# GeoMop/MLMC

Hardware: AMD Instinct MI355X
Metric: moment-evals/sec (samples x n_moments) (higher is better)
Workload: dtype f64

## Files before the change

mlmc_amd/csrc/api.hip:

```cpp
#include <cmath>
#include <chrono>
#include <cstring>
#include <new>

#include "common.hpp"
#include <algorithm>
#include <map>

namespace mlmc {

static thread_local std::string g_err;
void set_error(const std::string &msg) { g_err = msg; }
int fail(const std::string &msg) {
    g_err = msg;
    return 1;
}
Runtime &rt() {
    static Runtime r;
    return r;
}
std::recursive_mutex &api_mutex() {
    static std::recursive_mutex m;
    return m;
}

void bind_thread_to_device() {
    static thread_local int bound = -1;
    const Runtime &r = rt();
    if (r.ready && bound != r.device) {
        if (hipSetDevice(r.device) == hipSuccess) bound = r.device;
    } else if (!r.ready) {
        bound = -1;
    }
}

int ensure(void **p, size_t *cap, size_t bytes) {
    if (bytes <= *cap && *p) return 0;
    if (*p) {
        MLMC_HIP_CHECK(wait_stream(rt().stream));
        MLMC_HIP_CHECK(hipFree(*p));
        *p = nullptr;
        *cap = 0;
    }
    size_t want = bytes < 256 ? 256 : bytes;
    MLMC_HIP_CHECK(hipMalloc(p, want));
    *cap = want;
    return 0;
}

static int timing_collect(mlmc_accum *a);
int timing_begin(mlmc_accum *a) {
    if (!(rt().flags & 1)) return 0;
    if (a->ev_used >= 8192) {
        MLMC_HIP_CHECK(hipEventSynchronize(a->ev[a->ev_used - 1]));
        if (int rc = timing_collect(a)) return rc;
    }
    if (a->ev_used + 2 > a->ev.size()) {
        hipEvent_t e0, e1;
        MLMC_HIP_CHECK(hipEventCreate(&e0));
        MLMC_HIP_CHECK(hipEventCreate(&e1));
        a->ev.push_back(e0);
        a->ev.push_back(e1);
    }
    MLMC_HIP_CHECK(hipEventRecord(a->ev[a->ev_used], rt().stream));
    return 0;
}
int timing_end(mlmc_accum *a) {
    if (!(rt().flags & 1)) return 0;
    MLMC_HIP_CHECK(hipEventRecord(a->ev[a->ev_used + 1], rt().stream));
    a->ev_used += 2;
    return 0;
}
static int timing_collect(mlmc_accum *a) {
    for (size_t i = 0; i + 1 < a->ev_used; i += 2) {
        float ms = 0.f;
        MLMC_HIP_CHECK(hipEventElapsedTime(&ms, a->ev[i], a->ev[i + 1]));
        a->ms_total += ms;
    }
    a->ev_used = 0;
    return 0;
}

static void log_keep_interval(const BasisParams &p, double *x_lo, double *x_hi) {
    auto t_of = [&](uint64_t bits) {
        double x;
        std::memcpy(&x, &bits, sizeof x);
        volatile double v = std::log(x);
        volatile double w = (v - p.shift) * p.scale;
        return (double)(w + p.ref0);
    };
    auto as_double = [](uint64_t bits) { double x; std::memcpy(&x, &bits, sizeof x); return x; };
    const uint64_t top = 0x7ff0000000000000ull;
    uint64_t lo = 1, hi = top;
    while (lo < hi) {
        const uint64_t mid = lo + (hi - lo) / 2;
        if (t_of(mid) >= p.ref0) hi = mid; else lo = mid + 1;
    }
    const uint64_t first = lo;
    lo = 0; hi = top - 1;
    while (lo < hi) {
        const uint64_t mid = lo + (hi - lo + 1) / 2;
        if (t_of(mid) <= p.ref1) lo = mid; else hi = mid - 1;
    }
    const uint64_t last = lo;
    if (first >= top || last == 0 || first > last) {
        *x_lo = HUGE_VAL;
        *x_hi = 0.0;
        return;
    }
    *x_lo = as_double(first);
    *x_hi = as_double(last);
}

bool product_table(int kind, int R, std::vector<double> &out) {
    if (kind != MLMC_LEGENDRE && kind != MLMC_MONOMIAL) return false;
    const int K = 2 * R - 1;
    const size_t RR = (size_t)R * R;
    out.assign((size_t)K * RR, 0.0);
    for (int i = 0; i < R; ++i)
        for (int j = 0; j < R; ++j) {
            const size_t ij = (size_t)i * R + j;
            if (kind == MLMC_MONOMIAL) { out[(size_t)(i + j) * RR + ij] = 1.0; continue; }
            typedef long double ld;
            const int hi = i > j ? i : j, lo = i > j ? j : i;
            const ld diff = (ld)(hi - lo);
            ld c = (2 * diff + 1) / (2 * (ld)hi + 1);
            for (int t = 1; t <= lo; ++t) {
                const ld tt = (ld)t;
                c = c * ((2 * tt - 1) / tt * (diff + tt) / (2 * (diff + tt) - 1));
            }
            for (int t = 0; t <= lo; ++t) {
                const int k = (hi - lo) + 2 * t;
                out[(size_t)k * RR + ij] = (double)c;
                if (t == lo) break;
                const ld s = (ld)hi + t, kk = (ld)k;
                const ld si = s - hi, sj = s - lo, sk = s - kk;
                ld ratio = ((2 * kk + 5) / (2 * s + 3)) / ((2 * kk + 1) / (2 * s + 1));
                ratio = ratio * ((2 * si + 1) / (si + 1)) * ((2 * sj + 1) / (sj + 1));
                ratio = ratio * (sk / (2 * sk - 1));
                ratio = ratio * ((s + 1) / (2 * s + 1));
                c = c * ratio;
            }
        }
    return true;
}

bool square_product_table(int kind, int R, std::vector<double> &out) {
    if (kind != MLMC_LEGENDRE && kind != MLMC_MONOMIAL) return false;
    const int K = 4 * R - 3;
    const size_t RR = (size_t)R * R;
    out.assign((size_t)K * RR, 0.0);
    if (kind == MLMC_MONOMIAL) {
        for (int i = 0; i < R; ++i)
            for (int j = 0; j < R; ++j) out[(size_t)(2 * (i + j)) * RR + (size_t)i * R + j] = 1.0;
        return true;
    }
    typedef long double ld;
    const int Q = 4 * R;
    const ld pi = 3.14159265358979323846264338327950288L;
    std::vector<ld> x(Q), w(Q), P((size_t)K * Q);
    for (int q = 0; q < Q; ++q) {
        ld t = std::cos(pi * ((ld)q + 0.75L) / ((ld)Q + 0.5L)), dp = 1.0L;
        for (int it = 0; it < 100; ++it) {
            ld p0 = 1.0L, p1 = t;
            for (int k = 2; k <= Q; ++k) {
                const ld p2 = ((2 * k - 1) * t * p1 - (k - 1) * p0) / k;
                p0 = p1;
                p1 = p2;
            }
            dp = Q * (t * p1 - p0) / (t * t - 1.0L);
            const ld dt = p1 / dp;
            t -= dt;
            if (std::fabs(dt) < 1e-20L) break;
        }
        {
            ld p0 = 1.0L, p1 = t;
            for (int k = 2; k <= Q; ++k) {
                const ld p2 = ((2 * k - 1) * t * p1 - (k - 1) * p0) / k;
                p0 = p1;
                p1 = p2;
            }
            dp = Q * (t * p1 - p0) / (t * t - 1.0L);
        }
        x[q] = t;
        w[q] = 2.0L / ((1.0L - t * t) * dp * dp);
        ld p0 = 1.0L, p1 = t;
        P[(size_t)0 * Q + q] = 1.0L;
        if (K > 1) P[(size_t)1 * Q + q] = t;
        for (int k = 2; k < K; ++k) {
            const ld p2 = ((2 * k - 1) * t * p1 - (k - 1) * p0) / k;
            p0 = p1;
            p1 = p2;
            P[(size_t)k * Q + q] = p2;
        }
    }
    std::vector<ld> sq(Q);
    for (int i = 0; i < R; ++i)
        for (int j = i; j < R; ++j) {
            for (int q = 0; q < Q; ++q) {
                const ld u = P[(size_t)i * Q + q] * P[(size_t)j * Q + q];
                sq[q] = w[q] * u * u;
            }
            for (int k = 0; k <= 2 * (i + j); k += 2) {
                ld acc = 0.0L;
                const ld *Pk = &P[(size_t)k * Q];
                for (int q = 0; q < Q; ++q) acc += sq[q] * Pk[q];
                const double c = (double)(acc * (2 * k + 1) / 2);
                out[(size_t)k * RR + (size_t)i * R + j] = c;
                out[(size_t)k * RR + (size_t)j * R + i] = c;
            }
        }
    std::vector<double> t1;
    product_table(kind, R, t1);
    for (int j = 0; j < R; ++j)
        for (int k = 0; k < K; ++k) {
            const double c = k < 2 * R - 1 ? t1[(size_t)k * RR + (size_t)j * R + j] : 0.0;
            out[(size_t)k * RR + (size_t)j] = c;
            out[(size_t)k * RR + (size_t)j * R] = c;
        }
    return true;
}

static bool linearize_enabled() {
    const char *e = std::getenv("MLMC_HIP_LINEARIZE");
    return !(e && e[0] == '0');
}

static int lin_min_size() {
    const char *e = std::getenv("MLMC_HIP_LINEARIZE_MIN");
    return e ? std::atoi(e) : 16;
}

static int need_runtime() {
    if (!rt().ready) return fail("mlmc_init has not been called (no HIP device bound)");
    return 0;
}

}

using namespace mlmc;

extern "C" {

int mlmc_abi_version(void) { return MLMC_ABI_VERSION; }
const char *mlmc_last_error(void) { return g_err.c_str(); }

int mlmc_init(int device, int flags) {
    MLMC_API_GUARD;
    Runtime &r = rt();
    int count = 0;
    hipError_t e = hipGetDeviceCount(&count);
    if (e != hipSuccess || count <= 0) return fail("no HIP device available: libmlmc_hip has no CPU fallback");
    if (device < 0 || device >= count) return fail("mlmc_init: device index out of range");
    if (r.ready && r.device == device) {
        r.flags = flags;
        return 0;
    }
    if (r.ready) return fail("mlmc_init: this process is already bound to another device (one process per GPU)");
    MLMC_HIP_CHECK(hipSetDevice(device));
    MLMC_HIP_CHECK(hipGetDeviceProperties(&r.prop, device));
    if (std::strncmp(r.prop.gcnArchName, "gfx950", 6) != 0)
        return fail(std::string("mlmc_init: kernels are built for gfx950 only, device is ") + r.prop.gcnArchName);
    MLMC_HIP_CHECK(hipStreamCreateWithFlags(&r.stream, hipStreamNonBlocking));
    r.own_stream = true;
    r.device = device;
    r.flags = flags;
    r.n_cu = r.prop.multiProcessorCount;
    r.ready = true;
    return 0;
}

}

namespace mlmc {
hipError_t wait_stream(hipStream_t st) {
    const auto t0 = std::chrono::steady_clock::now();
    for (int spins = 0;; ++spins) {
        const hipError_t e = hipStreamQuery(st);
        if (e != hipErrorNotReady) return e;
        if ((spins & 63) == 63 && std::chrono::steady_clock::now() - t0 > std::chrono::milliseconds(4)) break;
    }
    return hipStreamSynchronize(st);
}
}

extern "C" {

int mlmc_set_stream(void *stream) {
    MLMC_API_GUARD;
    Runtime &r = rt();
    if (!r.ready) return fail("mlmc_init has not been called (no HIP device bound)");
    MLMC_HIP_CHECK(wait_stream(r.stream));
    if (r.own_stream) (void)hipStreamDestroy(r.stream);
    r.stream = (hipStream_t)stream;
    r.own_stream = false;
    return 0;
}

int mlmc_wait_event(void *hip_event) {
    MLMC_API_GUARD;
    Runtime &r = rt();
    if (!r.ready) return fail("mlmc_init has not been called (no HIP device bound)");
    if (!hip_event) return fail("mlmc_wait_event: null event");
    MLMC_HIP_CHECK(hipStreamWaitEvent(r.stream, (hipEvent_t)hip_event, 0));
    return 0;
}

int mlmc_synchronize(void) {
    MLMC_API_GUARD;
    Runtime &r = rt();
    if (!r.ready) return fail("mlmc_init has not been called (no HIP device bound)");
    MLMC_HIP_CHECK(wait_stream(r.stream));
    return 0;
}

void mlmc_shutdown(void) {
    MLMC_API_GUARD;
    Runtime &r = rt();
    if (!r.ready) return;
    (void)wait_stream(r.stream);
    if (r.own_stream) (void)hipStreamDestroy(r.stream);
    r.stream = nullptr;
    r.ready = false;
    r.device = -1;
}

int mlmc_device_info(char *name, int name_len, int *n_cu, int *wave_size, int64_t *hbm_bytes) {
    MLMC_API_GUARD;
    if (need_runtime()) return 1;
    if (name && name_len > 0) {
        std::strncpy(name, rt().prop.name, (size_t)name_len - 1);
        name[name_len - 1] = 0;
    }
    if (n_cu) *n_cu = rt().prop.multiProcessorCount;
    if (wave_size) *wave_size = rt().prop.warpSize;
    if (hbm_bytes) *hbm_bytes = (int64_t)rt().prop.totalGlobalMem;
    return 0;
}

int mlmc_basis_create(const mlmc_basis_desc *d, mlmc_basis **out) {
    MLMC_API_GUARD;
    if (need_runtime()) return 1;
    if (!d || !out) return fail("mlmc_basis_create: null argument");
    if (d->size <= 0) return fail("mlmc_basis_create: size must be > 0");
    if (d->kind < MLMC_LEGENDRE || d->kind > MLMC_SPLINE) return fail("mlmc_basis_create: unknown kind");
    if (d->kind == MLMC_SPLINE && d->size < 4) return fail("mlmc_basis_create: cubic spline moments need size >= 4");
    if (d->kind == MLMC_IDENTITY && d->size != 1) return fail("mlmc_basis_create: IDENTITY has size 1");
    if (d->out_size < 0 || (d->out_size > 0 && !d->matrix)) return fail("mlmc_basis_create: matrix missing");
    if (d->kind == MLMC_LEGENDRE && d->size > 512) return fail("mlmc_basis_create: at most 512 Legendre moments");
    mlmc_basis *b = new (std::nothrow) mlmc_basis();
    if (!b) return fail("out of memory");
    b->p.kind = d->kind;
    b->p.size = d->size;
    b->p.shift = d->shift;
    b->p.scale = d->scale;
    b->p.ref0 = d->ref0;
    b->p.ref1 = d->ref1;
    b->p.is_log = d->is_log;
    b->p.is_clip = d->is_clip;
    b->p.x_lo = d->x_lo;
    b->p.x_hi = d->x_hi;
    if (d->is_log && d->is_clip && d->x_lo == 0.0 && d->x_hi == 0.0) log_keep_interval(b->p, &b->p.x_lo, &b->p.x_hi);
    b->out_size = d->out_size;
    const int R = d->size;
    b->scale_c.assign(R, 1.0);
    if (d->kind == MLMC_LEGENDRE) {
        long double c = 1.0L;
        for (int i = 0; i < R; ++i) {
            if (i >= 1) c = c * (long double)(2 * i - 1) / (long double)(2 * i);
            b->scale_c[i] = (double)c;
        }
    }
    hipError_t e = hipMalloc(&b->d_scale, sizeof(double) * R);
    if (e == hipSuccess) e = hipMemcpy(b->d_scale, b->scale_c.data(), sizeof(double) * R, hipMemcpyHostToDevice);
    if (e == hipSuccess && d->out_size > 0) {
        b->matrix.assign(d->matrix, d->matrix + (size_t)d->out_size * R);
        e = hipMalloc(&b->d_matrix, sizeof(double) * b->matrix.size());
        if (e == hipSuccess)
            e = hipMemcpy(b->d_matrix, b->matrix.data(), sizeof(double) * b->matrix.size(), hipMemcpyHostToDevice);
    }
    if (e != hipSuccess) {
        mlmc_basis_destroy(b);
        return fail(std::string("mlmc_basis_create: ") + hipGetErrorString(e));
    }
    *out = b;
    return 0;
}

void mlmc_basis_destroy(mlmc_basis *b) {
    MLMC_API_GUARD;
    if (!b) return;
    if (b->d_scale) (void)hipFree(b->d_scale);
    if (b->d_matrix) (void)hipFree(b->d_matrix);
    delete b;
}

int mlmc_basis_eval(const mlmc_basis *b, const double *x, int64_t n, int32_t size, double *out, int mem_kind) {
    MLMC_API_GUARD;
    if (need_runtime()) return 1;
    if (!b || (n > 0 && (!x || !out))) return fail("mlmc_basis_eval: null argument");
    const int max_size = b->out_size > 0 ? b->out_size : b->p.size;
    if (size <= 0 || size > max_size) return fail("mlmc_basis_eval: size out of range");
    if (n == 0) return 0;
    hipStream_t st = rt().stream;
    if (mem_kind == MLMC_DEVICE) {
        if (int rc = launch_eval(b, x, n, size, out)) return rc;
        MLMC_HIP_CHECK(wait_stream(st));
        return 0;
    }
    double *d_x = nullptr, *d_o = nullptr;
    hipError_t e0 = hipMalloc(&d_x, sizeof(double) * (size_t)n);
    if (e0 == hipSuccess) e0 = hipMalloc(&d_o, sizeof(double) * (size_t)n * size);
    if (e0 == hipSuccess) e0 = hipMemcpyAsync(d_x, x, sizeof(double) * (size_t)n, hipMemcpyHostToDevice, st);
    int rc = e0 == hipSuccess ? launch_eval(b, d_x, n, size, d_o) : fail(std::string("mlmc_basis_eval: ") + hipGetErrorString(e0));
    if (!rc) {
        hipError_t e = hipMemcpyAsync(out, d_o, sizeof(double) * (size_t)n * size, hipMemcpyDeviceToHost, st);
        if (e == hipSuccess) e = wait_stream(st);
        if (e != hipSuccess) rc = fail(std::string("mlmc_basis_eval copy back: ") + hipGetErrorString(e));
    }
    (void)hipFree(d_x);
    (void)hipFree(d_o);
    return rc;
}

struct LinTables {
    double *d_prod = nullptr, *d_prod2 = nullptr;
};
static int lin_tables(int kind, int R, bool squares, LinTables **out) {
    static std::map<std::pair<int, int>, LinTables> cache;
    LinTables &t = cache[std::make_pair(kind, R)];
    if (!t.d_prod) {
        std::vector<double> h;
        product_table(kind, R, h);
        MLMC_HIP_CHECK(hipMalloc(&t.d_prod, sizeof(double) * h.size()));
        MLMC_HIP_CHECK(hipMemcpy(t.d_prod, h.data(), sizeof(double) * h.size(), hipMemcpyHostToDevice));
    }
    if (squares && !t.d_prod2) {
        std::vector<double> h;
        square_product_table(kind, R, h);
        MLMC_HIP_CHECK(hipMalloc(&t.d_prod2, sizeof(double) * h.size()));
        MLMC_HIP_CHECK(hipMemcpy(t.d_prod2, h.data(), sizeof(double) * h.size(), hipMemcpyHostToDevice));
    }
    *out = &t;
    return 0;
}

static int ensure_lin(mlmc_accum *a) {
    if (a->lin) return 0;
    const mlmc_basis *b = a->basis;
    LinTables *t = nullptr;
    if (int rc = lin_tables(b->p.kind, a->R, a->lin0_eligible, &t)) return rc;
    mlmc_basis_desc d;
    std::memset(&d, 0, sizeof(d));
    d.kind = b->p.kind;
    d.size = 2 * a->R - 1;
    d.shift = b->p.shift; d.scale = b->p.scale; d.ref0 = b->p.ref0; d.ref1 = b->p.ref1;
    d.is_log = b->p.is_log; d.is_clip = b->p.is_clip;
    d.x_lo = b->p.x_lo; d.x_hi = b->p.x_hi;
    int rc = mlmc_basis_create(&d, &a->lin_basis);
    if (!rc) rc = mlmc_accum_create(a->lin_basis, a->n_levels, MLMC_MODE_MOMENTS | MLMC_MODE_MEAN_ONLY, a->n_comp, &a->lin);
    if (!rc) {
        a->lin_basis->p.x_lo = b->p.x_lo;
        a->lin_basis->p.x_hi = b->p.x_hi;
        a->lin->host_outputs = false;
        a->lin_K = d.size;
        a->d_lin_prod = t->d_prod;
    }
    if (!rc && a->lin0_eligible) {
        d.size = 4 * a->R - 3;
        rc = mlmc_basis_create(&d, &a->lin0_basis);
        if (!rc) rc = mlmc_accum_create(a->lin0_basis, a->n_levels, MLMC_MODE_MOMENTS | MLMC_MODE_MEAN_ONLY, a->n_comp, &a->lin0);
        if (!rc) {
            a->lin0_basis->p.x_lo = b->p.x_lo;
            a->lin0_basis->p.x_hi = b->p.x_hi;
            a->lin0->host_outputs = false;
            a->lin0_K = d.size;
            a->d_lin0_prod = t->d_prod2;
        }
    }
    if (rc) {
        if (a->lin) mlmc_accum_destroy(a->lin);
        if (a->lin_basis) mlmc_basis_destroy(a->lin_basis);
        if (a->lin0) mlmc_accum_destroy(a->lin0);
        if (a->lin0_basis) mlmc_basis_destroy(a->lin0_basis);
        a->lin = a->lin0 = nullptr;
        a->lin_basis = a->lin0_basis = nullptr;
        a->lin_eligible = a->lin0_eligible = false;
    }
    return rc;
}

int mlmc_accum_create(const mlmc_basis *b, int32_t n_levels, int32_t mode, int32_t n_comp, mlmc_accum **out) {
    MLMC_API_GUARD;
    if (need_runtime()) return 1;
    if (!b || !out) return fail("mlmc_accum_create: null argument");
    if (n_levels <= 0 || n_comp <= 0) return fail("mlmc_accum_create: n_levels and n_comp must be > 0");
    const bool mean_only = (mode & MLMC_MODE_MEAN_ONLY) != 0;
    mode &= ~MLMC_MODE_MEAN_ONLY;
    if (mode != MLMC_MODE_MOMENTS && mode != MLMC_MODE_COV) return fail("mlmc_accum_create: unknown mode");
    mlmc_accum *a = new (std::nothrow) mlmc_accum();
    if (!a) return fail("out of memory");
    a->basis = b;
    a->n_levels = n_levels;
    a->mode = mode;
    const bool spline_band = mode == MLMC_MODE_COV && mean_only && b->out_size == 0 && b->p.kind == MLMC_SPLINE && b->p.size <= SPLINE_BAND_MAX_R;
    a->cov_from_values = mode == MLMC_MODE_COV && (b->out_size > 0 || (b->p.size > 128 && !spline_band));
    a->mean_only = mean_only && ((mode == MLMC_MODE_COV && !a->cov_from_values) || (mode == MLMC_MODE_MOMENTS && b->out_size > 0));
    a->mean_only_plain = mean_only && mode == MLMC_MODE_MOMENTS && b->out_size == 0 &&
                         (b->p.kind == MLMC_LEGENDRE || b->p.kind == MLMC_MONOMIAL) && b->p.size > 64 && b->p.size <= 256;
    a->n_comp = n_comp;
    a->R = b->p.size;
    a->Rout = b->out_size > 0 ? b->out_size : b->p.size;
    a->RP = (((mode == MLMC_MODE_COV && b->out_size > 0 ? a->Rout : a->R) + 15) / 16) * 16;
    if (mode == MLMC_MODE_MOMENTS) {
        a->K = (int64_t)n_comp * a->Rout;
        a->int_width = 2 * (int64_t)a->R + (b->out_size > 0 ? (int64_t)a->RP * a->RP : 0);
    } else {
        a->K = (int64_t)n_comp * a->Rout * a->Rout;
        a->int_width = 3 * (int64_t)a->RP * a->RP;
    }
    const size_t tot = (size_t)n_levels * n_comp * a->int_width;
    a->state_bytes = sizeof(double) * tot + sizeof(int64_t) * 2 * n_levels;
    a->out_bytes = (sizeof(int64_t) + sizeof(double)) * 2 * n_levels + 2 * sizeof(double) * (size_t)n_levels * a->K;
    if (hipMalloc(&a->d_state, a->state_bytes) != hipSuccess || hipMalloc(&a->d_out, a->out_bytes) != hipSuccess ||
        hipHostMalloc(&a->h_out, a->out_bytes, hipHostMallocDefault) != hipSuccess) {
        mlmc_accum_destroy(a);
        return fail("mlmc_accum_create: device / pinned allocation failed");
    }
    a->d_totals = (double *)a->d_state;
    a->d_counts = (int64_t *)(a->d_totals + tot);
    a->level_flushed.assign(n_levels, 0);
    if (mode == MLMC_MODE_MOMENTS && n_comp == 1 && b->out_size == 0) {
        void *dev_view = nullptr;
        if (hipHostGetDevicePointer(&dev_view, a->h_out, 0) == hipSuccess && dev_view) {
            a->host_outputs = true;
            a->h_out_n = (int64_t *)dev_view;
            a->h_out_s = (double *)(a->h_out_n + 2 * (size_t)n_levels) + 2 * (size_t)n_levels;
            a->h_out_sp = a->h_out_s + (size_t)n_levels * a->K;
        }
    }
    a->d_out_n = (int64_t *)a->d_out;
    a->d_out_nd = (double *)(a->d_out_n + 2 * (size_t)n_levels);
    a->d_out_s = a->d_out_nd + 2 * (size_t)n_levels;
    a->d_out_sp = a->d_out_s + (size_t)n_levels * a->K;
    if (mode == MLMC_MODE_COV && !mean_only && !a->cov_from_values && b->out_size == 0 && b->p.size > lin_min_size() && b->p.size <= 128 &&
        (b->p.kind == MLMC_LEGENDRE || b->p.kind == MLMC_MONOMIAL) && b->p.is_clip &&
        std::fabs(b->p.ref0) <= 1.0 && std::fabs(b->p.ref1) <= 1.0 &&
        linearize_enabled()) {
        a->lin_eligible = true;
        const char *min_n = std::getenv("MLMC_HIP_LINEARIZE_MIN_N");
        a->lin_min_n = min_n ? std::atoll(min_n) : (a->R > 32 ? 100000 : 1500000);
        const char *lin0_env = std::getenv("MLMC_HIP_LINEARIZE_LEVEL0");
        a->lin0_eligible = a->R <= 64 && !(lin0_env && lin0_env[0] == '0');
    }
    *out = a;
    return mlmc_accum_reset(a);
}

int mlmc_accum_reset(mlmc_accum *a) {
    MLMC_API_GUARD;
    if (need_runtime()) return 1;
    if (!a) return fail("mlmc_accum_reset: null argument");
    hipStream_t st = rt().stream;
    a->pending.clear();
    std::fill(a->level_flushed.begin(), a->level_flushed.end(), 0);
    MLMC_HIP_CHECK(hipMemsetAsync(a->d_state, 0, a->state_bytes, st));
    if (a->xcov) {
        MLMC_HIP_CHECK(hipMemcpyAsync(a->d_shift, a->shift_host.data(), sizeof(double) * a->shift_host.size(), hipMemcpyHostToDevice, st));
        a->xcov_pushes = 0;
    }
    a->lin_used = a->lin0_used = false;
    if (a->lin0)
        if (int rc = mlmc_accum_reset(a->lin0)) return rc;
    if (a->lin) return mlmc_accum_reset(a->lin);
    return 0;
}

void mlmc_accum_destroy(mlmc_accum *a) {
    MLMC_API_GUARD;
    if (!a) return;
    if (rt().ready) (void)wait_stream(rt().stream);
    if (a->lin) mlmc_accum_destroy(a->lin);
    if (a->lin_basis) mlmc_basis_destroy(a->lin_basis);
    if (a->lin0) mlmc_accum_destroy(a->lin0);
    if (a->lin0_basis) mlmc_basis_destroy(a->lin0_basis);
    void *ptrs[] = {a->d_state, a->d_partials, a->d_pcounts, a->d_stage_f, a->d_stage_c, a->d_mask, a->d_out, a->d_vals_f, a->d_vals_c, a->d_vals_tmp,
                    a->d_shift};
    for (void *p : ptrs)
        if (p) (void)hipFree(p);
    if (a->h_out) (void)hipHostFree(a->h_out);
    for (hipEvent_t e : a->ev) (void)hipEventDestroy(e);
    delete a;
}

int mlmc_accum_push(mlmc_accum *a, int32_t level, const double *fine, const double *coarse, int64_t n, int mem_kind) {
    MLMC_API_GUARD;
    if (need_runtime()) return 1;
    if (!a) return fail("mlmc_accum_push: null argument");
    if (level < 0 || level >= a->n_levels) return fail("mlmc_accum_push: level out of range");
    if (n < 0) return fail("mlmc_accum_push: negative n");
    if (n == 0) return 0;
    if (!fine) return fail("mlmc_accum_push: fine is NULL");
    if (n > ((int64_t)1 << 40)) return fail("mlmc_accum_push: chunk too large, split it");
    hipStream_t st = rt().stream;
    const size_t bytes = sizeof(double) * (size_t)n * a->n_comp;
    const double *d_f = fine, *d_c = coarse;
    if (mem_kind == MLMC_HOST) {
        if (bytes > a->stage_cap) {
            MLMC_HIP_CHECK(wait_stream(st));
            if (a->d_stage_f) (void)hipFree(a->d_stage_f);
            if (a->d_stage_c) (void)hipFree(a->d_stage_c);
            a->d_stage_f = a->d_stage_c = nullptr;
            a->stage_cap = 0;
            MLMC_HIP_CHECK(hipMalloc(&a->d_stage_f, bytes));
            MLMC_HIP_CHECK(hipMalloc(&a->d_stage_c, bytes));
            a->stage_cap = bytes;
        } else {
            MLMC_HIP_CHECK(wait_stream(st));
        }
        MLMC_HIP_CHECK(hipMemcpyAsync(a->d_stage_f, fine, bytes, hipMemcpyHostToDevice, st));
        d_f = a->d_stage_f;
        if (coarse) {
            MLMC_HIP_CHECK(hipMemcpyAsync(a->d_stage_c, coarse, bytes, hipMemcpyHostToDevice, st));
            d_c = a->d_stage_c;
        }
        MLMC_HIP_CHECK(wait_stream(st));
    } else if (mem_kind != MLMC_DEVICE) {
        return fail("mlmc_accum_push: bad mem_kind");
    }
    if (a->xcov) {
        ++a->xcov_pushes;
        return launch_xcov_push(a, level, d_f, d_c, n);
    }
    const uint8_t *d_mask = nullptr;
    bool count_in_kernel = true;
    if (a->n_comp > 1) {
        if (int rc = ensure((void **)&a->d_mask, &a->mask_cap, (size_t)n)) return rc;
        if (int rc = launch_mask(a, d_f, d_c, n, a->d_mask, a->d_counts + 2 * (int64_t)level)) return rc;
        d_mask = a->d_mask;
        count_in_kernel = false;
    }
    for (int m = 0; m < a->n_comp; ++m) {
        const double *f_m = d_f + (int64_t)m * n;
        const double *c_m = d_c ? d_c + (int64_t)m * n : nullptr;
        const bool count = count_in_kernel && m == 0;
        int rc;
        if (a->mode == MLMC_MODE_MOMENTS) {
            const bool defer = mem_kind == MLMC_DEVICE || a->n_comp > 1;
            rc = launch_moments_accum(a, level, m, f_m, c_m, d_mask, n, count, defer);
            if (!rc && a->basis->out_size > 0 && !a->mean_only) {
                if (a->R <= 128) {
                    rc = launch_cov_accum(a, level, m, f_m, c_m, d_mask, n, false, 1);
                } else {
                    int64_t chunk = 1 << 22;
                    while (chunk > 4096 && chunk * a->R > ((int64_t)1 << 28)) chunk >>= 1;
                    const size_t need = sizeof(double) * (size_t)(n < chunk ? n : chunk) * a->R;
                    if (need > a->vals_cap) {
                        MLMC_HIP_CHECK(wait_stream(st));
                        if (a->d_vals_f) (void)hipFree(a->d_vals_f);
                        if (a->d_vals_c) (void)hipFree(a->d_vals_c);
                        a->d_vals_f = a->d_vals_c = nullptr;
                        a->vals_cap = 0;
                        MLMC_HIP_CHECK(hipMalloc(&a->d_vals_f, need));
                        MLMC_HIP_CHECK(hipMalloc(&a->d_vals_c, need));
                        a->vals_cap = need;
                    }
                    for (int64_t off = 0; off < n && !rc; off += chunk) {
                        const int64_t m_n = (n - off < chunk) ? n - off : chunk;
                        rc = launch_eval_scaled_base(a->basis, f_m + off, m_n, a->d_vals_f);
                        if (!rc && c_m) rc = launch_eval_scaled_base(a->basis, c_m + off, m_n, a->d_vals_c);
                        if (!rc) rc = launch_cov_from_values(a, level, m, a->d_vals_f, c_m ? a->d_vals_c : nullptr,
                                                             d_mask ? d_mask + off : nullptr, m_n, false, 1);
                    }
                }
            }
        } else if (a->cov_from_values) {
            const int R1 = a->Rout;
            int64_t chunk = 1 << 22;
            while (chunk > 4096 && chunk * R1 > ((int64_t)1 << 28)) chunk >>= 1;
            const size_t need = sizeof(double) * (size_t)(n < chunk ? n : chunk) * R1;
            if (need > a->vals_cap) {
                MLMC_HIP_CHECK(wait_stream(st));
                if (a->d_vals_f) (void)hipFree(a->d_vals_f);
                if (a->d_vals_c) (void)hipFree(a->d_vals_c);
                a->d_vals_f = a->d_vals_c = nullptr;
                a->vals_cap = 0;
                MLMC_HIP_CHECK(hipMalloc(&a->d_vals_f, need));
                MLMC_HIP_CHECK(hipMalloc(&a->d_vals_c, need));
                a->vals_cap = need;
            }
            if (a->basis->out_size > 0) {
                const size_t need_tmp = sizeof(double) * (size_t)(n < chunk ? n : chunk) * a->R;
                if (need_tmp > a->vals_tmp_cap) {
                    MLMC_HIP_CHECK(wait_stream(st));
                    if (a->d_vals_tmp) (void)hipFree(a->d_vals_tmp);
                    a->d_vals_tmp = nullptr;
                    a->vals_tmp_cap = 0;
                    MLMC_HIP_CHECK(hipMalloc(&a->d_vals_tmp, need_tmp));
                    a->vals_tmp_cap = need_tmp;
                }
            }
            rc = 0;
            for (int64_t off = 0; off < n && !rc; off += chunk) {
                const int64_t m_n = (n - off < chunk) ? n - off : chunk;
                rc = launch_eval(a->basis, f_m + off, m_n, R1, a->d_vals_f, a->d_vals_tmp);
                if (!rc && c_m) rc = launch_eval(a->basis, c_m + off, m_n, R1, a->d_vals_c, a->d_vals_tmp);
                if (!rc) rc = launch_cov_from_values(a, level, m, a->d_vals_f, c_m ? a->d_vals_c : nullptr,
                                                     d_mask ? d_mask + off : nullptr, m_n, count);
            }
        } else {
            if (a->lin_eligible && !a->lin && n >= a->lin_min_n)
                if (int rcl = ensure_lin(a)) return rcl;
            const bool use_lin0 = a->lin0 && !d_c && n >= a->lin_min_n;
            if (use_lin0) {
                a->lin0_used = true;
                rc = launch_moments_accum(a->lin0, level, m, f_m, nullptr, d_mask, n, count_in_kernel && m == 0,
                                          mem_kind == MLMC_DEVICE || a->n_comp > 1);
                if (rc) return rc;
                continue;
            }
            const bool use_lin = a->lin && n >= a->lin_min_n;
            rc = m == 0 ? launch_cov_accum(a, level, 0, d_f, d_c, d_mask, n, count_in_kernel, a->mean_only ? 2 : (use_lin ? 3 : 0), a->n_comp) : 0;
            if (!rc && use_lin) a->lin_used = true;
            if (!rc && use_lin)
                rc = launch_moments_accum(a->lin, level, m, f_m, c_m, d_mask, n, false, mem_kind == MLMC_DEVICE || a->n_comp > 1);
        }
        if (rc) return rc;
    }
    if (a->mode == MLMC_MODE_MOMENTS && (mem_kind == MLMC_HOST || a->n_comp > 1))
        if (int rc = flush_moments(a)) return rc;
    if (a->lin && (mem_kind == MLMC_HOST || a->n_comp > 1))
        if (int rc = flush_moments(a->lin)) return rc;
    if (a->lin0 && (mem_kind == MLMC_HOST || a->n_comp > 1))
        if (int rc = flush_moments(a->lin0)) return rc;
    return 0;
}

int mlmc_accum_finalize(mlmc_accum *a, int64_t *n, int64_t *n_rm, double *s, double *sp, int mem_kind) {
    MLMC_API_GUARD;
    if (need_runtime()) return 1;
    if (!a || !n || !n_rm || !s || !sp) return fail("mlmc_accum_finalize: null argument");
    hipStream_t st = rt().stream;
    if (a->mode == MLMC_MODE_MOMENTS)
        if (int rcf = flush_moments(a)) return rcf;
    const int L = a->n_levels;
    const size_t nk = (size_t)L * a->K;
    if (a->host_outputs && mem_kind == MLMC_HOST) {
        MLMC_HIP_CHECK(wait_stream(st));
        const int64_t *hn = (const int64_t *)a->h_out;
        const double *hs = (const double *)(hn + 2 * (size_t)L) + 2 * (size_t)L;
        const size_t K = (size_t)a->K;
        for (int l = 0; l < L; ++l) {
            if (a->level_flushed[l]) {
                n[l] = hn[l];
                n_rm[l] = hn[L + l];
                std::memcpy(s + l * K, hs + l * K, sizeof(double) * K);
                std::memcpy(sp + l * K, hs + nk + l * K, sizeof(double) * K);
            } else {
                n[l] = n_rm[l] = 0;
                std::fill(s + l * K, s + (l + 1) * K, 0.0);
                std::fill(sp + l * K, sp + (l + 1) * K, 0.0);
            }
        }
        return 0;
    }
    int rc = a->xcov ? launch_xcov_finalize(a) : (a->mode == MLMC_MODE_MOMENTS) ? launch_moments_finalize(a) : launch_cov_finalize(a);
    if (rc) return rc;
    if (mem_kind == MLMC_DEVICE) {
        MLMC_HIP_CHECK(hipMemcpyAsync(n, a->d_out_n, sizeof(int64_t) * L, hipMemcpyDeviceToDevice, st));
        MLMC_HIP_CHECK(hipMemcpyAsync(n_rm, a->d_out_n + L, sizeof(int64_t) * L, hipMemcpyDeviceToDevice, st));
        MLMC_HIP_CHECK(hipMemcpyAsync(s, a->d_out_s, sizeof(double) * nk, hipMemcpyDeviceToDevice, st));
        MLMC_HIP_CHECK(hipMemcpyAsync(sp, a->d_out_sp, sizeof(double) * nk, hipMemcpyDeviceToDevice, st));
        MLMC_HIP_CHECK(wait_stream(st));
    } else {
        MLMC_HIP_CHECK(hipMemcpyAsync(a->h_out, a->d_out, a->out_bytes, hipMemcpyDeviceToHost, st));
        MLMC_HIP_CHECK(wait_stream(st));
        const int64_t *hn = (const int64_t *)a->h_out;
        const double *hs = (const double *)(hn + 2 * (size_t)L) + 2 * (size_t)L;
        std::memcpy(n, hn, sizeof(int64_t) * L);
        std::memcpy(n_rm, hn + L, sizeof(int64_t) * L);
        std::memcpy(s, hs, sizeof(double) * nk);
        std::memcpy(sp, hs + nk, sizeof(double) * nk);
    }
    return 0;
}

int mlmc_accum_estimate(mlmc_accum *a, int32_t n_chunks, const int32_t *levels, const double *const *fine,
                        const double *const *coarse, const int64_t *n_samples, int mem_kind, int64_t *n, int64_t *n_rm,
                        double *s, double *sp) {
    MLMC_API_GUARD;
    if (!a || n_chunks < 0 || (n_chunks > 0 && (!levels || !fine || !n_samples))) return fail("mlmc_accum_estimate: null argument");
    if (int rc = mlmc_accum_reset(a)) return rc;
    for (int k = 0; k < n_chunks; ++k)
        if (int rc = mlmc_accum_push(a, levels[k], fine[k], coarse ? coarse[k] : nullptr, n_samples[k], mem_kind)) return rc;
    return mlmc_accum_finalize(a, n, n_rm, s, sp, MLMC_HOST);
}

int mlmc_accum_finalize_packed(mlmc_accum *a, double *packed, int mem_kind) {
    MLMC_API_GUARD;
    if (need_runtime()) return 1;
    if (!a || !packed) return fail("mlmc_accum_finalize_packed: null argument");
    hipStream_t st = rt().stream;
    if (a->mode == MLMC_MODE_MOMENTS && a->host_outputs && mem_kind == MLMC_DEVICE && a->R <= MAX_TERMS_PER_PASS &&
        (int)a->pending.size() == a->n_levels &&
        std::none_of(a->level_flushed.begin(), a->level_flushed.end(), [](char f) { return f != 0; })) {
        a->packed_target = packed;
        const int rcf = flush_moments(a);
        a->packed_target = nullptr;
        return rcf;
    }
    if (a->mode == MLMC_MODE_MOMENTS)
        if (int rcf = flush_moments(a)) return rcf;
    int rc = a->xcov ? launch_xcov_finalize(a) : (a->mode == MLMC_MODE_MOMENTS) ? launch_moments_finalize(a) : launch_cov_finalize(a);
    if (rc) return rc;
    const size_t bytes = sizeof(double) * (2 * (size_t)a->n_levels + 2 * (size_t)a->n_levels * a->K);
    MLMC_HIP_CHECK(hipMemcpyAsync(packed, a->d_out_nd, bytes, mem_kind == MLMC_DEVICE ? hipMemcpyDeviceToDevice : hipMemcpyDeviceToHost, st));
    if (mem_kind == MLMC_DEVICE) return 0;
    MLMC_HIP_CHECK(wait_stream(st));
    return 0;
}

int mlmc_accum_estimate_packed(mlmc_accum *a, int32_t n_chunks, const int32_t *levels, const double *const *fine,
                               const double *const *coarse, const int64_t *n_samples, int mem_kind, double *packed,
                               int packed_kind) {
    MLMC_API_GUARD;
    if (!a || n_chunks < 0 || (n_chunks > 0 && (!levels || !fine || !n_samples))) return fail("mlmc_accum_estimate_packed: null argument");
    if (int rc = mlmc_accum_reset(a)) return rc;
    for (int k = 0; k < n_chunks; ++k)
        if (int rc = mlmc_accum_push(a, levels[k], fine[k], coarse ? coarse[k] : nullptr, n_samples[k], mem_kind)) return rc;
    return mlmc_accum_finalize_packed(a, packed, packed_kind);
}

int mlmc_accum_kernel_time(mlmc_accum *a, double *ms, int64_t *launches, int64_t *alg_bytes) {
    MLMC_API_GUARD;
    if (!a) return fail("mlmc_accum_kernel_time: null argument");
    if (a->ev_used) {
        MLMC_HIP_CHECK(hipEventSynchronize(a->ev[a->ev_used - 1]));
        if (int rc = timing_collect(a)) return rc;
    }
    if (ms) *ms = a->ms_total;
    if (launches) *launches = a->launches;
    if (alg_bytes) *alg_bytes = a->alg_bytes;
    a->ms_total = 0;
    a->launches = 0;
    a->alg_bytes = 0;
    return 0;
}

int mlmc_accum_aux_kernel_time(mlmc_accum *a, double *ms, int64_t *launches, int64_t *alg_bytes) {
    MLMC_API_GUARD;
    if (!a) return fail("mlmc_accum_aux_kernel_time: null argument");
    double t = 0.0, t0 = 0.0;
    int64_t l = 0, l0 = 0, b = 0, b0 = 0;
    if (a->lin)
        if (int rc = mlmc_accum_kernel_time(a->lin, &t, &l, &b)) return rc;
    if (a->lin0)
        if (int rc = mlmc_accum_kernel_time(a->lin0, &t0, &l0, &b0)) return rc;
    if (ms) *ms = t + t0;
    if (launches) *launches = l + l0;
    if (alg_bytes) *alg_bytes = b + b0;
    return 0;
}

int mlmc_linearization_table(int32_t kind, int32_t R, int32_t squares, double *out, int64_t out_len) {
    if (!out) return fail("mlmc_linearization_table: null argument");
    if (kind != MLMC_LEGENDRE && kind != MLMC_MONOMIAL) return fail("mlmc_linearization_table: Legendre or monomial moments");
    if (R < 1 || R > (squares ? 64 : 128)) return fail("mlmc_linearization_table: size out of range");
    const int64_t K = squares ? 4 * (int64_t)R - 3 : 2 * (int64_t)R - 1;
    if (out_len < K * R * R) return fail("mlmc_linearization_table: output too small");
    std::vector<double> t;
    if (squares) square_product_table(kind, R, t);
    else product_table(kind, R, t);
    std::memcpy(out, t.data(), sizeof(double) * t.size());
    return 0;
}

int mlmc_xcov_create(int32_t M, int32_t n_levels, int32_t flags, mlmc_accum **out) {
    MLMC_API_GUARD;
    if (need_runtime()) return 1;
    if (!out) return fail("mlmc_xcov_create: null argument");
    if (M < 1 || M > XCOV_MAX_M)
        return fail("mlmc_xcov_create: M = " + std::to_string(M) + " components, supported are 1 .. " + std::to_string(XCOV_MAX_M));
    if (n_levels <= 0) return fail("mlmc_xcov_create: n_levels must be > 0");
    if (flags & ~MLMC_MODE_MEAN_ONLY) return fail("mlmc_xcov_create: unknown flags (only MLMC_MODE_MEAN_ONLY)");
    mlmc_accum *a = new (std::nothrow) mlmc_accum();
    if (!a) return fail("out of memory");
    a->xcov = true;
    a->mode = MODE_XCOV;
    a->n_levels = n_levels;
    a->n_comp = M;
    a->mean_only = (flags & MLMC_MODE_MEAN_ONLY) != 0;
    a->K = (int64_t)M * M;
    a->int_width = 2 * a->K;
    const size_t tot = (size_t)n_levels * a->int_width;
    a->state_bytes = sizeof(double) * tot + sizeof(int64_t) * 2 * n_levels;
    a->out_bytes = (sizeof(int64_t) + sizeof(double)) * 2 * n_levels + 2 * sizeof(double) * (size_t)n_levels * a->K;
    a->shift_host.assign(M, 0.0);
    if (hipMalloc(&a->d_state, a->state_bytes) != hipSuccess || hipMalloc(&a->d_out, a->out_bytes) != hipSuccess ||
        hipMalloc(&a->d_shift, sizeof(double) * M) != hipSuccess ||
        hipHostMalloc(&a->h_out, a->out_bytes, hipHostMallocDefault) != hipSuccess) {
        mlmc_accum_destroy(a);
        return fail("mlmc_xcov_create: device / pinned allocation failed");
    }
    a->d_totals = (double *)a->d_state;
    a->d_counts = (int64_t *)(a->d_totals + tot);
    a->level_flushed.assign(n_levels, 0);
    a->d_out_n = (int64_t *)a->d_out;
    a->d_out_nd = (double *)(a->d_out_n + 2 * (size_t)n_levels);
    a->d_out_s = a->d_out_nd + 2 * (size_t)n_levels;
    a->d_out_sp = a->d_out_s + (size_t)n_levels * a->K;
    *out = a;
    return mlmc_accum_reset(a);
}

int mlmc_xcov_set_shift(mlmc_accum *a, const double *shift_host) {
    MLMC_API_GUARD;
    if (need_runtime()) return 1;
    if (!a) return fail("mlmc_xcov_set_shift: null argument");
    if (!a->xcov) return fail("mlmc_xcov_set_shift: not a component-covariance accumulator (mlmc_xcov_create)");
    if (a->xcov_pushes > 0) return fail("mlmc_xcov_set_shift: pushes are pending; reset the accumulator first");
    const int M = a->n_comp;
    if (shift_host)
        for (int m = 0; m < M; ++m)
            if (!std::isfinite(shift_host[m])) return fail("mlmc_xcov_set_shift: shift[" + std::to_string(m) + "] is not finite");
    MLMC_HIP_CHECK(wait_stream(rt().stream));
    if (shift_host) std::memcpy(a->shift_host.data(), shift_host, sizeof(double) * M);
    else std::fill(a->shift_host.begin(), a->shift_host.end(), 0.0);
    return 0;
}

int mlmc_accum_kernel_flops(mlmc_accum *a, int64_t *mfma_flops) {
    MLMC_API_GUARD;
    if (!a) return fail("mlmc_accum_kernel_flops: null argument");
    if (mfma_flops) *mfma_flops = a->mfma_flops;
    a->mfma_flops = 0;
    return 0;
}

}
```

mlmc_amd/csrc/common.hpp:

```cpp
#pragma once
#include <hip/hip_runtime.h>
#include <stdint.h>
#include <mutex>
#include <string>
#include <vector>

#include "../../include/mlmc_hip.h"

namespace mlmc {

constexpr int WAVE = 64;
constexpr int ACC_THREADS = 256;
#ifndef MLMC_TERMS_PER_PASS
#define MLMC_TERMS_PER_PASS 64
#endif
constexpr int MAX_TERMS_PER_PASS = MLMC_TERMS_PER_PASS;
constexpr int SPLINE_BAND_MAX_R = 256;

void set_error(const std::string &msg);
int fail(const std::string &msg);
#define MLMC_HIP_CHECK(expr)                                                                   \
    do {                                                                                       \
        hipError_t _e = (expr);                                                                \
        if (_e != hipSuccess)                                                                  \
            return ::mlmc::fail(std::string(#expr) + ": " + hipGetErrorString(_e));            \
    } while (0)

std::recursive_mutex &api_mutex();
void bind_thread_to_device();
struct ApiGuard {
    std::lock_guard<std::recursive_mutex> lock;
    ApiGuard() : lock(api_mutex()) { bind_thread_to_device(); }
};
#define MLMC_API_GUARD ::mlmc::ApiGuard mlmc_api_guard_

struct Runtime {
    bool ready = false;
    int device = -1;
    int flags = 0;
    int n_cu = 0;
    hipStream_t stream = nullptr;
    bool own_stream = false;
    hipDeviceProp_t prop;
};
Runtime &rt();
hipError_t wait_stream(hipStream_t st);

__device__ __forceinline__ unsigned long long order_key(double x) {
    unsigned long long u = (unsigned long long)__double_as_longlong(x);
    return (u >> 63) ? ~u : (u | 0x8000000000000000ull);
}

__device__ __forceinline__ void philox_round(uint32_t (&c)[4], uint32_t k0, uint32_t k1) {
    const uint64_t p0 = (uint64_t)0xD2511F53u * c[0], p1 = (uint64_t)0xCD9E8D57u * c[2];
    const uint32_t n0 = (uint32_t)(p1 >> 32) ^ c[1] ^ k0, n1 = (uint32_t)p1;
    const uint32_t n2 = (uint32_t)(p0 >> 32) ^ c[3] ^ k1, n3 = (uint32_t)p0;
    c[0] = n0; c[1] = n1; c[2] = n2; c[3] = n3;
}

struct BasisParams {
    int kind;
    int size;
    double shift, scale, ref0, ref1;
    int is_log, is_clip;
    double x_lo, x_hi;
};

}

struct mlmc_basis {
    mlmc::BasisParams p;
    int out_size = 0;
    std::vector<double> matrix;
    std::vector<double> scale_c;
    double *d_scale = nullptr;
    double *d_matrix = nullptr;
};

struct PendingSeg {
    const double *fine, *coarse;
    const uint8_t *mask;
    int64_t n;
    int level, comp;
    bool count;
};

struct mlmc_accum {
    const mlmc_basis *basis = nullptr;
    int n_levels = 0, mode = 0, n_comp = 1;
    bool mean_only = false;
    bool cov_from_values = false;
    bool mean_only_plain = false;
    int R = 0;
    int Rout = 0;
    int64_t K = 0;
    int64_t int_width = 0;
    void *d_state = nullptr;
    size_t state_bytes = 0;
    double *d_totals = nullptr;
    int64_t *d_counts = nullptr;
    double *d_partials = nullptr; size_t partials_cap = 0;
    int64_t *d_pcounts = nullptr; size_t pcounts_cap = 0;
    double *d_stage_f = nullptr, *d_stage_c = nullptr; size_t stage_cap = 0;
    uint8_t *d_mask = nullptr; size_t mask_cap = 0;
    double *d_vals_f = nullptr, *d_vals_c = nullptr; size_t vals_cap = 0;
    double *d_vals_tmp = nullptr; size_t vals_tmp_cap = 0;
    void *d_out = nullptr;
    size_t out_bytes = 0;
    void *h_out = nullptr;
    bool host_outputs = false;
    double *packed_target = nullptr;
    double *h_out_s = nullptr, *h_out_sp = nullptr; int64_t *h_out_n = nullptr;
    std::vector<char> level_flushed;
    double *d_out_s = nullptr, *d_out_sp = nullptr, *d_out_nd = nullptr; int64_t *d_out_n = nullptr;
    std::vector<hipEvent_t> ev;
    size_t ev_used = 0;
    double ms_total = 0;
    int64_t launches = 0, alg_bytes = 0;
    int64_t mfma_flops = 0;
    int RP = 0;
    bool lin_eligible = false, lin0_eligible = false;
    mlmc_accum *lin = nullptr;
    mlmc_basis *lin_basis = nullptr;
    double *d_lin_prod = nullptr;
    int lin_K = 0;
    mlmc_accum *lin0 = nullptr;
    mlmc_basis *lin0_basis = nullptr;
    double *d_lin0_prod = nullptr;
    int lin0_K = 0;
    bool lin0_used = false;
    int64_t lin_min_n = 0;
    bool lin_used = false;
    std::vector<PendingSeg> pending;
    bool xcov = false;
    double *d_shift = nullptr;
    std::vector<double> shift_host;
    int64_t xcov_pushes = 0;
};

namespace mlmc {
int launch_eval(const mlmc_basis *b, const double *d_x, int64_t n, int size, double *d_out, double *scratch = nullptr);
int launch_eval_scaled_base(const mlmc_basis *b, const double *d_x, int64_t n, double *d_out);
int launch_mask(const mlmc_accum *a, const double *d_f, const double *d_c, int64_t n, uint8_t *d_mask, int64_t *d_counts_level);
int launch_moments_accum(mlmc_accum *a, int level, int comp, const double *d_f, const double *d_c, const uint8_t *d_mask,
                         int64_t n, bool count, bool defer);
int flush_moments(mlmc_accum *a);
int launch_moments_finalize(mlmc_accum *a);
int launch_cov_accum(mlmc_accum *a, int level, int comp, const double *d_f, const double *d_c, const uint8_t *d_mask,
                     int64_t n, bool count, int gram_mode, int ncomp = 1);
int launch_cov_finalize(mlmc_accum *a);
constexpr int XCOV_MAX_M = 1024;
constexpr int MODE_XCOV = 2;
int launch_xcov_push(mlmc_accum *a, int level, const double *d_f, const double *d_c, int64_t n);
int launch_xcov_finalize(mlmc_accum *a);
bool product_table(int kind, int R, std::vector<double> &out);
bool square_product_table(int kind, int R, std::vector<double> &out);
int launch_cov_from_values(mlmc_accum *a, int level, int comp, const double *d_vf, const double *d_vc, const uint8_t *d_mask,
                           int64_t n, bool count, int gram_mode = 0);
int ensure(void **p, size_t *cap, size_t bytes);
void gauss_legendre(int n, std::vector<double> &x, std::vector<double> &w);
std::vector<double> effective_coeffs(const mlmc_basis *b, const double *lambda, const double *sigma, int R1);
int timing_begin(mlmc_accum *a);
int timing_end(mlmc_accum *a);
}
```

mlmc_amd/csrc/cov.hip:

```cpp
#include "device_basis.hpp"

namespace mlmc {

typedef double v4f64 __attribute__((ext_vector_type(4)));
#ifdef MLMC_PROF_COV
__device__ unsigned long long *g_prof_cov;
#define MLMC_COV_STAMP(slot)                                      \
    {                                                             \
        const unsigned long long now_ = __builtin_amdgcn_s_memtime(); \
        prof_acc[slot] += now_ - prof_t;                          \
        prof_t = now_;                                            \
    }
#else
#define MLMC_COV_STAMP(slot)
#endif
#ifndef MLMC_COV_PRIO_MFMA
#define MLMC_COV_PRIO_MFMA 0
#define MLMC_COV_PRIO_EVAL 2
#endif
#ifndef MLMC_COV_SLICE_BITS
#define MLMC_COV_SLICE_BITS 17
#endif
#ifndef MLMC_COV_EXTRA
#define MLMC_COV_EXTRA 2
#endif
#define MLMC_COV_MFMA_PRIO(ranks, slot, nslots, clock)                                                \
    do {                                                                                              \
        const unsigned t_ = (unsigned)((clock) >> MLMC_COV_SLICE_BITS);                               \
        unsigned top_ = t_ % (nslots);                                                                \
        if (MLMC_COV_EXTRA > 0) {                                                                     \
            const unsigned u_ = t_ % ((nslots) * MLMC_COV_EXTRA + 1u);                                \
            top_ = u_ == (nslots) * MLMC_COV_EXTRA ? (nslots) - 1u : u_ % (nslots);                   \
        }                                                                                             \
        const unsigned rank_ = ((slot) + (nslots) - top_ + (nslots) - 1u) % (nslots);   \
        if (ranks) {                                                                                  \
            if (rank_ == 0) __builtin_amdgcn_s_setprio(0);                                            \
            else if (rank_ == 1) __builtin_amdgcn_s_setprio(1);                                       \
            else if (rank_ == 2) __builtin_amdgcn_s_setprio(2);                                       \
            else __builtin_amdgcn_s_setprio(3);                                                       \
        } else {                                                                                      \
            if (rank_ == (nslots) - 1u) __builtin_amdgcn_s_setprio(1);                                \
            else __builtin_amdgcn_s_setprio(0);                                                       \
        }                                                                                             \
    } while (0)
#define MLMC_COV_EVAL_PRIO(ranks)                                                                     \
    do {                                                                                              \
        if (ranks) __builtin_amdgcn_s_setprio(3);                                                     \
        else __builtin_amdgcn_s_setprio(MLMC_COV_PRIO_EVAL);                                          \
    } while (0)
constexpr int COV_BATCH = 64;
#ifndef MLMC_COV_BLK22
#define MLMC_COV_BLK22 1
#endif
#ifndef MLMC_COV_T4_ONE_LIST
#define MLMC_COV_T4_ONE_LIST 1
#endif
#ifndef MLMC_COV_T4_BATCH
#define MLMC_COV_T4_BATCH 32
#define MLMC_COV_T4_WGS 4
#endif
constexpr int COV_T4_BATCH = MLMC_COV_T4_BATCH;
constexpr int COV_T4_WGS = MLMC_COV_T4_WGS;
#ifndef MLMC_COV_B128
#define MLMC_COV_B128 1
#endif
#ifndef MLMC_COV_B128_PAD
#define MLMC_COV_B128_PAD (MLMC_COV_B128 ? 4 : 2)
#endif
__device__ __forceinline__ int cov_t4_pos(int s) { return MLMC_COV_B128 ? ((s & ~7) | ((s & 3) << 1) | ((s >> 2) & 1)) : s; }
#ifndef MLMC_COV_WIDE_BATCH
#define MLMC_COV_WIDE_BATCH 32
#endif
__host__ __device__ constexpr int cov_ng(int mode) { return mode == 0 ? 3 : (mode == 3 ? 2 : 1); }
#ifndef MLMC_COV_VAR_RANKS
#define MLMC_COV_VAR_RANKS 1
#endif
__host__ __device__ constexpr int cov_batch(int T, bool wide, bool vals, bool pair = true) {
    return (T <= 2 && !wide && !vals) ? (pair ? 128 : 256) : ((wide && pair && !vals) ? MLMC_COV_WIDE_BATCH : 64);
}

template <int NT, int STRIDE, int TA>
__device__ __forceinline__ void cov_spline_store(const TermGen<MLMC_SPLINE> &g, double *__restrict__ dst, int samp) {
#pragma unroll
    for (int i = 0; i < NT; ++i) dst[i * STRIDE + samp] = 0.0;
    if (TA == 0) dst[samp] = g.w;
    const double nj[4] = {g.n0, g.n1, g.n2, g.n3};
#pragma unroll
    for (int j = 0; j < 4; ++j) {
        const int term = g.k + j;
        const int r = term - TA;
        if (term >= 1 && r >= 0 && r < NT) dst[r * STRIDE + samp] = nj[j];
    }
}

template <int KIND, int T, bool PAIR, int MODE, int BI = 0, int BJ = 0, bool VALS = false>
__global__ __launch_bounds__(256, (BI != BJ && (!PAIR || MLMC_COV_WIDE_BATCH == 64 || VALS)) ? 1 : 2) void k_cov_accum(BasisParams bp, 
                                                      const double *__restrict__ fine,
                                                      const double *__restrict__ coarse,
                                                      const uint8_t *__restrict__ mask, int64_t n, int R,
                                                      double *__restrict__ partials, int64_t *__restrict__ pcounts,
                                                      int vals_ta, int vals_tb) {
    constexpr int NT = 16 * T;
    constexpr int BATCH = cov_batch(T, BI != BJ, VALS, PAIR);
    constexpr int STRIDE = BATCH + 2;
    constexpr int NSL = 4 / T;
    constexpr bool M0 = MODE == 0 || MODE == 3;
    constexpr bool DO_G0 = MODE == 0;
    constexpr int NG = M0 ? (PAIR ? 3 : 2) : 1;
    constexpr bool WIDE = BI != BJ;
    constexpr int TA = 64 * BI, TB = 64 * BJ;
    constexpr int N_EVAL = (BI > BJ ? TA : TB) + NT;
    static_assert(T == 4 || (BI == 0 && BJ == 0), "term windows need T = 4");
    __shared__ double lds_f[NT * STRIDE];
    __shared__ double lds_c[PAIR ? NT * STRIDE : 1];
    __shared__ double lds_fb[WIDE ? NT * STRIDE : 1];
    __shared__ double lds_cb[(WIDE && PAIR) ? NT * STRIDE : 1];
    __shared__ int ldc[4][2];
    __shared__ unsigned char keep_s[VALS ? BATCH : 1];

    fine += (int64_t)blockIdx.y * n;
    if (PAIR) coarse += (int64_t)blockIdx.y * n;
    partials += (int64_t)blockIdx.y * gridDim.x * ((T <= 2 && BI == BJ) ? 4 : 4 / T) * ((M0 ? 3 : 1) * (16 * T) * (16 * T));
    if (blockIdx.y) pcounts = nullptr;

    const int lane = threadIdx.x & 63, wave = threadIdx.x >> 6;
    const int I = wave % T, kslice = wave / T;

    constexpr bool SLICED = (T <= 2) && !WIDE;
    constexpr int TI = SLICED ? T : 1;
    v4f64 acc[NG][TI][T];
#pragma unroll
    for (int g = 0; g < NG; ++g)
#pragma unroll
        for (int i = 0; i < TI; ++i)
#pragma unroll
            for (int j = 0; j < T; ++j) acc[g][i][j] = (v4f64){0.0, 0.0, 0.0, 0.0};

    const int n_eval_waves = PAIR ? BATCH / 32 : BATCH / 64;
    const bool evaluator = wave < n_eval_waves;
    const int samp = PAIR ? (wave * 32 + (lane & 31)) : (wave * 64 + lane);
    const bool is_coarse = PAIR && (lane >> 5);
    const double *__restrict__ src = is_coarse ? coarse : fine;
    double *__restrict__ dst = is_coarse ? lds_c : lds_f;
    double *__restrict__ dst_b = WIDE ? (is_coarse ? lds_cb : lds_fb) : dst;
    int n_keep = 0, n_rm = 0;

    const int64_t n_batches = (n + BATCH - 1) / BATCH;
    int64_t batch = blockIdx.x;
    double xv = 0.0;
    uint8_t mv = 1;
    if (!VALS && evaluator && batch < n_batches) {
        int64_t idx = batch * BATCH + samp;
        if (idx < n) { xv = src[idx]; if (mask) mv = mask[idx]; }
    }
    constexpr int VSPP = 256 / NT;
    constexpr int VNP = VALS ? BATCH / VSPP : 1;
    const int vtt = threadIdx.x % NT, vss = threadIdx.x / NT;
    const bool v_in_a = VALS && vals_ta + vtt < R, v_in_b = VALS && WIDE && vals_tb + vtt < R;
    double pf[VNP][4];
    auto vals_load = [&](int64_t b) {
#pragma unroll
        for (int p = 0; p < VNP; ++p) {
            int64_t idx = b * BATCH + p * VSPP + vss;
            if (idx >= n) idx = n - 1;
            const int64_t ra = idx * (int64_t)R + (v_in_a ? vals_ta + vtt : 0), rb = idx * (int64_t)R + (v_in_b ? vals_tb + vtt : 0);
            pf[p][0] = fine[ra];
            pf[p][1] = PAIR ? coarse[ra] : 0.0;
            pf[p][2] = WIDE ? fine[rb] : 0.0;
            pf[p][3] = (WIDE && PAIR) ? coarse[rb] : 0.0;
        }
    };
    if (VALS && batch < n_batches) vals_load(batch);
#ifdef MLMC_PROF_COV
    unsigned long long prof_acc[4] = {0, 0, 0, 0}, prof_t = __builtin_amdgcn_s_memtime();
    const unsigned long long prof_t0 = prof_t, prof_r0 = __builtin_amdgcn_s_memrealtime();
#endif
    __builtin_amdgcn_s_setprio(MLMC_COV_PRIO_EVAL);
    for (; batch < n_batches; batch += gridDim.x) {
        if (VALS) {
            if (threadIdx.x < BATCH) {
                const int64_t idx = batch * BATCH + threadIdx.x;
                const bool valid = idx < n;
                bool keep = valid && (!mask || mask[idx] != 0);
                if (keep) { const double v0 = fine[idx * (int64_t)R]; keep = !(v0 != v0); }
                if (PAIR && keep) { const double c0 = coarse[idx * (int64_t)R]; keep = !(c0 != c0); }
                n_keep += (int)keep;
                n_rm += (int)(valid && !keep);
                keep_s[threadIdx.x] = keep ? 1 : 0;
            }
            __syncthreads();
#pragma unroll
            for (int p = 0; p < VNP; ++p) {
                const int sl = p * VSPP + vss;
                const bool k = keep_s[sl] != 0;
                lds_f[vtt * STRIDE + sl] = (k && v_in_a) ? pf[p][0] : 0.0;
                if (PAIR) lds_c[vtt * STRIDE + sl] = (k && v_in_a) ? pf[p][1] : 0.0;
                if (WIDE) {
                    lds_fb[vtt * STRIDE + sl] = (k && v_in_b) ? pf[p][2] : 0.0;
                    if (PAIR) lds_cb[vtt * STRIDE + sl] = (k && v_in_b) ? pf[p][3] : 0.0;
                }
            }
            if (batch + gridDim.x < n_batches) vals_load(batch + gridDim.x);
        } else if (evaluator) {
            const int64_t idx = batch * BATCH + samp;
            const bool valid = idx < n;
            bool keep;
            double t = transform_value(bp, xv, keep);
            keep = keep && valid && (mv != 0);
            if (PAIR) {
                const int other = __shfl_xor((int)keep, 32, 64);
                keep = keep && (other != 0);
            }
            if (!is_coarse) { n_keep += (int)keep; n_rm += (int)(valid && !keep); }
            const int64_t nidx = (batch + gridDim.x) * BATCH + samp;
            if (nidx < n) { xv = src[nidx]; if (mask) mv = mask[nidx]; }
            TermGen<KIND> g;
            g.init(keep ? t : 0.0, keep ? 1.0 : 0.0, bp);
            if constexpr (KIND == MLMC_SPLINE) {
                cov_spline_store<NT, STRIDE, TA>(g, dst, samp);
                if (WIDE) cov_spline_store<NT, STRIDE, TB>(g, dst_b, samp);
            } else {
#pragma unroll
                for (int i = 0; i < N_EVAL; ++i) {
                    const double q = g.next(i);
                    if (i >= TA && i < TA + NT) dst[(i - TA) * STRIDE + samp] = q;
                    if (WIDE && i >= TB && i < TB + NT) dst_b[(i - TB) * STRIDE + samp] = q;
                }
            }
        }
        MLMC_COV_STAMP(0)
        __syncthreads();
        MLMC_COV_STAMP(1)
        __builtin_amdgcn_s_setprio(MLMC_COV_PRIO_MFMA);
        if constexpr (SLICED) {
            const int rowl = lane & 15;
#pragma unroll
            for (int kk = 0; kk < BATCH / 16; ++kk) {
                const int col = 4 * (wave + 4 * kk) + (lane >> 4);
                double d[T], sv[T], dd[T], ss[T], ds[T];
#pragma unroll
                for (int i = 0; i < T; ++i) {
                    const double f = lds_f[(16 * i + rowl) * STRIDE + col];
                    d[i] = sv[i] = f;
                    if (PAIR) {
                        const double c = lds_c[(16 * i + rowl) * STRIDE + col];
                        d[i] = f - c;
                        sv[i] = f + c;
                    }
                    if (M0) {
                        dd[i] = d[i] * d[i];
                        ss[i] = sv[i] * sv[i];
                        ds[i] = d[i] * sv[i];
                    }
                }
#pragma unroll
                for (int i = 0; i < T; ++i)
#pragma unroll
                    for (int j = 0; j < T; ++j) {
                        const bool upper = j >= i;
                        if (M0) {
                            if (DO_G0 && (PAIR || upper)) acc[0][i][j] = __builtin_amdgcn_mfma_f64_16x16x4f64(d[i], sv[j], acc[0][i][j], 0, 0, 0);
                            if (PAIR || upper) acc[1][i][j] = __builtin_amdgcn_mfma_f64_16x16x4f64(dd[i], ss[j], acc[1][i][j], 0, 0, 0);
                            if (PAIR && upper) acc[NG - 1][i][j] = __builtin_amdgcn_mfma_f64_16x16x4f64(ds[i], ds[j], acc[NG - 1][i][j], 0, 0, 0);
                        } else if (MODE == 1 || !PAIR) {
                            if (upper) acc[0][i][j] = __builtin_amdgcn_mfma_f64_16x16x4f64(d[i], d[j], acc[0][i][j], 0, 0, 0);
                        } else {
                            acc[0][i][j] = __builtin_amdgcn_mfma_f64_16x16x4f64(d[i], sv[j], acc[0][i][j], 0, 0, 0);
                        }
                    }
            }
            __builtin_amdgcn_s_setprio(MLMC_COV_PRIO_EVAL);
            MLMC_COV_STAMP(2)
            __syncthreads();
            MLMC_COV_STAMP(3)
            continue;
        }
        const int arow = 16 * I + (lane & 15);
#pragma unroll
        for (int kk = 0; kk < BATCH / 4 / NSL; ++kk) {
            const int ks = kslice + kk * NSL;
            const int col = 4 * ks + (lane >> 4);
            double fa = lds_f[arow * STRIDE + col];
            double da = fa, sa = fa;
            if (PAIR) {
                double ca = lds_c[arow * STRIDE + col];
                da = fa - ca;
                sa = fa + ca;
            }
            const double a1 = da * da, a2 = da * sa;
#pragma unroll
            for (int J = 0; J < T; ++J) {
                const int brow = 16 * J + (lane & 15);
                double fb = (WIDE ? lds_fb : lds_f)[brow * STRIDE + col];
                double db = fb, sb = fb;
                if (PAIR) {
                    double cb = (WIDE ? lds_cb : lds_c)[brow * STRIDE + col];
                    db = fb - cb;
                    sb = fb + cb;
                }
                if (M0) {
                    if (DO_G0) acc[0][0][J] = __builtin_amdgcn_mfma_f64_16x16x4f64(da, sb, acc[0][0][J], 0, 0, 0);
                    if (PAIR) {
                        acc[1][0][J] = __builtin_amdgcn_mfma_f64_16x16x4f64(a1, sb * sb, acc[1][0][J], 0, 0, 0);
                        acc[2][0][J] = __builtin_amdgcn_mfma_f64_16x16x4f64(a2, db * sb, acc[2][0][J], 0, 0, 0);
                    } else {
                        acc[1][0][J] = __builtin_amdgcn_mfma_f64_16x16x4f64(a1, fb * fb, acc[1][0][J], 0, 0, 0);
                    }
                } else {
                    acc[0][0][J] = __builtin_amdgcn_mfma_f64_16x16x4f64(da, MODE == 2 ? sb : db, acc[0][0][J], 0, 0, 0);
                }
            }
        }
        __builtin_amdgcn_s_setprio(MLMC_COV_PRIO_EVAL);
        __syncthreads();
    }

#ifdef MLMC_PROF_COV
    if (lane == 0 && blockIdx.y == 0) {
        unsigned long long *q = g_prof_cov + ((size_t)blockIdx.x * 4 + wave) * 6;
        q[0] = prof_acc[0]; q[1] = prof_acc[1]; q[2] = prof_acc[2]; q[3] = prof_acc[3];
        q[4] = __builtin_amdgcn_s_memtime() - prof_t0;
        q[5] = ((unsigned long long)__builtin_amdgcn_s_getreg((4 << 0) | (0 << 6) | (31 << 11)) & 0xffffu) |
               ((unsigned long long)__builtin_amdgcn_s_getreg((20 << 0) | (0 << 6) | (3 << 11)) << 16) |
               ((__builtin_amdgcn_s_memrealtime() - prof_r0) << 24);
    }
#endif
    constexpr int NGOUT = M0 ? 3 : 1;
    double *__restrict__ prow = partials + (SLICED ? ((int64_t)blockIdx.x * 4 + wave) : ((int64_t)blockIdx.x * NSL + kslice)) * (NGOUT * NT * NT);
#pragma unroll
    for (int Iw = 0; Iw < TI; ++Iw) {
        const int It = SLICED ? Iw : I;
#pragma unroll
        for (int J = 0; J < T; ++J) {
#pragma unroll
            for (int r = 0; r < 4; ++r) {
                const int row = 16 * It + (lane >> 4) + 4 * r;
                const int col = 16 * J + (lane & 15);
                const bool low = SLICED && J < It;
                const int mirror = (16 * It + (lane & 15)) * NT + (16 * J + (lane >> 4) + 4 * r);
                if (M0) {
                    if (PAIR) {
                        prow[0 * NT * NT + row * NT + col] = acc[0][Iw][J][r];
                        prow[1 * NT * NT + row * NT + col] = acc[1][Iw][J][r];
                        if (!low) prow[2 * NT * NT + row * NT + col] = acc[NG - 1][Iw][J][r];
                        else prow[2 * NT * NT + mirror] = acc[NG - 1][SLICED ? J : 0][It][r];
                    } else if (!low) {
                        prow[0 * NT * NT + row * NT + col] = acc[0][Iw][J][r];
                        prow[1 * NT * NT + row * NT + col] = acc[1][Iw][J][r];
                        prow[2 * NT * NT + row * NT + col] = acc[1][Iw][J][r];
                    } else {
                        prow[0 * NT * NT + mirror] = acc[0][SLICED ? J : 0][It][r];
                        prow[1 * NT * NT + mirror] = acc[1][SLICED ? J : 0][It][r];
                        prow[2 * NT * NT + mirror] = acc[1][SLICED ? J : 0][It][r];
                    }
                } else if (low && (MODE == 1 || !PAIR)) {
                    prow[mirror] = acc[0][SLICED ? J : 0][It][r];
                } else {
                    prow[row * NT + col] = acc[0][Iw][J][r];
                }
            }
        }
    }
    if (pcounts) {
        n_keep = wave_sum_i(n_keep);
        n_rm = wave_sum_i(n_rm);
        if (lane == 0) { ldc[wave][0] = n_keep; ldc[wave][1] = n_rm; }
        __syncthreads();
        if (threadIdx.x < 2) {
            const int v = ldc[0][threadIdx.x] + ldc[1][threadIdx.x] + ldc[2][threadIdx.x] + ldc[3][threadIdx.x];
            pcounts[(int64_t)blockIdx.x * 2 + threadIdx.x] = v;
        }
    }
}

__host__ __device__ constexpr int sym_n(int w) { return w < 2 ? 2 : 3; }
__host__ __device__ constexpr int sym_i(int w, int t) { return t == 0 ? w : (w < 2 ? w : (w == 2 ? (t == 1 ? 2 : 0) : (t == 1 ? 0 : 1))); }
__host__ __device__ constexpr int sym_j(int w, int t) { return t == 0 ? w : (w < 2 ? w + 1 : (w == 2 ? (t == 1 ? 3 : 2) : 3)); }
__host__ __device__ constexpr int psym_n(int w) { return w == 0 ? 1 : 3; }
__host__ __device__ constexpr int psym_i(int w, int t) { return t == 0 ? w : (w == 1 ? (t == 1 ? 1 : 0) : (w == 2 ? (t == 1 ? 2 : 0) : (t == 1 ? 0 : 1))); }
__host__ __device__ constexpr int psym_j(int w, int t) { return t == 0 ? w : (w == 1 ? (t == 1 ? 2 : 1) : (w == 2 ? (t == 1 ? 3 : 2) : 3)); }
__host__ __device__ constexpr int bsym_n(int w) { return (w == 0 || w == 3) ? 3 : 2; }
__host__ __device__ constexpr int bsym_i(int w, int t) { return w == 0 ? (t == 2 ? 1 : 0) : (w == 1 ? 0 : (w == 2 ? 1 : (t == 2 ? 3 : 2))); }
__host__ __device__ constexpr int bsym_j(int w, int t) { return w == 0 ? (t == 0 ? 0 : 1) : (w == 1 ? 2 + t : (w == 2 ? 2 + t : (t == 0 ? 2 : 3))); }
__host__ __device__ constexpr int xsym_n(int kind, int w) { return kind == 2 ? bsym_n(w) : (kind == 1 ? psym_n(w) : sym_n(w)); }
__host__ __device__ constexpr int xsym_i(int kind, int w, int t) { return kind == 2 ? bsym_i(w, t) : (kind == 1 ? psym_i(w, t) : sym_i(w, t)); }
__host__ __device__ constexpr int xsym_j(int kind, int w, int t) { return kind == 2 ? bsym_j(w, t) : (kind == 1 ? psym_j(w, t) : sym_j(w, t)); }

template <int KIND, bool PAIR, int MODE, int BD, int W>
__device__ __forceinline__ void cov_t4_body(const BasisParams &bp, 
                                            const double *__restrict__ fine, const double *__restrict__ coarse,
                                            const uint8_t *__restrict__ mask, int64_t n, double *__restrict__ partials,
                                            int64_t *__restrict__ pcounts, double *__restrict__ lds_f,
                                            double *__restrict__ lds_c, int (*ldc)[2]) {
    constexpr int NT = 64;
    constexpr int TA = 64 * BD;
    constexpr int N_EVAL = TA + NT;
    constexpr bool BLK = PAIR && (MODE == 0 || MODE == 3) && MLMC_COV_BLK22 && COV_T4_BATCH == 32;
    constexpr bool BLK2 = PAIR && MODE == 2 && MLMC_COV_BLK22 && COV_T4_BATCH == 32;
    constexpr int ONE = BLK ? 2 : ((PAIR && MLMC_COV_T4_ONE_LIST && COV_T4_BATCH == 32) ? 1 : 0);
    constexpr int NS = xsym_n(ONE, W);
    constexpr int W1 = (MODE == 0 && !PAIR) ? (W + 2) % 4 : W;
    constexpr int NS1 = sym_n(W1);
    constexpr int NFULL = (MODE == 0 && PAIR) ? 2 : (((MODE == 2 || MODE == 3) && PAIR) ? 1 : 0);
    constexpr int GV = MODE == 3 ? 0 : 1;
    constexpr int NSYMM = (MODE == 0 && !PAIR) ? 2 : 1;
    const int lane = threadIdx.x & 63;

    v4f64 accf[NFULL > 0 ? NFULL : 1][4];
    v4f64 accs[NSYMM][3];
#pragma unroll
    for (int g = 0; g < (NFULL > 0 ? NFULL : 1); ++g)
#pragma unroll
        for (int j = 0; j < 4; ++j) accf[g][j] = (v4f64){0.0, 0.0, 0.0, 0.0};
#pragma unroll
    for (int g = 0; g < NSYMM; ++g)
#pragma unroll
        for (int t = 0; t < 3; ++t) accs[g][t] = (v4f64){0.0, 0.0, 0.0, 0.0};

    constexpr int BATCH = PAIR ? COV_T4_BATCH : 2 * COV_T4_BATCH;
    constexpr int STRIDE = BATCH + MLMC_COV_B128_PAD;
    constexpr bool evaluator = BLK ? (W == 1) : (W < COV_T4_BATCH / 32);
    constexpr int EW = BLK ? 0 : W;
    const int samp = PAIR ? (EW * 32 + (lane & 31)) : (EW * 64 + lane);
    const int psamp = cov_t4_pos(samp);
    const bool is_coarse = PAIR && (lane >> 5);
    const double *__restrict__ src = is_coarse ? coarse : fine;
    double *__restrict__ dst = is_coarse ? lds_c : lds_f;
    int n_keep = 0, n_rm = 0;

    const int64_t n_batches = (n + BATCH - 1) / BATCH;
    int64_t batch = blockIdx.x;
    double xv = 0.0;
    uint8_t mv = 1;
    if (evaluator && batch < n_batches) {
        int64_t idx = batch * BATCH + samp;
        if (idx < n) { xv = src[idx]; if (mask) mv = mask[idx]; }
    }
#ifdef MLMC_PROF_COV
    unsigned long long prof_acc[4] = {0, 0, 0, 0}, prof_t = __builtin_amdgcn_s_memtime();
    const unsigned long long prof_t0 = prof_t, prof_r0 = __builtin_amdgcn_s_memrealtime();
#endif
    constexpr bool RANKS = (MODE == 0 || (MODE == 3 && MLMC_COV_VAR_RANKS)) && PAIR;
    const unsigned per_round = gridDim.x >= (unsigned)COV_T4_WGS ? gridDim.x / (unsigned)COV_T4_WGS : 1u;
    const unsigned prio_slot = (blockIdx.x / per_round) % (unsigned)COV_T4_WGS;
    MLMC_COV_EVAL_PRIO(RANKS);
    for (; batch < n_batches; batch += gridDim.x) {
        if (evaluator) {
            const int64_t idx = batch * BATCH + samp;
            const bool valid = idx < n;
            bool keep;
            double t = transform_value(bp, xv, keep);
            keep = keep && valid && (mv != 0);
            if (PAIR) {
                const int other = __shfl_xor((int)keep, 32, 64);
                keep = keep && (other != 0);
            }
            if (!is_coarse) { n_keep += (int)keep; n_rm += (int)(valid && !keep); }
            const int64_t nidx = (batch + gridDim.x) * BATCH + samp;
            if (nidx < n) { xv = src[nidx]; if (mask) mv = mask[nidx]; }
            TermGen<KIND> g;
            g.init(keep ? t : 0.0, keep ? 1.0 : 0.0, bp);
            if constexpr (KIND == MLMC_SPLINE) {
                cov_spline_store<NT, STRIDE, TA>(g, dst, psamp);
            } else {
#pragma unroll
                for (int i = 0; i < N_EVAL; ++i) {
                    const double q = g.next(i);
                    if (i >= TA) dst[(i - TA) * STRIDE + psamp] = q;
                }
            }
        }
        MLMC_COV_STAMP(0)
        const unsigned long long prio_clock = __builtin_amdgcn_s_memtime();
        __syncthreads();
        MLMC_COV_STAMP(1)
        MLMC_COV_MFMA_PRIO(RANKS, prio_slot, (unsigned)COV_T4_WGS, prio_clock);
        typedef double v2f64 __attribute__((ext_vector_type(2)));
        v2f64 f2[4], c2[4];
#pragma unroll
        for (int ks = 0; ks < BATCH / 4; ++ks) {
            const int col = 4 * ks + (lane >> 4);
            double d[4], sm[4];
#pragma unroll
            for (int J = 0; J < 4; ++J) {
                const int row = 16 * J + (lane & 15);
                double f, c = 0.0;
                if (MLMC_COV_B128) {
                    if ((ks & 1) == 0) {
                        const int base = row * STRIDE + 8 * (ks >> 1) + 2 * (lane >> 4);
                        f2[J] = *reinterpret_cast<const v2f64 *>(lds_f + base);
                        if (PAIR) c2[J] = *reinterpret_cast<const v2f64 *>(lds_c + base);
                    }
                    f = (ks & 1) ? f2[J].y : f2[J].x;
                    if (PAIR) c = (ks & 1) ? c2[J].y : c2[J].x;
                } else {
                    f = lds_f[row * STRIDE + col];
                    if (PAIR) c = lds_c[row * STRIDE + col];
                }
                d[J] = f;
                sm[J] = f;
                if (PAIR) {
                    d[J] = f - c;
                    sm[J] = f + c;
                }
            }
            if (BLK) {
                constexpr int RA = 2 * (W >> 1), CA = 2 * (W & 1);
                double ds[4];
#pragma unroll
                for (int J = 0; J < 4; ++J) ds[J] = d[J] * sm[J];
#pragma unroll
                for (int r = 0; r < 2; ++r) {
                    const double dr2 = d[RA + r] * d[RA + r];
#pragma unroll
                    for (int c = 0; c < 2; ++c) {
                        if (MODE == 0)
                            accf[0][2 * r + c] = __builtin_amdgcn_mfma_f64_16x16x4f64(d[RA + r], sm[CA + c], accf[0][2 * r + c], 0, 0, 0);
                        accf[GV][2 * r + c] = __builtin_amdgcn_mfma_f64_16x16x4f64(dr2, sm[CA + c] * sm[CA + c], accf[GV][2 * r + c], 0, 0, 0);
                    }
                }
#pragma unroll
                for (int t = 0; t < NS; ++t)
                    accs[0][t] = __builtin_amdgcn_mfma_f64_16x16x4f64(ds[xsym_i(ONE, W, t)], ds[xsym_j(ONE, W, t)], accs[0][t], 0, 0, 0);
            } else if ((MODE == 0 || MODE == 3) && PAIR) {
                const double dw2 = d[W] * d[W];
                double ds[4];
#pragma unroll
                for (int J = 0; J < 4; ++J) {
                    if (MODE == 0) accf[0][J] = __builtin_amdgcn_mfma_f64_16x16x4f64(d[W], sm[J], accf[0][J], 0, 0, 0);
                    accf[GV][J] = __builtin_amdgcn_mfma_f64_16x16x4f64(dw2, sm[J] * sm[J], accf[GV][J], 0, 0, 0);
                    ds[J] = d[J] * sm[J];
                }
#pragma unroll
                for (int t = 0; t < NS; ++t)
                    accs[0][t] = __builtin_amdgcn_mfma_f64_16x16x4f64(ds[xsym_i(ONE, W, t)], ds[xsym_j(ONE, W, t)], accs[0][t], 0, 0, 0);
            } else if (MODE == 0) {
                double f2[4];
#pragma unroll
                for (int J = 0; J < 4; ++J) f2[J] = d[J] * d[J];
#pragma unroll
                for (int t = 0; t < NS; ++t)
                    accs[0][t] = __builtin_amdgcn_mfma_f64_16x16x4f64(d[xsym_i(ONE, W, t)], d[xsym_j(ONE, W, t)], accs[0][t], 0, 0, 0);
#pragma unroll
                for (int t = 0; t < NS1; ++t)
                    accs[1][t] = __builtin_amdgcn_mfma_f64_16x16x4f64(f2[sym_i(W1, t)], f2[sym_j(W1, t)], accs[1][t], 0, 0, 0);
            } else if (MODE == 3) {
                double f2[4];
#pragma unroll
                for (int J = 0; J < 4; ++J) f2[J] = d[J] * d[J];
#pragma unroll
                for (int t = 0; t < NS; ++t)
                    accs[0][t] = __builtin_amdgcn_mfma_f64_16x16x4f64(f2[xsym_i(ONE, W, t)], f2[xsym_j(ONE, W, t)], accs[0][t], 0, 0, 0);
            } else if (MODE == 2 && PAIR && BLK2) {
                constexpr int RA = 2 * (W >> 1), CA = 2 * (W & 1);
#pragma unroll
                for (int r = 0; r < 2; ++r)
#pragma unroll
                    for (int c = 0; c < 2; ++c)
                        accf[0][2 * r + c] = __builtin_amdgcn_mfma_f64_16x16x4f64(d[RA + r], sm[CA + c], accf[0][2 * r + c], 0, 0, 0);
            } else if (MODE == 2 && PAIR) {
#pragma unroll
                for (int J = 0; J < 4; ++J)
                    accf[0][J] = __builtin_amdgcn_mfma_f64_16x16x4f64(d[W], sm[J], accf[0][J], 0, 0, 0);
            } else {
#pragma unroll
                for (int t = 0; t < NS; ++t)
                    accs[0][t] = __builtin_amdgcn_mfma_f64_16x16x4f64(d[xsym_i(ONE, W, t)], d[xsym_j(ONE, W, t)], accs[0][t], 0, 0, 0);
            }
        }
        MLMC_COV_EVAL_PRIO(RANKS);
        MLMC_COV_STAMP(2)
        __syncthreads();
        MLMC_COV_STAMP(3)
    }
#ifdef MLMC_PROF_COV
    if (lane == 0 && blockIdx.y == 0) {
        unsigned long long *q = g_prof_cov + ((size_t)blockIdx.x * 4 + W) * 6;
        q[0] = prof_acc[0]; q[1] = prof_acc[1]; q[2] = prof_acc[2]; q[3] = prof_acc[3];
        q[4] = __builtin_amdgcn_s_memtime() - prof_t0;
        q[5] = ((unsigned long long)__builtin_amdgcn_s_getreg((4 << 0) | (0 << 6) | (31 << 11)) & 0xffffu) |
               ((unsigned long long)__builtin_amdgcn_s_getreg((20 << 0) | (0 << 6) | (3 << 11)) << 16) |
               ((__builtin_amdgcn_s_memrealtime() - prof_r0) << 24);
    }
#endif

    constexpr int NGOUT = cov_ng(MODE);
    double *__restrict__ prow = partials + (int64_t)blockIdx.x * (NGOUT * NT * NT);
    const int r0 = lane >> 4, c0 = lane & 15;
    if (MODE == 3 && PAIR) {
#pragma unroll
        for (int J = 0; J < 4; ++J)
#pragma unroll
            for (int r = 0; r < 4; ++r) {
                const int tr = BLK ? 2 * (W >> 1) + (J >> 1) : W, tc = BLK ? 2 * (W & 1) + (J & 1) : J;
                prow[(16 * tr + r0 + 4 * r) * NT + 16 * tc + c0] = accf[0][J][r];
            }
    }
    if (MODE == 0 && PAIR) {
#pragma unroll
        for (int J = 0; J < 4; ++J)
#pragma unroll
            for (int r = 0; r < 4; ++r) {
                const int tr = BLK ? 2 * (W >> 1) + (J >> 1) : W, tc = BLK ? 2 * (W & 1) + (J & 1) : J;
                const int row = 16 * tr + r0 + 4 * r, col = 16 * tc + c0;
                prow[0 * NT * NT + row * NT + col] = accf[0][J][r];
                prow[1 * NT * NT + row * NT + col] = accf[1][J][r];
            }
    }
    if (MODE == 2 && PAIR) {
#pragma unroll
        for (int J = 0; J < 4; ++J)
#pragma unroll
            for (int r = 0; r < 4; ++r) {
                const int tr = BLK2 ? 2 * (W >> 1) + (J >> 1) : W, tc = BLK2 ? 2 * (W & 1) + (J & 1) : J;
                prow[(16 * tr + r0 + 4 * r) * NT + 16 * tc + c0] = accf[0][J][r];
            }
    }
#pragma unroll
    for (int t = 0; t < ((MODE == 2 && PAIR) ? 0 : NS); ++t)
#pragma unroll
        for (int r = 0; r < 4; ++r) {
            const int row = 16 * xsym_i(ONE, W, t) + r0 + 4 * r, col = 16 * xsym_j(ONE, W, t) + c0;
            if (MODE == 0 && PAIR) {
                prow[2 * NT * NT + row * NT + col] = accs[0][t][r];
                if (xsym_i(ONE, W, t) != xsym_j(ONE, W, t)) prow[2 * NT * NT + col * NT + row] = accs[0][t][r];
            } else if (MODE == 3) {
                const bool off = xsym_i(ONE, W, t) != xsym_j(ONE, W, t);
                prow[NT * NT + row * NT + col] = accs[0][t][r];
                if (off) prow[NT * NT + col * NT + row] = accs[0][t][r];
                if (!PAIR) {
                    prow[row * NT + col] = accs[0][t][r];
                    if (off) prow[col * NT + row] = accs[0][t][r];
                }
            } else if (MODE == 0) {
                prow[0 * NT * NT + row * NT + col] = accs[0][t][r];
                if (xsym_i(ONE, W, t) != xsym_j(ONE, W, t)) prow[0 * NT * NT + col * NT + row] = accs[0][t][r];
            } else {
                prow[row * NT + col] = accs[0][t][r];
                if (xsym_i(ONE, W, t) != xsym_j(ONE, W, t)) prow[col * NT + row] = accs[0][t][r];
            }
        }
    if (MODE == 0 && !PAIR) {
#pragma unroll
        for (int t = 0; t < NS1; ++t)
#pragma unroll
            for (int r = 0; r < 4; ++r) {
                const int row = 16 * sym_i(W1, t) + r0 + 4 * r, col = 16 * sym_j(W1, t) + c0;
                prow[1 * NT * NT + row * NT + col] = accs[1][t][r];
                prow[2 * NT * NT + row * NT + col] = accs[1][t][r];
                if (sym_i(W1, t) != sym_j(W1, t)) {
                    prow[1 * NT * NT + col * NT + row] = accs[1][t][r];
                    prow[2 * NT * NT + col * NT + row] = accs[1][t][r];
                }
            }
    }
    if (pcounts) {
        n_keep = wave_sum_i(n_keep);
        n_rm = wave_sum_i(n_rm);
        if (lane == 0 && W < 2) { ldc[W][0] = n_keep; ldc[W][1] = n_rm; }
        __syncthreads();
        if (threadIdx.x < 2) pcounts[(int64_t)blockIdx.x * 2 + threadIdx.x] = ldc[0][threadIdx.x] + ldc[1][threadIdx.x];
    }
}

template <int KIND, bool PAIR, int MODE, int BD>
__global__ __launch_bounds__(256, COV_T4_WGS) void k_cov_accum_t4(BasisParams bp, 
                                                         const double *__restrict__ fine, const double *__restrict__ coarse,
                                                         const uint8_t *__restrict__ mask, int64_t n, int R,
                                                         double *__restrict__ partials, int64_t *__restrict__ pcounts) {
    __shared__ __attribute__((aligned(16))) double lds_f[64 * ((PAIR ? COV_T4_BATCH : 2 * COV_T4_BATCH) + MLMC_COV_B128_PAD)];
    __shared__ __attribute__((aligned(16))) double lds_c[PAIR ? 64 * (COV_T4_BATCH + MLMC_COV_B128_PAD) : 1];
    __shared__ int ldc[2][2];
    (void)R;
    fine += (int64_t)blockIdx.y * n;
    if (PAIR) coarse += (int64_t)blockIdx.y * n;
    partials += (int64_t)blockIdx.y * gridDim.x * (cov_ng(MODE) * 64 * 64);
    if (blockIdx.y) pcounts = nullptr;
    switch (__builtin_amdgcn_readfirstlane((int)(threadIdx.x >> 6))) {
        case 0: cov_t4_body<KIND, PAIR, MODE, BD, 0>(bp, fine, coarse, mask, n, partials, pcounts, lds_f, lds_c, ldc); break;
        case 1: cov_t4_body<KIND, PAIR, MODE, BD, 1>(bp, fine, coarse, mask, n, partials, pcounts, lds_f, lds_c, ldc); break;
        case 2: cov_t4_body<KIND, PAIR, MODE, BD, 2>(bp, fine, coarse, mask, n, partials, pcounts, lds_f, lds_c, ldc); break;
        default: cov_t4_body<KIND, PAIR, MODE, BD, 3>(bp, fine, coarse, mask, n, partials, pcounts, lds_f, lds_c, ldc); break;
    }
}

__global__ __launch_bounds__(1024) void k_reduce_cov(const double *__restrict__ partials, int nrows, int NT, int NG, int RP,
                                                    int roff, int coff, double *__restrict__ totals, int64_t comp_stride,
                                                    int mirror, const int64_t *__restrict__ pcounts, int nblocks,
                                                    int64_t *__restrict__ counts) {
    __shared__ double lds[64][17];
    const int c = threadIdx.x & 15, g = threadIdx.x >> 4;
    const int width = NG * NT * NT;
    if (pcounts && blockIdx.x == gridDim.x - 1) {
        if (blockIdx.y == 0 && threadIdx.x < 64) {
            int64_t a = 0, b = 0;
            for (int i = threadIdx.x; i < nblocks; i += 64) { a += pcounts[2 * i]; b += pcounts[2 * i + 1]; }
            for (int off = 32; off >= 1; off >>= 1) { a += __shfl_xor(a, off, 64); b += __shfl_xor(b, off, 64); }
            if (threadIdx.x == 0) { counts[0] += a; counts[1] += b; }
        }
        return;
    }
    partials += (int64_t)blockIdx.y * nrows * width;
    totals += (int64_t)blockIdx.y * comp_stride;
    const int col = blockIdx.x * 16 + c;
    double acc = 0.0;
    if (col < width)
        for (int b = g; b < nrows; b += 64) acc += partials[(int64_t)b * width + col];
    lds[g][c] = acc;
    __syncthreads();
    if (g == 0 && col < width) {
        double v = 0.0;
#pragma unroll
        for (int k = 0; k < 64; ++k) v += lds[k][c];
        const int gi = col / (NT * NT), rem = col % (NT * NT);
        const int row = roff + rem / NT, cc = coff + rem % NT;
        if (row < RP && cc < RP) {
            totals[(int64_t)gi * RP * RP + (int64_t)row * RP + cc] += v;
            if (mirror) totals[(int64_t)gi * RP * RP + (int64_t)cc * RP + row] += v;
        }
    }
}

template <int KIND, int T, int MODE, int BI, int BJ>
static int launch_cov_t(const BasisParams &bp, bool pair, int blocks, int ncomp, const double *d_f, const double *d_c,
                        const uint8_t *d_mask, int64_t n, int R, double *partials, int64_t *pcounts) {
    hipStream_t st = rt().stream;
    if constexpr (T == 4 && BI == BJ) {
        if (pair)
            hipLaunchKernelGGL((k_cov_accum_t4<KIND, true, MODE, BI>), dim3(blocks, ncomp), dim3(256), 0, st, bp, d_f, d_c, d_mask, n, R, partials, pcounts);
        else
            hipLaunchKernelGGL((k_cov_accum_t4<KIND, false, MODE, BI>), dim3(blocks, ncomp), dim3(256), 0, st, bp, d_f, d_c, d_mask, n, R, partials, pcounts);
    } else {
        if (pair)
            hipLaunchKernelGGL((k_cov_accum<KIND, T, true, MODE, BI, BJ>), dim3(blocks, ncomp), dim3(256), 0, st, bp, d_f, d_c, d_mask, n, R, partials, pcounts, 0, 0);
        else
            hipLaunchKernelGGL((k_cov_accum<KIND, T, false, MODE, BI, BJ>), dim3(blocks, ncomp), dim3(256), 0, st, bp, d_f, d_c, d_mask, n, R, partials, pcounts, 0, 0);
    }
    MLMC_HIP_CHECK(hipGetLastError());
    return 0;
}

template <int KIND, int MODE>
static int launch_cov_kind(const BasisParams &bp, int T, int bi, int bj, bool pair, int blocks, int ncomp, const double *d_f,
                           const double *d_c, const uint8_t *d_mask, int64_t n, int R, double *partials, int64_t *pcounts) {
#define MLMC_COV_ARGS bp, pair, blocks, ncomp, d_f, d_c, d_mask, n, R, partials, pcounts
    if (T == 1) return launch_cov_t<KIND, 1, MODE, 0, 0>(MLMC_COV_ARGS);
    if (T == 2) return launch_cov_t<KIND, 2, MODE, 0, 0>(MLMC_COV_ARGS);
    if (bi == 0 && bj == 0) return launch_cov_t<KIND, 4, MODE, 0, 0>(MLMC_COV_ARGS);
    if (bi == 0 && bj == 1) return launch_cov_t<KIND, 4, MODE, 0, 1>(MLMC_COV_ARGS);
    if (bi == 1 && bj == 0) return launch_cov_t<KIND, 4, MODE, 1, 0>(MLMC_COV_ARGS);
    if (bi == 1 && bj == 1) return launch_cov_t<KIND, 4, MODE, 1, 1>(MLMC_COV_ARGS);
#undef MLMC_COV_ARGS
    return fail("covariance: at most 128 moments");
}

int launch_cov_from_values(mlmc_accum *a, int level, int comp, const double *d_vf, const double *d_vc, const uint8_t *d_mask,
                           int64_t n, bool count, int gram_mode) {
    if (n == 0) return 0;
    const bool diff_gram = gram_mode == 1;
    const int R = diff_gram ? a->R : a->Rout;
    hipStream_t st = rt().stream;
    const int T = (R <= 16) ? 1 : (R <= 32 ? 2 : 4);
    const int NT = 16 * T, NSL = 4 / T;
    const bool pair = d_vc != nullptr;
    const int NB = (R + 63) / 64;
    const int64_t n_batches = (n + COV_BATCH - 1) / COV_BATCH;
    const int NG = diff_gram ? 1 : 3;
    const size_t width = (size_t)NG * NT * NT;
    const BasisParams &bp = a->basis->p;
    double *totals = a->d_totals + ((int64_t)level * a->n_comp + comp) * a->int_width + (diff_gram ? 2 * (int64_t)R : 0);
    const bool symmetric = !pair || diff_gram;
    for (int bi = 0; bi < NB; ++bi)
        for (int bj = 0; bj < NB; ++bj) {
            if (symmetric && bj < bi) continue;
            const bool wide = bi != bj;
            int blocks = rt().n_cu * (wide ? 1 : 2);
            if (n_batches < blocks) blocks = (int)n_batches;
            const int n_slices = T <= 2 ? 4 : NSL;
            if (int rc = ensure((void **)&a->d_partials, &a->partials_cap, sizeof(double) * (size_t)blocks * n_slices * width)) return rc;
            if (int rc = ensure((void **)&a->d_pcounts, &a->pcounts_cap, sizeof(int64_t) * (size_t)blocks * 2)) return rc;
            const bool do_count = count && bi == 0 && bj == 0 && !diff_gram;
            int64_t *pc = do_count ? a->d_pcounts : nullptr;
            if (int rc = timing_begin(a)) return rc;
#define MLMC_COV_VALS1(TT, BJJ, MODE)                                                                                           \
    do {                                                                                                                        \
        if (pair)                                                                                                               \
            hipLaunchKernelGGL((k_cov_accum<MLMC_IDENTITY, TT, true, MODE, 0, BJJ, true>), dim3(blocks), dim3(256), 0, st, bp,      \
                               d_vf, d_vc, d_mask, n, R, a->d_partials, pc, 64 * bi, 64 * bj);                                  \
        else                                                                                                                    \
            hipLaunchKernelGGL((k_cov_accum<MLMC_IDENTITY, TT, false, MODE, 0, BJJ, true>), dim3(blocks), dim3(256), 0, st, bp,     \
                               d_vf, d_vc, d_mask, n, R, a->d_partials, pc, 64 * bi, 64 * bj);                                  \
    } while (0)
#define MLMC_COV_VALS(TT, BJJ)                                                                                                  \
    do {                                                                                                                        \
        if (diff_gram) MLMC_COV_VALS1(TT, BJJ, 1); else MLMC_COV_VALS1(TT, BJJ, 0);                                             \
    } while (0)
            if (T == 1) MLMC_COV_VALS(1, 0);
            else if (T == 2) MLMC_COV_VALS(2, 0);
            else if (!wide) MLMC_COV_VALS(4, 0);
            else MLMC_COV_VALS(4, 1);
#undef MLMC_COV_VALS
#undef MLMC_COV_VALS1
            MLMC_HIP_CHECK(hipGetLastError());
            if (int rc = timing_end(a)) return rc;
            if (!diff_gram) {
                a->launches += 1;
                a->alg_bytes += (int64_t)n * (pair ? 16 : 8);
                a->mfma_flops += (int64_t)512 * n * (T <= 2 ? (pair ? 2 * T * T + T * (T + 1) / 2 : T * (T + 1)) : (pair ? 3 : 2) * 16);
            }
            hipLaunchKernelGGL(k_reduce_cov, dim3((unsigned)((width + 15) / 16) + (do_count ? 1u : 0u)), dim3(1024), 0, st, a->d_partials,
                               blocks * n_slices, NT, NG, a->RP, 64 * bi, 64 * bj, totals, (int64_t)0, (symmetric && wide) ? 1 : 0,
                               do_count ? a->d_pcounts : (const int64_t *)nullptr, blocks, a->d_counts + 2 * (int64_t)level);
            MLMC_HIP_CHECK(hipGetLastError());
        }
    return 0;
}

constexpr int BAND_W = 5;
template <bool PAIR>
__global__ __launch_bounds__(256) void k_spline_band_accum(BasisParams bp, const double *__restrict__ fine,
                                                          const double *__restrict__ coarse, const uint8_t *__restrict__ mask,
                                                          int64_t n, int R, double *__restrict__ partials,
                                                          int64_t *__restrict__ pcounts) {
    extern __shared__ double band_tab[];
    __shared__ int ldc[4][2];
    const int RP8 = R + 8;
    fine += (int64_t)blockIdx.y * n;
    if (PAIR) coarse += (int64_t)blockIdx.y * n;
    partials += (int64_t)blockIdx.y * gridDim.x * (BAND_W * R);
    if (blockIdx.y) pcounts = nullptr;
    const int lane = threadIdx.x & 63, wave = threadIdx.x >> 6;
    for (int i = threadIdx.x; i < 4 * RP8 * BAND_W; i += 256) band_tab[i] = 0.0;
    __syncthreads();
    double *__restrict__ tab = band_tab + (size_t)wave * RP8 * BAND_W;
    int n_keep = 0, n_rm = 0;
    const int64_t T = (int64_t)gridDim.x * 256;
    for (int64_t i = (int64_t)blockIdx.x * 256 + threadIdx.x; i < n; i += T) {
        bool kf, kc = true;
        const double tf = transform_value(bp, fine[i], kf);
        double tc = 0.0;
        if (PAIR) tc = transform_value(bp, coarse[i], kc);
        const bool keep = kf && kc && (!mask || mask[i] != 0);
        n_keep += (int)keep;
        n_rm += (int)!keep;
        if (!keep) continue;
        TermGen<MLMC_SPLINE> gf, gc;
        gf.init(tf, 1.0, bp);
        const double nf[4] = {gf.n0, gf.n1, gf.n2, gf.n3};
        double nc[4] = {0.0, 0.0, 0.0, 0.0};
        bool same = false;
        if (PAIR) {
            gc.init(tc, 1.0, bp);
            nc[0] = gc.n0; nc[1] = gc.n1; nc[2] = gc.n2; nc[3] = gc.n3;
            same = gc.k == gf.k;
        }
#pragma unroll
        for (int j = 0; j < 4; ++j) {
            const int r = gf.k + j;
            if (r < 1) continue;
            double *__restrict__ row = tab + (size_t)r * BAND_W;
            atomicAdd(&row[4], same ? nf[j] - nc[j] : nf[j]);
#pragma unroll
            for (int j2 = j; j2 < 4; ++j2)
                atomicAdd(&row[j2 - j], same ? __builtin_fma(nf[j], nf[j2], -(nc[j] * nc[j2])) : nf[j] * nf[j2]);
        }
        if (PAIR && !same) {
#pragma unroll
            for (int j = 0; j < 4; ++j) {
                const int r = gc.k + j;
                if (r < 1) continue;
                double *__restrict__ row = tab + (size_t)r * BAND_W;
                atomicAdd(&row[4], -nc[j]);
#pragma unroll
                for (int j2 = j; j2 < 4; ++j2) atomicAdd(&row[j2 - j], -(nc[j] * nc[j2]));
            }
        }
    }
    n_keep = wave_sum_i(n_keep);
    n_rm = wave_sum_i(n_rm);
    if (lane == 0) { ldc[wave][0] = n_keep; ldc[wave][1] = n_rm; }
    __syncthreads();
    for (int j = threadIdx.x; j < BAND_W * R; j += 256) {
        const int o = j;
        partials[(int64_t)blockIdx.x * (BAND_W * R) + j] =
            ((band_tab[o] + band_tab[(size_t)RP8 * BAND_W + o]) + band_tab[(size_t)2 * RP8 * BAND_W + o]) + band_tab[(size_t)3 * RP8 * BAND_W + o];
    }
    if (pcounts && threadIdx.x < 2)
        pcounts[(int64_t)blockIdx.x * 2 + threadIdx.x] = ldc[0][threadIdx.x] + ldc[1][threadIdx.x] + ldc[2][threadIdx.x] + ldc[3][threadIdx.x];
}

__global__ __launch_bounds__(1024) void k_reduce_band(const double *__restrict__ partials, const int64_t *__restrict__ pcounts, int nblocks,
                                                     int R, int RP, double *__restrict__ totals, int64_t comp_stride,
                                                     int64_t *__restrict__ counts, int corner) {
    __shared__ double lds[64][17];
    __shared__ long long lc[16][2];
    const int width = BAND_W * R;
    const int n_col_groups = (width + 15) / 16;
    totals += (int64_t)blockIdx.y * comp_stride;
    if ((int)blockIdx.x == n_col_groups) {
        long long a = 0, b = 0;
        for (int i = threadIdx.x; i < nblocks; i += 1024) { a += pcounts[2 * i]; b += pcounts[2 * i + 1]; }
        for (int off = 32; off >= 1; off >>= 1) { a += __shfl_xor(a, off, 64); b += __shfl_xor(b, off, 64); }
        if ((threadIdx.x & 63) == 0) { lc[threadIdx.x >> 6][0] = a; lc[threadIdx.x >> 6][1] = b; }
        __syncthreads();
        if (threadIdx.x == 0) {
            a = 0; b = 0;
            for (int w = 0; w < 16; ++w) { a += lc[w][0]; b += lc[w][1]; }
            if (counts && blockIdx.y == 0) { counts[0] += a; counts[1] += b; }
            if (corner) totals[0] += (double)a;
        }
        return;
    }
    partials += (int64_t)blockIdx.y * nblocks * width;
    const int c = threadIdx.x & 15, g = threadIdx.x >> 4;
    const int col = blockIdx.x * 16 + c;
    double acc = 0.0;
    if (col < width)
        for (int b = g; b < nblocks; b += 64) acc += partials[(int64_t)b * width + col];
    lds[g][c] = acc;
    __syncthreads();
    if (g == 0 && col < width) {
        double v = 0.0;
#pragma unroll
        for (int k = 0; k < 64; ++k) v += lds[k][c];
        const int r = col / BAND_W, w = col % BAND_W;
        if (r >= 1) {
            if (w == 4) {
                totals[r] += v;
                totals[(int64_t)r * RP] += v;
            } else if (r + w < R) {
                totals[(int64_t)r * RP + r + w] += v;
                if (w) totals[(int64_t)(r + w) * RP + r] += v;
            }
        }
    }
}

static int launch_spline_band(mlmc_accum *a, int level, int comp, const double *d_f, const double *d_c, const uint8_t *d_mask, int64_t n,
                              bool count, int ncomp) {
    hipStream_t st = rt().stream;
    const int R = a->R;
    const bool pair = d_c != nullptr;
    int blocks = rt().n_cu * 4;
    const int64_t want = (n + 255) / 256;
    if (want < blocks) blocks = (int)want;
    if (int rc = ensure((void **)&a->d_partials, &a->partials_cap, sizeof(double) * (size_t)blocks * BAND_W * R * ncomp)) return rc;
    if (int rc = ensure((void **)&a->d_pcounts, &a->pcounts_cap, sizeof(int64_t) * (size_t)blocks * 2)) return rc;
    const size_t lds = sizeof(double) * 4 * (size_t)(R + 8) * BAND_W;
    const BasisParams &bp = a->basis->p;
    double *totals = a->d_totals + ((int64_t)level * a->n_comp + comp) * a->int_width;
    if (int rc = timing_begin(a)) return rc;
    if (pair)
        hipLaunchKernelGGL(k_spline_band_accum<true>, dim3(blocks, ncomp), dim3(256), lds, st, bp, d_f, d_c, d_mask, n, R, a->d_partials, a->d_pcounts);
    else
        hipLaunchKernelGGL(k_spline_band_accum<false>, dim3(blocks, ncomp), dim3(256), lds, st, bp, d_f, d_c, d_mask, n, R, a->d_partials, a->d_pcounts);
    MLMC_HIP_CHECK(hipGetLastError());
    if (int rc = timing_end(a)) return rc;
    a->launches += 1;
    a->alg_bytes += (int64_t)n * (pair ? 16 : 8) * ncomp;
    hipLaunchKernelGGL(k_reduce_band, dim3((BAND_W * R + 15) / 16 + 1, ncomp), dim3(1024), 0, st, a->d_partials, a->d_pcounts, blocks, R, a->RP,
                       totals, a->int_width, count ? a->d_counts + 2 * (int64_t)level : (int64_t *)nullptr, pair ? 0 : 1);
    MLMC_HIP_CHECK(hipGetLastError());
    return 0;
}

static int cov_tiles_per_sample(int T, bool diagonal, bool pair, int gram_mode) {
    const int full = T * T, upper = T * (T + 1) / 2;
    if (!diagonal) return (gram_mode == 0 ? (pair ? 3 : 2) : (gram_mode == 3 ? (pair ? 2 : 1) : 1)) * full;
    if (gram_mode == 0) return pair ? 2 * full + upper : 2 * upper;
    if (gram_mode == 3) return pair ? full + upper : upper;
    if (gram_mode == 1 || !pair) return upper;
    return full;
}

int launch_cov_accum(mlmc_accum *a, int level, int comp, const double *d_f, const double *d_c, const uint8_t *d_mask,
                     int64_t n, bool count, int gram_mode, int ncomp) {
    const bool diff_gram_only = gram_mode == 1;
    if (n == 0) return 0;
    const int R = a->R;
    if (a->basis->p.kind == MLMC_SPLINE && gram_mode == 2 && R <= SPLINE_BAND_MAX_R)
        return launch_spline_band(a, level, comp, d_f, d_c, d_mask, n, count, ncomp);
    if (R > 128) return fail("covariance accumulation in registers covers 128 moments; larger bases go through launch_cov_from_values");
    hipStream_t st = rt().stream;
    const int T = (R <= 16) ? 1 : (R <= 32 ? 2 : 4);
    const int NT = 16 * T, NSL = 4 / T;
    const int NB = (R + 63) / 64;
    const bool pair = d_c != nullptr;
    const int64_t bsz = T == 4 ? (pair ? COV_T4_BATCH : 2 * COV_T4_BATCH) : cov_batch(T, false, false, pair);
    const int64_t n_batches = (n + bsz - 1) / bsz;
    const BasisParams &bp = a->basis->p;
    double *totals0 = a->d_totals + ((int64_t)level * a->n_comp + comp) * a->int_width + (diff_gram_only ? 2 * (int64_t)R : 0);
    for (int bi = 0; bi < NB; ++bi)
        for (int bj = 0; bj < NB; ++bj) {
            if (!pair && bj < bi) continue;
            const bool two_slots = gram_mode == 3 && T == 4 && bi == bj;
            const int NG = gram_mode == 3 ? (two_slots ? 2 : 3) : cov_ng(gram_mode);
            const size_t width = (size_t)NG * NT * NT;
            double *totals = totals0 + (two_slots ? (int64_t)a->RP * a->RP : 0);
            int blocks = rt().n_cu * ((bi != bj) ? ((pair && MLMC_COV_WIDE_BATCH < 64) ? 2 : 1) : (T == 1 ? 4 : (T == 4 ? COV_T4_WGS : 2)));
            if ((n_batches + 3) / 4 < blocks) blocks = (int)((n_batches + 3) / 4);
            const int n_slices = T <= 2 ? 4 : NSL;
            if (int rc = ensure((void **)&a->d_partials, &a->partials_cap, sizeof(double) * (size_t)blocks * n_slices * width * ncomp)) return rc;
            if (int rc = ensure((void **)&a->d_pcounts, &a->pcounts_cap, sizeof(int64_t) * (size_t)blocks * 2)) return rc;
            const bool do_count = count && bi == 0 && bj == 0;
            int64_t *pc = do_count ? a->d_pcounts : nullptr;
            const bool timed = !diff_gram_only;
            if (timed) if (int rc = timing_begin(a)) return rc;
            int rc;
#define MLMC_COV_DISPATCH(KIND)                                                                                               \
    rc = gram_mode == 3 ? launch_cov_kind<KIND, 3>(bp, T, bi, bj, pair, blocks, ncomp, d_f, d_c, d_mask, n, R, a->d_partials, pc) \
       : gram_mode == 2 ? launch_cov_kind<KIND, 2>(bp, T, bi, bj, pair, blocks, ncomp, d_f, d_c, d_mask, n, R, a->d_partials, pc) \
       : diff_gram_only ? launch_cov_kind<KIND, 1>(bp, T, bi, bj, pair, blocks, ncomp, d_f, d_c, d_mask, n, R, a->d_partials, pc) \
                        : launch_cov_kind<KIND, 0>(bp, T, bi, bj, pair, blocks, ncomp, d_f, d_c, d_mask, n, R, a->d_partials, pc)
#define MLMC_COV_DISPATCH012(KIND)                                                                                            \
    rc = gram_mode == 2 ? launch_cov_kind<KIND, 2>(bp, T, bi, bj, pair, blocks, ncomp, d_f, d_c, d_mask, n, R, a->d_partials, pc) \
       : diff_gram_only ? launch_cov_kind<KIND, 1>(bp, T, bi, bj, pair, blocks, ncomp, d_f, d_c, d_mask, n, R, a->d_partials, pc) \
                        : launch_cov_kind<KIND, 0>(bp, T, bi, bj, pair, blocks, ncomp, d_f, d_c, d_mask, n, R, a->d_partials, pc)
            if (gram_mode == 3 && bp.kind != MLMC_LEGENDRE && bp.kind != MLMC_MONOMIAL)
                return fail("covariance: the variance-only pass exists for the polynomial families");
            switch (bp.kind) {
                case MLMC_LEGENDRE: MLMC_COV_DISPATCH(MLMC_LEGENDRE); break;
                case MLMC_MONOMIAL: MLMC_COV_DISPATCH(MLMC_MONOMIAL); break;
                case MLMC_FOURIER: MLMC_COV_DISPATCH012(MLMC_FOURIER); break;
                case MLMC_SPLINE: MLMC_COV_DISPATCH012(MLMC_SPLINE); break;
                default: return fail("covariance: unsupported basis kind");
            }
#undef MLMC_COV_DISPATCH
#undef MLMC_COV_DISPATCH012
            if (rc) return rc;
            if (timed) {
                if (int rc2 = timing_end(a)) return rc2;
                a->launches += 1;
                a->alg_bytes += (int64_t)n * (pair ? 16 : 8) * ncomp;
                a->mfma_flops += (int64_t)512 * cov_tiles_per_sample(T, bi == bj, pair, gram_mode) * n * ncomp;
            }
            hipLaunchKernelGGL(k_reduce_cov, dim3((unsigned)((width + 15) / 16) + (do_count ? 1u : 0u), ncomp), dim3(1024), 0, st, a->d_partials,
                               blocks * n_slices, NT, NG, a->RP, 64 * bi, 64 * bj, totals, a->int_width, (!pair && bi != bj) ? 1 : 0,
                               do_count ? a->d_pcounts : (const int64_t *)nullptr, blocks, a->d_counts + 2 * (int64_t)level);
            MLMC_HIP_CHECK(hipGetLastError());
        }
    return 0;
}

__global__ void k_cov_finalize(const double *__restrict__ totals, const double *__restrict__ scale_c, int R, int RP,
                               int64_t int_width, double *__restrict__ out_s, double *__restrict__ out_sp,
                               const int64_t *__restrict__ counts, int n_levels, int64_t *__restrict__ out_n,
                               double *__restrict__ out_nd, int mean_only, const int64_t *__restrict__ counts2) {
    const int lc = blockIdx.y;
    if (lc == 0 && blockIdx.x == 0)
        for (int l = threadIdx.x; l < n_levels; l += blockDim.x) {
            const int64_t kept = counts[2 * l] + (counts2 ? counts2[2 * l] : 0), removed = counts[2 * l + 1] + (counts2 ? counts2[2 * l + 1] : 0);
            out_n[l] = kept;
            out_n[n_levels + l] = removed;
            out_nd[l] = (double)kept;
            out_nd[n_levels + l] = (double)removed;
        }
    const double *G0 = totals + (int64_t)lc * int_width;
    const double *G1 = G0 + (int64_t)RP * RP;
    const double *G2 = G1 + (int64_t)RP * RP;
    const int idx = blockIdx.x * blockDim.x + threadIdx.x;
    if (idx >= R * R) return;
    const int i = idx / R, j = idx % R;
    const double ci = scale_c ? scale_c[i] : 1.0, cj = scale_c ? scale_c[j] : 1.0;
    const double cc = ci * cj;
    out_s[(int64_t)lc * R * R + idx] = 0.5 * cc * (G0[i * RP + j] + G0[j * RP + i]);
    out_sp[(int64_t)lc * R * R + idx] = mean_only ? __builtin_nan("")
                                                  : 0.25 * (cc * cc) * ((G1[i * RP + j] + G1[j * RP + i]) + 2.0 * G2[i * RP + j]);
}

constexpr int LIN_LC = 8;
__global__ void k_cov_lin_mean(const double *__restrict__ prod, const double *__restrict__ lin_totals, const double *__restrict__ lin_scale,
                               int R, int K, int64_t lin_width, double *__restrict__ out_s, int n_lc, int parity_step, int squares) {
    extern __shared__ double m_s[];
    const int lc0 = blockIdx.y * LIN_LC;
    for (int q = threadIdx.x; q < LIN_LC * K; q += blockDim.x) {
        const int l = q / K, k = q % K;
        m_s[q] = lc0 + l < n_lc ? lin_scale[k] * lin_totals[(int64_t)(lc0 + l) * lin_width + k] : 0.0;
    }
    __syncthreads();
    const int idx = blockIdx.x * blockDim.x + threadIdx.x;
    const int RR = R * R;
    if (idx >= RR) return;
    double acc[LIN_LC];
#pragma unroll
    for (int l = 0; l < LIN_LC; ++l) acc[l] = 0.0;
    const int k0 = (parity_step == 2 && !squares) ? ((idx / R + idx % R) & 1) : 0;
    for (int k = k0; k < K; k += parity_step) {
        const double c = prod[(int64_t)k * RR + idx];
#pragma unroll
        for (int l = 0; l < LIN_LC; ++l) acc[l] = __builtin_fma(c, m_s[l * K + k], acc[l]);
    }
#pragma unroll
    for (int l = 0; l < LIN_LC; ++l)
        if (lc0 + l < n_lc) out_s[(int64_t)(lc0 + l) * RR + idx] += acc[l];
}

int launch_cov_finalize(mlmc_accum *a) {
    if (a->lin && a->lin_used) {
        if (int rc = flush_moments(a->lin)) return rc;
    }
    const bool lin0 = a->lin0 && a->lin0_used;
    if (lin0) {
        if (int rc = flush_moments(a->lin0)) return rc;
    }
    const dim3 lin_grid((a->R * a->R + 255) / 256, (a->n_levels * a->n_comp + LIN_LC - 1) / LIN_LC);
    const int pstep = a->basis->p.kind == MLMC_LEGENDRE ? 2 : 1;
    const int n_lc = a->n_levels * a->n_comp;
    const bool vals = a->cov_from_values;
    const int R = vals ? a->Rout : a->R;
    hipLaunchKernelGGL(k_cov_finalize, dim3((R * R + 255) / 256, n_lc), dim3(256), 0, rt().stream, a->d_totals,
                       vals ? (const double *)nullptr : a->basis->d_scale, R,
                       a->RP, a->int_width, a->d_out_s, a->d_out_sp, a->d_counts, a->n_levels, a->d_out_n, a->d_out_nd,
                       a->mean_only ? 1 : 0, lin0 ? a->lin0->d_counts : (const int64_t *)nullptr);
    MLMC_HIP_CHECK(hipGetLastError());
    if (lin0) {
        hipLaunchKernelGGL(k_cov_lin_mean, lin_grid, dim3(256), sizeof(double) * LIN_LC * a->lin_K, rt().stream,
                           a->d_lin_prod, a->lin0->d_totals, a->lin0_basis->d_scale, R, a->lin_K, a->lin0->int_width, a->d_out_s, n_lc, pstep, 0);
        hipLaunchKernelGGL(k_cov_lin_mean, lin_grid, dim3(256), sizeof(double) * LIN_LC * a->lin0_K, rt().stream,
                           a->d_lin0_prod, a->lin0->d_totals, a->lin0_basis->d_scale, R, a->lin0_K, a->lin0->int_width, a->d_out_sp, n_lc, pstep, 1);
        MLMC_HIP_CHECK(hipGetLastError());
    }
    if (a->lin && a->lin_used) {
        hipLaunchKernelGGL(k_cov_lin_mean, lin_grid, dim3(256), sizeof(double) * LIN_LC * a->lin_K, rt().stream,
                           a->d_lin_prod, a->lin->d_totals, a->lin_basis->d_scale, R, a->lin_K, a->lin->int_width, a->d_out_s, n_lc, pstep, 0);
        MLMC_HIP_CHECK(hipGetLastError());
    }
    return 0;
}

}
```

mlmc_amd/csrc/device_basis.hpp:

```cpp
#pragma once
#include "common.hpp"

namespace mlmc {

__device__ __forceinline__ double transform_value(const BasisParams &bp, double x, bool &keep) {
    if (bp.kind == MLMC_IDENTITY) {
        keep = !(x != x);
        return x;
    }
    if (bp.is_log) {
        const double tl = (log(x) - bp.shift) * bp.scale + bp.ref0;
        if (bp.is_clip)
            keep = (x >= bp.x_lo) && (x <= bp.x_hi);
        else
            keep = (x > 0.0) && (x < __builtin_inf()) && !(tl != tl) && !(fabs(tl) == __builtin_inf());
        return tl;
    }
    double t = (x - bp.shift) * bp.scale + bp.ref0;
    if (bp.is_clip)
        keep = (t >= bp.ref0) && (t <= bp.ref1);
    else
        keep = !(t != t) && !(fabs(t) == __builtin_inf());
    return t;
}

__device__ __forceinline__ double transform_plain(const BasisParams &bp, double x, bool &keep) {
    const double t = (x - bp.shift) * bp.scale + bp.ref0;
    keep = (t >= bp.ref0) && (t <= bp.ref1);
    return t;
}

constexpr int LEGENDRE_MAX_TERMS = 512;
struct LegendreG {
    double v[LEGENDRE_MAX_TERMS];
    constexpr LegendreG() : v() {
        for (int i = 0; i < LEGENDRE_MAX_TERMS; ++i)
            v[i] = i < 2 ? 0.0 : 4.0 * ((double)((long long)(i - 1) * (i - 1)) / (double)((long long)(2 * i - 1) * (2 * i - 3)));
    }
};
__device__ constexpr LegendreG kLegendreG = LegendreG();

template <int KIND>
struct TermGen {
    double x, p1, p2, c1, s1;
    __device__ __forceinline__ void init(double x_, double w, const BasisParams &) {
        x = KIND == MLMC_LEGENDRE ? 2.0 * x_ : x_;
        p1 = w;
        p2 = 0.0;
        if (KIND == MLMC_FOURIER) {
            sincos(x_, &s1, &c1);
            p1 = w;
            p2 = 0.0;
        }
    }
    __device__ __forceinline__ double skip(int j, double g) {
        if (KIND == MLMC_LEGENDRE) {
            const double q = __builtin_fma(x, p1, -(g * p2));
            p2 = p1;
            p1 = q;
            return q;
        } else {
            return next(2 + (j & 1));
        }
    }
    __device__ __forceinline__ double next(int i) {
        if (i == 0) return p1;
        if (KIND == MLMC_LEGENDRE) {
            double q;
            if (i == 1) q = x * p1;
            else q = __builtin_fma(x, p1, -(kLegendreG.v[i] * p2));
            p2 = p1;
            p1 = q;
            return q;
        } else if (KIND == MLMC_MONOMIAL) {
            p1 = p1 * x;
            return p1;
        } else if (KIND == MLMC_FOURIER) {
            if (i & 1) {
                double c = __builtin_fma(p1, c1, -(p2 * s1));
                double s = __builtin_fma(p2, c1, p1 * s1);
                p1 = c;
                p2 = s;
                return c;
            }
            return p2;
        } else {
            return 0.0;
        }
    }
};

template <>
struct TermGen<MLMC_IDENTITY> {
    double v;
    __device__ __forceinline__ void init(double x_, double w, const BasisParams &) { v = x_ * w; }
    __device__ __forceinline__ double next(int) { return v; }
};

template <>
struct TermGen<MLMC_SPLINE> {
    double n0, n1, n2, n3, w;
    int k;
    static __device__ __forceinline__ double knot(int j, int ns, double inv_ns) {
        int c = j - 3;
        c = c < 0 ? 0 : (c > ns ? ns : c);
        return (double)c * inv_ns;
    }
    __device__ __forceinline__ void init(double t, double w_, const BasisParams &bp) {
        w = w_;
        const int ns = bp.size - 3;
        const double inv_ns = 1.0 / (double)ns;
        const double u = (t - bp.ref0) / (bp.ref1 - bp.ref0);
        int s = (int)(u * (double)ns);
        s = s < 0 ? 0 : (s > ns - 1 ? ns - 1 : s);
        k = s;
        if (s >= 2 && s <= ns - 3) {
            const double v = u * (double)ns - (double)s;
            const double v2 = v * v, v3 = v2 * v, om = 1.0 - v;
            constexpr double sixth = 1.0 / 6.0;
            n0 = (om * om * om * sixth) * w;
            n1 = (__builtin_fma(3.0, v3, __builtin_fma(-6.0, v2, 4.0)) * sixth) * w;
            n2 = (__builtin_fma(-3.0, v3, __builtin_fma(3.0, v2, __builtin_fma(3.0, v, 1.0))) * sixth) * w;
            n3 = (v3 * sixth) * w;
            return;
        }
        const int mu = s + 3;
        double N[4], left[4], right[4];
        N[0] = 1.0;
#pragma unroll
        for (int j = 1; j <= 3; ++j) {
            left[j] = u - knot(mu + 1 - j, ns, inv_ns);
            right[j] = knot(mu + j, ns, inv_ns) - u;
            double saved = 0.0;
#pragma unroll
            for (int r = 0; r < j; ++r) {
                const double temp = N[r] / (right[r + 1] + left[j - r]);
                N[r] = saved + right[r + 1] * temp;
                saved = left[j - r] * temp;
            }
            N[j] = saved;
        }
        n0 = N[0] * w; n1 = N[1] * w; n2 = N[2] * w; n3 = N[3] * w;
    }
    __device__ __forceinline__ double next(int i) {
        if (i == 0) return w;
        const int j = i - k;
        return j == 0 ? n0 : (j == 1 ? n1 : (j == 2 ? n2 : (j == 3 ? n3 : 0.0)));
    }
};

__device__ __forceinline__ double wave_sum(double v) {
#pragma unroll
    for (int off = 32; off >= 1; off >>= 1) v += __shfl_xor(v, off, 64);
    return v;
}
__device__ __forceinline__ int wave_sum_i(int v) {
#pragma unroll
    for (int off = 32; off >= 1; off >>= 1) v += __shfl_xor(v, off, 64);
    return v;
}

}
```

mlmc_amd/csrc/moments.hip:

```cpp
#include <cstdlib>
#include <cstring>

#include "device_basis.hpp"

namespace mlmc {

template <int KIND>
__global__ void k_eval(BasisParams bp, const double *__restrict__ scale_c,
                       const double *__restrict__ x, int64_t n, int size, double *__restrict__ out) {
    int64_t i = (int64_t)blockIdx.x * blockDim.x + threadIdx.x;
    if (i >= n) return;
    bool keep;
    double t = transform_value(bp, x[i], keep);
    TermGen<KIND> g;
    g.init(keep ? t : 0.0, 1.0, bp);
    const double nan = __builtin_nan("");
    for (int r = 0; r < size; ++r) {
        double q = g.next(r);
        if (KIND == MLMC_LEGENDRE && scale_c) q *= scale_c[r];
        out[i * size + r] = keep ? q : nan;
    }
}

__global__ void k_apply_matrix(const double *__restrict__ phi, const double *__restrict__ T, int64_t n, int R0, int size,
                               double *__restrict__ out) {
    int64_t idx = (int64_t)blockIdx.x * blockDim.x + threadIdx.x;
    if (idx >= n * size) return;
    int64_t i = idx / size;
    int j = (int)(idx % size);
    double acc = 0.0;
    for (int r = 0; r < R0; ++r) acc = __builtin_fma(phi[i * R0 + r], T[(int64_t)j * R0 + r], acc);
    out[idx] = acc;
}

__global__ __launch_bounds__(256) void k_apply_matrix_mfma(const double *__restrict__ phi, const double *__restrict__ T, int64_t n,
                                                            int R0, int size, double *__restrict__ out) {
    typedef double v4f64 __attribute__((ext_vector_type(4)));
    const int lane = threadIdx.x & 63, wave = threadIdx.x >> 6;
    const int64_t i0 = (int64_t)blockIdx.x * 64 + 16 * wave;
    if (i0 >= n) return;
    const int64_t ia = i0 + (lane & 15) < n ? i0 + (lane & 15) : n - 1;
    const int kq = lane >> 4;
    const double *__restrict__ arow = phi + ia * (int64_t)R0;
    for (int j0 = 0; j0 < size; j0 += 64) {
        v4f64 acc[4];
        const double *brow[4];
        bool bok[4];
#pragma unroll
        for (int t = 0; t < 4; ++t) {
            acc[t] = (v4f64){0.0, 0.0, 0.0, 0.0};
            const int j = j0 + 16 * t + (lane & 15);
            bok[t] = j < size;
            brow[t] = T + (int64_t)(bok[t] ? j : 0) * R0;
        }
        for (int k0 = 0; k0 < R0; k0 += 4) {
            const int k = k0 + kq;
            const bool kin = k < R0;
            const double a = kin ? arow[k] : 0.0;
#pragma unroll
            for (int t = 0; t < 4; ++t) {
                const double b = (kin && bok[t]) ? brow[t][k] : 0.0;
                acc[t] = __builtin_amdgcn_mfma_f64_16x16x4f64(a, b, acc[t], 0, 0, 0);
            }
        }
#pragma unroll
        for (int t = 0; t < 4; ++t) {
            const int j = j0 + 16 * t + (lane & 15);
#pragma unroll
            for (int r = 0; r < 4; ++r) {
                const int64_t i = i0 + (lane >> 4) + 4 * r;
                if (i < n && j < size) out[i * (int64_t)size + j] = acc[t][r];
            }
        }
    }
}

int launch_eval_scaled_base(const mlmc_basis *b, const double *d_x, int64_t n, double *d_out) {
    if (n == 0) return 0;
    hipStream_t st = rt().stream;
    const int threads = 256;
    const int64_t blocks = (n + threads - 1) / threads;
    const BasisParams &bp = b->p;
    const double *no_scale = nullptr;
    switch (bp.kind) {
        case MLMC_LEGENDRE: hipLaunchKernelGGL(k_eval<MLMC_LEGENDRE>, dim3(blocks), dim3(threads), 0, st, bp, no_scale, d_x, n, bp.size, d_out); break;
        case MLMC_MONOMIAL: hipLaunchKernelGGL(k_eval<MLMC_MONOMIAL>, dim3(blocks), dim3(threads), 0, st, bp, no_scale, d_x, n, bp.size, d_out); break;
        case MLMC_FOURIER: hipLaunchKernelGGL(k_eval<MLMC_FOURIER>, dim3(blocks), dim3(threads), 0, st, bp, no_scale, d_x, n, bp.size, d_out); break;
        case MLMC_SPLINE: hipLaunchKernelGGL(k_eval<MLMC_SPLINE>, dim3(blocks), dim3(threads), 0, st, bp, no_scale, d_x, n, bp.size, d_out); break;
        default: return fail("unknown basis kind");
    }
    MLMC_HIP_CHECK(hipGetLastError());
    return 0;
}

int launch_eval(const mlmc_basis *b, const double *d_x, int64_t n, int size, double *d_out, double *scratch) {
    if (n == 0) return 0;
    hipStream_t st = rt().stream;
    int threads = 256;
    int64_t blocks = (n + threads - 1) / threads;
    const BasisParams &bp = b->p;
    double *target = d_out;
    double *d_tmp = nullptr;
    int esize = size;
    if (b->out_size > 0) {
        esize = bp.size;
        if (scratch) d_tmp = scratch;
        else MLMC_HIP_CHECK(hipMalloc(&d_tmp, sizeof(double) * (size_t)n * esize));
        target = d_tmp;
    }
    switch (bp.kind) {
        case MLMC_LEGENDRE: hipLaunchKernelGGL(k_eval<MLMC_LEGENDRE>, dim3(blocks), dim3(threads), 0, st, bp, b->d_scale, d_x, n, esize, target); break;
        case MLMC_MONOMIAL: hipLaunchKernelGGL(k_eval<MLMC_MONOMIAL>, dim3(blocks), dim3(threads), 0, st, bp, b->d_scale, d_x, n, esize, target); break;
        case MLMC_FOURIER: hipLaunchKernelGGL(k_eval<MLMC_FOURIER>, dim3(blocks), dim3(threads), 0, st, bp, b->d_scale, d_x, n, esize, target); break;
        case MLMC_IDENTITY: hipLaunchKernelGGL(k_eval<MLMC_IDENTITY>, dim3(blocks), dim3(threads), 0, st, bp, b->d_scale, d_x, n, esize, target); break;
        case MLMC_SPLINE: hipLaunchKernelGGL(k_eval<MLMC_SPLINE>, dim3(blocks), dim3(threads), 0, st, bp, b->d_scale, d_x, n, esize, target); break;
        default: return fail("unknown basis kind");
    }
    MLMC_HIP_CHECK(hipGetLastError());
    if (b->out_size > 0) {
        int64_t tot = n * size;
        if (n >= 64)
            hipLaunchKernelGGL(k_apply_matrix_mfma, dim3((unsigned)((n + 63) / 64)), dim3(256), 0, st, d_tmp, b->d_matrix, n, bp.size, size, d_out);
        else
            hipLaunchKernelGGL(k_apply_matrix, dim3((tot + 255) / 256), dim3(256), 0, st, d_tmp, b->d_matrix, n, bp.size, size, d_out);
        MLMC_HIP_CHECK(hipGetLastError());
        if (!scratch) {
            MLMC_HIP_CHECK(wait_stream(st));
            MLMC_HIP_CHECK(hipFree(d_tmp));
        }
    }
    return 0;
}

__global__ __launch_bounds__(256) void k_mask(BasisParams bp, const double *__restrict__ f, const double *__restrict__ c, int64_t n,
                                              int n_comp, uint8_t *__restrict__ mask, int64_t *__restrict__ counts) {
    __shared__ int red[4][2];
    int kept = 0, removed = 0;
    for (int64_t i = (int64_t)blockIdx.x * blockDim.x + threadIdx.x; i < n; i += (int64_t)gridDim.x * blockDim.x) {
        bool keep = true;
        for (int m = 0; m < n_comp; ++m) {
            bool k1, k2 = true;
            transform_value(bp, f[(int64_t)m * n + i], k1);
            if (c) transform_value(bp, c[(int64_t)m * n + i], k2);
            keep = keep && k1 && k2;
        }
        mask[i] = keep ? 1 : 0;
        kept += keep;
        removed += !keep;
    }
    kept = wave_sum_i(kept);
    removed = wave_sum_i(removed);
    if ((threadIdx.x & 63) == 0) { red[threadIdx.x >> 6][0] = kept; red[threadIdx.x >> 6][1] = removed; }
    __syncthreads();
    if (threadIdx.x < 2) {
        const int v = red[0][threadIdx.x] + red[1][threadIdx.x] + red[2][threadIdx.x] + red[3][threadIdx.x];
        atomicAdd((unsigned long long *)&counts[threadIdx.x], (unsigned long long)v);
    }
}

int launch_mask(const mlmc_accum *a, const double *d_f, const double *d_c, int64_t n, uint8_t *d_mask, int64_t *d_counts_level) {
    if (n == 0) return 0;
    const int64_t want = (n + 255) / 256;
    hipLaunchKernelGGL(k_mask, dim3((unsigned)(want < 2048 ? want : 2048)), dim3(256), 0, rt().stream, a->basis->p, d_f, d_c, n,
                       a->n_comp, d_mask, d_counts_level);
    MLMC_HIP_CHECK(hipGetLastError());
    return 0;
}

#ifdef MLMC_PROF
__device__ unsigned long long *g_prof;
#endif
constexpr int MAX_SEG = 16;
constexpr int PRIO_SLICE_BITS = 16;
struct Seg {
    const double *fine, *coarse;
    const uint8_t *mask;
    int64_t n;
    int block0, nblocks;
};
struct SegTable {
    int nseg;
    int prio_mod;
    Seg seg[MAX_SEG];
};
struct ReduceTarget {
    double *totals;
    int64_t *counts;
    double *h_s, *h_sp;
    int64_t *h_n;
    double *p_nd;
    double *p_s, *p_sp;
    const double *scale;
    int64_t h_n_stride;
};
struct ReduceTable {
    ReduceTarget t[MAX_SEG];
};

template <int KIND, int RT, bool PAIR, int T0C, bool PLAIN>
__device__ __forceinline__ void accum_samples(const BasisParams &bp, 
                                              const double *__restrict__ fine, const double *__restrict__ coarse,
                                              const uint8_t *__restrict__ mask, int64_t n, int t0, int bid, int nb,
                                              unsigned prio_mod, double (&s)[RT], double (&sp)[RT], int &n_keep, int &n_rm) {
    const int64_t T = (int64_t)nb * ACC_THREADS;
    const int64_t gtid = (int64_t)bid * ACC_THREADS + threadIdx.x;

    int64_t i0 = gtid, i1 = gtid + T;
    double f0 = 0, f1 = 0, c0 = 0, c1 = 0;
    uint8_t m0 = 1, m1 = 1;
    if (i0 < n) { f0 = fine[i0]; if (PAIR) c0 = coarse[i0]; if (!PLAIN && mask) m0 = mask[i0]; }
    if (i1 < n) { f1 = fine[i1]; if (PAIR) c1 = coarse[i1]; if (!PLAIN && mask) m1 = mask[i1]; }

    const unsigned prio_phase = (__builtin_amdgcn_s_getreg((3 << 11) | (0 << 6) | 4) & 15u) % prio_mod;
    unsigned long long prio_clock = __builtin_amdgcn_s_memtime();
    while (i0 < n) {
        if (((unsigned)(prio_clock >> PRIO_SLICE_BITS)) % prio_mod == prio_phase) __builtin_amdgcn_s_setprio(2);
        else __builtin_amdgcn_s_setprio(0);
        prio_clock = __builtin_amdgcn_s_memtime();
        const bool v1 = i1 < n;
        const double xf0 = f0, xf1 = f1, xc0 = c0, xc1 = c1;
        const uint8_t mm0 = m0, mm1 = m1;
        const int64_t j0 = i0 + 2 * T, j1 = i1 + 2 * T;
        if (j0 < n) { f0 = fine[j0]; if (PAIR) c0 = coarse[j0]; if (!PLAIN && mask) m0 = mask[j0]; }
        if (j1 < n) { f1 = fine[j1]; if (PAIR) c1 = coarse[j1]; if (!PLAIN && mask) m1 = mask[j1]; }

        bool kf0, kf1, kc0 = true, kc1 = true;
        const double tf0 = PLAIN ? transform_plain(bp, xf0, kf0) : transform_value(bp, xf0, kf0);
        const double tf1 = PLAIN ? transform_plain(bp, xf1, kf1) : transform_value(bp, xf1, kf1);
        double tc0 = 0, tc1 = 0;
        if (PAIR) {
            tc0 = PLAIN ? transform_plain(bp, xc0, kc0) : transform_value(bp, xc0, kc0);
            tc1 = PLAIN ? transform_plain(bp, xc1, kc1) : transform_value(bp, xc1, kc1);
        }
        const bool k0 = kf0 && kc0 && (PLAIN || mm0 != 0);
        const bool k1 = v1 && kf1 && kc1 && (PLAIN || mm1 != 0);
        n_keep += (int)k0 + (int)k1;
        n_rm += (int)(!k0) + (int)(v1 && !k1);
        const double w0 = k0 ? 1.0 : 0.0, w1 = k1 ? 1.0 : 0.0;

        TermGen<KIND> gf0, gf1, gc0, gc1;
        gf0.init(k0 ? tf0 : 0.0, w0, bp);
        gf1.init(k1 ? tf1 : 0.0, w1, bp);
        if (PAIR) { gc0.init(k0 ? tc0 : 0.0, w0, bp); gc1.init(k1 ? tc1 : 0.0, w1, bp); }

        if constexpr (T0C > 0) {
#pragma unroll
            for (int i = 0; i < T0C; ++i) {
                gf0.next(i); gf1.next(i);
                if (PAIR) { gc0.next(i); gc1.next(i); }
            }
        } else if constexpr (T0C < 0) {
#pragma unroll
            for (int i = 0; i < 128; ++i) {
                gf0.next(i); gf1.next(i);
                if (PAIR) { gc0.next(i); gc1.next(i); }
            }
            for (int b = 128; b < t0; b += 64) {
                double gb[64];
#pragma unroll
                for (int j = 0; j < 64; ++j) gb[j] = KIND == MLMC_LEGENDRE ? kLegendreG.v[b + j] : 0.0;
#pragma unroll
                for (int j = 0; j < 64; ++j) {
                    gf0.skip(j, gb[j]); gf1.skip(j, gb[j]);
                    if (PAIR) { gc0.skip(j, gb[j]); gc1.skip(j, gb[j]); }
                }
            }
        }
        if constexpr (T0C < 0) {
            static_assert(RT % 16 == 0, "run-time term windows use 64-term tiles");
#pragma unroll
            for (int i0 = 0; i0 < RT; i0 += 16) {
                double ga[16];
#pragma unroll
                for (int j = 0; j < 16; ++j) ga[j] = KIND == MLMC_LEGENDRE ? kLegendreG.v[t0 + i0 + j] : 0.0;
#pragma unroll
                for (int j = 0; j < 16; ++j) {
                    const int i = i0 + j;
                    double d0 = gf0.skip(i, ga[j]);
                    double d1 = gf1.skip(i, ga[j]);
                    if (PAIR) { d0 -= gc0.skip(i, ga[j]); d1 -= gc1.skip(i, ga[j]); }
                    s[i] += d0;
                    sp[i] = __builtin_fma(d0, d0, sp[i]);
                    s[i] += d1;
                    sp[i] = __builtin_fma(d1, d1, sp[i]);
                }
            }
        } else {
#pragma unroll
        for (int i = 0; i < RT; ++i) {
            double d0 = gf0.next(t0 + i);
            double d1 = gf1.next(t0 + i);
            if (PAIR) { d0 -= gc0.next(t0 + i); d1 -= gc1.next(t0 + i); }
            s[i] += d0;
            sp[i] = __builtin_fma(d0, d0, sp[i]);
            s[i] += d1;
            sp[i] = __builtin_fma(d1, d1, sp[i]);
        }
        }
        i0 = j0;
        i1 = j1;
    }
}

template <int KIND, int RT, bool PAIR>
__device__ __forceinline__ void accum_samples_wide(const BasisParams &bp, const double *__restrict__ fine,
                                                   const double *__restrict__ coarse, int64_t n, int bid, int nb,
                                                   double (&s)[RT], double (&sp)[RT], int &n_keep, int &n_rm) {
    constexpr int S = 4;
    const int64_t T = (int64_t)nb * ACC_THREADS;
    int64_t i = (int64_t)bid * ACC_THREADS + threadIdx.x;
    double f[S], c[S];
#pragma unroll
    for (int k = 0; k < S; ++k) {
        const int64_t ik = i + k * T;
        f[k] = 0.0;
        c[k] = 0.0;
        if (ik < n) { f[k] = fine[ik]; if (PAIR) c[k] = coarse[ik]; }
    }
    while (i < n) {
        double xf[S], xc[S];
        bool valid[S];
#pragma unroll
        for (int k = 0; k < S; ++k) { xf[k] = f[k]; xc[k] = c[k]; valid[k] = i + k * T < n; }
        const int64_t j = i + S * T;
#pragma unroll
        for (int k = 0; k < S; ++k) {
            const int64_t jk = j + k * T;
            if (jk < n) { f[k] = fine[jk]; if (PAIR) c[k] = coarse[jk]; }
        }
        TermGen<KIND> gf[S], gc[S];
#pragma unroll
        for (int k = 0; k < S; ++k) {
            bool kf, kc = true;
            const double tf = transform_plain(bp, xf[k], kf);
            const double tc = PAIR ? transform_plain(bp, xc[k], kc) : 0.0;
            const bool keep = valid[k] && kf && kc;
            n_keep += (int)keep;
            n_rm += (int)(valid[k] && !keep);
            const double w = keep ? 1.0 : 0.0;
            gf[k].init(keep ? tf : 0.0, w, bp);
            if (PAIR) gc[k].init(keep ? tc : 0.0, w, bp);
        }
#pragma unroll
        for (int t = 0; t < RT; ++t) {
#pragma unroll
            for (int k = 0; k < S; ++k) {
                double d = gf[k].next(t);
                if (PAIR) d -= gc[k].next(t);
                s[t] += d;
                sp[t] = __builtin_fma(d, d, sp[t]);
            }
        }
        i = j;
    }
}

template <int KIND, int RT, int T0C, bool PLAIN>
__global__ __launch_bounds__(ACC_THREADS) void k_moments_accum(BasisParams bp, SegTable tab,
                                                              int t0_arg, double *__restrict__ partials,
                                                              int64_t *__restrict__ pcounts) {
    const int t0 = T0C >= 0 ? T0C : t0_arg;
    Seg sg = tab.seg[0];
#pragma unroll
    for (int k = 1; k < MAX_SEG; ++k)
        if (k < tab.nseg && (int)blockIdx.x >= tab.seg[k].block0) sg = tab.seg[k];
    const int bid = (int)blockIdx.x - sg.block0;
#ifdef MLMC_PROF
    const unsigned long long prof_r0 = __builtin_amdgcn_s_memrealtime(), prof_c0 = __builtin_amdgcn_s_memtime();
#endif

    double s[RT], sp[RT];
#pragma unroll
    for (int i = 0; i < RT; ++i) { s[i] = 0.0; sp[i] = 0.0; }
    int n_keep = 0, n_rm = 0;
    const unsigned prio_mod = tab.prio_mod > 0 ? (unsigned)tab.prio_mod : 1u;
    constexpr bool WIDE = RT <= 16 && T0C == 0;
    if (PLAIN && WIDE) {
        if (sg.coarse) accum_samples_wide<KIND, RT, true>(bp, sg.fine, sg.coarse, sg.n, bid, sg.nblocks, s, sp, n_keep, n_rm);
        else accum_samples_wide<KIND, RT, false>(bp, sg.fine, sg.coarse, sg.n, bid, sg.nblocks, s, sp, n_keep, n_rm);
    } else if (sg.coarse) {
        accum_samples<KIND, RT, true, T0C, PLAIN>(bp, sg.fine, sg.coarse, sg.mask, sg.n, t0, bid, sg.nblocks, prio_mod, s, sp, n_keep, n_rm);
    } else {
        accum_samples<KIND, RT, false, T0C, PLAIN>(bp, sg.fine, sg.coarse, sg.mask, sg.n, t0, bid, sg.nblocks, prio_mod, s, sp, n_keep, n_rm);
    }
#ifdef MLMC_PROF
    const unsigned long long prof_r1 = __builtin_amdgcn_s_memrealtime(), prof_c1 = __builtin_amdgcn_s_memtime();
#endif
    __shared__ double red[2 * RT][WAVE + 1];
    __shared__ int ldc[4][2];
    const int lane = threadIdx.x & 63, wave = threadIdx.x >> 6;
    for (int w = 0; w < 4; ++w) {
        if (wave == w) {
            if (w == 0) {
#pragma unroll
                for (int i = 0; i < RT; ++i) { red[i][lane] = s[i]; red[RT + i][lane] = sp[i]; }
            } else {
#pragma unroll
                for (int i = 0; i < RT; ++i) { red[i][lane] += s[i]; red[RT + i][lane] += sp[i]; }
            }
        }
        __syncthreads();
    }
    n_keep = wave_sum_i(n_keep);
    n_rm = wave_sum_i(n_rm);
    if (lane == 0) { ldc[wave][0] = n_keep; ldc[wave][1] = n_rm; }
    __syncthreads();
    for (int j = threadIdx.x; j < 2 * RT; j += ACC_THREADS) {
        double v = 0.0;
#pragma unroll 8
        for (int l = 0; l < WAVE; ++l) v += red[j][l];
        partials[(int64_t)blockIdx.x * (2 * RT) + j] = v;
    }
    if (threadIdx.x < 2) {
        int v = ldc[0][threadIdx.x] + ldc[1][threadIdx.x] + ldc[2][threadIdx.x] + ldc[3][threadIdx.x];
        pcounts[(int64_t)blockIdx.x * 2 + threadIdx.x] = v;
    }
#ifdef MLMC_PROF
    if ((threadIdx.x & 63) == 0) {
        unsigned long long *p = g_prof + ((size_t)blockIdx.x * 4 + (threadIdx.x >> 6)) * 5;
        p[0] = prof_r0; p[1] = prof_r1; p[2] = __builtin_amdgcn_s_memrealtime(); p[3] = prof_c1 - prof_c0;
        p[4] = (unsigned long long)__builtin_amdgcn_s_getreg((4 << 0) | (0 << 6) | (31 << 11)) |
               ((unsigned long long)__builtin_amdgcn_s_getreg((20 << 0) | (0 << 6) | (31 << 11)) << 32);
    }
#endif
}

constexpr int SPLIT_LANES = 128;
#ifndef MLMC_SPLIT_HEAD
#define MLMC_SPLIT_HEAD 30
#endif
constexpr int SPLIT_HEAD = MLMC_SPLIT_HEAD;
__host__ __device__ constexpr int split_max(int ht, int tt) { return ht > tt ? ht : tt; }
#ifndef MLMC_SPLIT_WPS
#define MLMC_SPLIT_WPS 2
#endif
#ifdef MLMC_SPLIT_NO_PRIO
#define MLMC_SPLIT_PRIO_INIT
#define MLMC_SPLIT_PRIO_TRIP
#else
#ifndef MLMC_SPLIT_PRIO_BITS
#define MLMC_SPLIT_PRIO_BITS 16
#endif
#define MLMC_SPLIT_PRIO_INIT                                                                                              \
    const unsigned prio_phase = (__builtin_amdgcn_s_getreg((3 << 11) | (0 << 6) | 4) & 15u) % MLMC_SPLIT_WPS;  \
    unsigned long long prio_clock = __builtin_amdgcn_s_memtime();
#define MLMC_SPLIT_PRIO_TRIP                                                                                              \
    if ((((unsigned)(prio_clock >> MLMC_SPLIT_PRIO_BITS)) % MLMC_SPLIT_WPS) == prio_phase) __builtin_amdgcn_s_setprio(2); \
    else __builtin_amdgcn_s_setprio(0);                                                                                   \
    prio_clock = __builtin_amdgcn_s_memtime();
#endif

template <int KIND>
__device__ __forceinline__ void split_export(const TermGen<KIND> &g, double *__restrict__ slot) {
    slot[0 * SPLIT_LANES] = g.x;
    slot[1 * SPLIT_LANES] = g.p1;
    if (KIND == MLMC_LEGENDRE) slot[2 * SPLIT_LANES] = g.p2;
}
template <int KIND>
__device__ __forceinline__ void split_import(TermGen<KIND> &g, const double *__restrict__ slot) {
    g.x = slot[0 * SPLIT_LANES];
    g.p1 = slot[1 * SPLIT_LANES];
    g.p2 = KIND == MLMC_LEGENDRE ? slot[2 * SPLIT_LANES] : 0.0;
    g.c1 = g.s1 = 0.0;
}

#ifndef MLMC_SPLIT_NS
#define MLMC_SPLIT_NS 2
#endif
template <int KIND, bool PAIR, bool PLAIN, int HT, int TT, bool SQ, int NS, int T0 = 0>
__device__ __forceinline__ void split_head(const BasisParams &bp, const double *__restrict__ fine, const double *__restrict__ coarse,
                                           const uint8_t *__restrict__ mask, int64_t n, int bid, int nb, int n_trips,
                                           double *__restrict__ hand, double (&s)[split_max(HT, TT)], double (&sp)[split_max(HT, TT)],
                                           int &n_keep, int &n_rm) {
    const int64_t T = (int64_t)nb * SPLIT_LANES;
    const int l128 = threadIdx.x & (SPLIT_LANES - 1);
    int64_t idx[NS];
    double f[NS], c[NS];
    uint8_t m[NS];
#pragma unroll
    for (int q = 0; q < NS; ++q) {
        idx[q] = (int64_t)bid * SPLIT_LANES + l128 + q * T;
        const int64_t j = idx[q] < n ? idx[q] : n - 1;
        f[q] = fine[j];
        c[q] = PAIR ? coarse[j] : 0.0;
        m[q] = (!PLAIN && mask) ? mask[j] : (uint8_t)1;
    }
    MLMC_SPLIT_PRIO_INIT
    for (int k = 0; k < n_trips; ++k) {
        MLMC_SPLIT_PRIO_TRIP
        bool valid[NS];
        double xf[NS], xc[NS];
        uint8_t mm[NS];
#pragma unroll
        for (int q = 0; q < NS; ++q) {
            valid[q] = idx[q] < n;
            xf[q] = f[q]; xc[q] = c[q]; mm[q] = m[q];
            idx[q] += (int64_t)NS * T;
            const int64_t j = idx[q] < n ? idx[q] : n - 1;
            f[q] = fine[j];
            if (PAIR) c[q] = coarse[j];
            if (!PLAIN && mask) m[q] = mask[j];
        }
        TermGen<KIND> gf[NS], gc[NS];
#pragma unroll
        for (int q = 0; q < NS; ++q) {
            bool kf, kc = true;
            const double tf = PLAIN ? transform_plain(bp, xf[q], kf) : transform_value(bp, xf[q], kf);
            double tc = 0;
            if (PAIR) tc = PLAIN ? transform_plain(bp, xc[q], kc) : transform_value(bp, xc[q], kc);
            const bool keep = valid[q] && kf && kc && (PLAIN || mm[q] != 0);
            n_keep += (int)keep;
            n_rm += (int)(valid[q] && !keep);
            const double w = keep ? 1.0 : 0.0;
            gf[q].init(keep ? tf : 0.0, w, bp);
            if (PAIR) gc[q].init(keep ? tc : 0.0, w, bp);
        }
        if (T0 > 0) {
#pragma unroll
            for (int i = 0; i < T0; ++i) {
#pragma unroll
                for (int q = 0; q < NS; ++q) {
                    gf[q].next(i);
                    if (PAIR) gc[q].next(i);
                }
            }
        }
#pragma unroll
        for (int i = 0; i < HT; ++i) {
#pragma unroll
            for (int q = 0; q < NS; ++q) {
                double d = gf[q].next(T0 + i);
                if (PAIR) d -= gc[q].next(T0 + i);
                s[i] += d;
                if (SQ) sp[i] = __builtin_fma(d, d, sp[i]);
            }
        }
        double *__restrict__ slot = hand + (size_t)(k & 1) * (6 * NS * SPLIT_LANES) + l128;
#pragma unroll
        for (int q = 0; q < NS; ++q) {
            split_export<KIND>(gf[q], slot + (3 * q) * SPLIT_LANES);
            if (PAIR) split_export<KIND>(gc[q], slot + (3 * (NS + q)) * SPLIT_LANES);
        }
        __syncthreads();
    }
    __syncthreads();
}

template <int KIND, bool PAIR, int HT, int TT, bool SQ, int NS, int T0 = 0>
__device__ __forceinline__ void split_tail(const BasisParams &bp, int n_trips, const double *__restrict__ hand,
                                           double (&s)[split_max(HT, TT)], double (&sp)[split_max(HT, TT)]) {
    const int l128 = threadIdx.x & (SPLIT_LANES - 1);
    __syncthreads();
    MLMC_SPLIT_PRIO_INIT
    for (int k = 0; k < n_trips; ++k) {
        MLMC_SPLIT_PRIO_TRIP
        const double *__restrict__ slot = hand + (size_t)(k & 1) * (6 * NS * SPLIT_LANES) + l128;
        TermGen<KIND> gf[NS], gc[NS];
#pragma unroll
        for (int q = 0; q < NS; ++q) {
            split_import<KIND>(gf[q], slot + (3 * q) * SPLIT_LANES);
            if (PAIR) split_import<KIND>(gc[q], slot + (3 * (NS + q)) * SPLIT_LANES);
        }
#pragma unroll
        for (int i = 0; i < TT; ++i) {
#pragma unroll
            for (int q = 0; q < NS; ++q) {
                double d = gf[q].next(T0 + HT + i);
                if (PAIR) d -= gc[q].next(T0 + HT + i);
                s[i] += d;
                if (SQ) sp[i] = __builtin_fma(d, d, sp[i]);
            }
        }
        __syncthreads();
    }
}

template <int KIND, bool PLAIN, int HT, int TT, int WPS, bool SQ = true, int NS = MLMC_SPLIT_NS, int T0 = 0>
__global__ __launch_bounds__(ACC_THREADS, WPS) void k_moments_accum_split(BasisParams bp, SegTable tab,
                                                                        double *__restrict__ partials,
                                                                        int64_t *__restrict__ pcounts) {
    __shared__ double hand[2 * 6 * NS * SPLIT_LANES];
    constexpr int MAXT = split_max(HT, TT), NTOT = HT + TT;
    __shared__ double wsum[4][2 * MAXT];
    __shared__ int ldc[2][2];
    Seg sg = tab.seg[0];
#pragma unroll
    for (int k = 1; k < MAX_SEG; ++k)
        if (k < tab.nseg && (int)blockIdx.x >= tab.seg[k].block0) sg = tab.seg[k];
    const int bid = (int)blockIdx.x - sg.block0;
    const int lane = threadIdx.x & 63;
    const int wave = __builtin_amdgcn_readfirstlane((int)(threadIdx.x >> 6));
    const int64_t T2 = NS * (int64_t)sg.nblocks * SPLIT_LANES;
    const int64_t first = (int64_t)bid * SPLIT_LANES;
    const int n_trips = first < sg.n ? (int)((sg.n - first + T2 - 1) / T2) : 0;

    double s[MAXT], sp[MAXT];
#pragma unroll
    for (int i = 0; i < MAXT; ++i) { s[i] = 0.0; sp[i] = 0.0; }
    int n_keep = 0, n_rm = 0;
    if (wave < 2) {
        if (sg.coarse) split_head<KIND, true, PLAIN, HT, TT, SQ, NS, T0>(bp, sg.fine, sg.coarse, sg.mask, sg.n, bid, sg.nblocks, n_trips, hand, s, sp, n_keep, n_rm);
        else split_head<KIND, false, PLAIN, HT, TT, SQ, NS, T0>(bp, sg.fine, sg.coarse, sg.mask, sg.n, bid, sg.nblocks, n_trips, hand, s, sp, n_keep, n_rm);
    } else {
        if (sg.coarse) split_tail<KIND, true, HT, TT, SQ, NS, T0>(bp, n_trips, hand, s, sp);
        else split_tail<KIND, false, HT, TT, SQ, NS, T0>(bp, n_trips, hand, s, sp);
    }
#pragma unroll
    for (int i = 0; i < MAXT; ++i) {
        const double a = wave_sum(s[i]), b = SQ ? wave_sum(sp[i]) : __builtin_nan("");
        if (lane == 0) { wsum[wave][i] = a; wsum[wave][MAXT + i] = b; }
    }
    n_keep = wave_sum_i(n_keep);
    n_rm = wave_sum_i(n_rm);
    if (lane == 0 && wave < 2) { ldc[wave][0] = n_keep; ldc[wave][1] = n_rm; }
    __syncthreads();
    if (threadIdx.x < 2 * NTOT) {
        const int which = threadIdx.x / NTOT, term = threadIdx.x % NTOT;
        const int half = term < HT ? 0 : 1, i = half ? term - HT : term;
        partials[(int64_t)blockIdx.x * (2 * NTOT) + threadIdx.x] = wsum[2 * half][which * MAXT + i] + wsum[2 * half + 1][which * MAXT + i];
    }
    if (threadIdx.x < 2) pcounts[(int64_t)blockIdx.x * 2 + threadIdx.x] = ldc[0][threadIdx.x] + ldc[1][threadIdx.x];
}

__global__ __launch_bounds__(1024) void k_reduce_partials(const double *__restrict__ partials,
                                                         const int64_t *__restrict__ pcounts, SegTable tab, ReduceTable rtab,
                                                         int width, int RT, int t0, int int_R) {
    __shared__ double lds[16][64];
    Seg sg = tab.seg[0];
    ReduceTarget tg = rtab.t[0];
#pragma unroll
    for (int k = 1; k < MAX_SEG; ++k)
        if ((int)blockIdx.x == k) { sg = tab.seg[k]; tg = rtab.t[k]; }
    const int row0 = sg.block0, nblocks = sg.nblocks;
    const int c = threadIdx.x & 63, g = threadIdx.x >> 6;
    for (int c0 = 0; c0 < width; c0 += 64) {
        const int col = c0 + c;
        double acc = 0.0;
        if (col < width) {
            const double *__restrict__ pc = partials + (int64_t)row0 * width + col;
#pragma unroll 8
            for (int b = g; b < nblocks; b += 16) acc += pc[(int64_t)b * width];
        }
        __syncthreads();
        lds[g][c] = acc;
        __syncthreads();
        if (g == 0 && col < width) {
            double v = 0.0;
#pragma unroll
            for (int k = 0; k < 16; ++k) v += lds[k][c];
            const int which = col / RT, term = t0 + col % RT;
            if (term < int_R) {
                const double t = tg.totals[(int64_t)which * int_R + term] + v;
                tg.totals[(int64_t)which * int_R + term] = t;
                if (tg.h_s) {
                    const double c = tg.scale[term];
                    if (which == 0) tg.h_s[term] = c * t;
                    else tg.h_sp[term] = (c * c) * t;
                    if (tg.p_s) {
                        if (which == 0) tg.p_s[term] = c * t;
                        else tg.p_sp[term] = (c * c) * t;
                    }
                }
            }
        }
    }
    if (tg.counts && g == 15) {
        int64_t a = 0, b = 0;
        for (int i = c; i < nblocks; i += 64) { a += pcounts[2 * (int64_t)(row0 + i)]; b += pcounts[2 * (int64_t)(row0 + i) + 1]; }
        for (int off = 32; off >= 1; off >>= 1) { a += __shfl_xor(a, off, 64); b += __shfl_xor(b, off, 64); }
        if (c == 0) {
            a += tg.counts[0];
            b += tg.counts[1];
            tg.counts[0] = a;
            tg.counts[1] = b;
            if (tg.h_n) { tg.h_n[0] = a; tg.h_n[tg.h_n_stride] = b; }
            if (tg.p_nd) { tg.p_nd[0] = (double)a; tg.p_nd[tg.h_n_stride] = (double)b; }
        }
    }
}

constexpr int SPLINE_MAX_R = 512;

template <bool NEED_SQ>
__global__ __launch_bounds__(ACC_THREADS) void k_spline_accum(BasisParams bp, SegTable tab, int R, double *__restrict__ partials,
                                                             int64_t *__restrict__ pcounts) {
    extern __shared__ double sacc[];
    __shared__ int ldc[4][2];
    const int RP = R + 8;
    Seg sg = tab.seg[0];
#pragma unroll
    for (int k = 1; k < MAX_SEG; ++k)
        if (k < tab.nseg && (int)blockIdx.x >= tab.seg[k].block0) sg = tab.seg[k];
    const int bid = (int)blockIdx.x - sg.block0;
    const int lane = threadIdx.x & 63, wave = threadIdx.x >> 6;
    for (int i = threadIdx.x; i < 4 * 2 * RP; i += ACC_THREADS) sacc[i] = 0.0;
    __syncthreads();
    double *__restrict__ ws = sacc + (size_t)wave * 2 * RP;
    double *__restrict__ wsp = ws + RP;
    const bool pair = sg.coarse != nullptr;
    int n_keep = 0, n_rm = 0;
    const int64_t T = (int64_t)sg.nblocks * ACC_THREADS;
    for (int64_t i = (int64_t)bid * ACC_THREADS + threadIdx.x; i < sg.n; i += T) {
        bool kf, kc = true;
        const double tf = transform_value(bp, sg.fine[i], kf);
        double tc = 0.0;
        if (pair) tc = transform_value(bp, sg.coarse[i], kc);
        const bool keep = kf && kc && (!sg.mask || sg.mask[i] != 0);
        n_keep += (int)keep;
        n_rm += (int)!keep;
        if (!keep) continue;
        TermGen<MLMC_SPLINE> gf, gc;
        gf.init(tf, 1.0, bp);
        const double nf[4] = {gf.n0, gf.n1, gf.n2, gf.n3};
        if (!pair) {
#pragma unroll
            for (int j = 0; j < 4; ++j) {
                const int r = gf.k + j;
                if (r > 0) { atomicAdd(&ws[r], nf[j]); if (NEED_SQ) atomicAdd(&wsp[r], nf[j] * nf[j]); }
            }
            continue;
        }
        gc.init(tc, 1.0, bp);
        const double nc[4] = {gc.n0, gc.n1, gc.n2, gc.n3};
        const int delta = gc.k - gf.k;
        if (delta == 0) {
#pragma unroll
            for (int j = 0; j < 4; ++j) {
                const int r = gf.k + j;
                const double d = nf[j] - nc[j];
                if (r > 0) { atomicAdd(&ws[r], d); if (NEED_SQ) atomicAdd(&wsp[r], d * d); }
            }
        } else {
#pragma unroll
            for (int j = 0; j < 4; ++j) {
                const int r = gf.k + j, jc = j - delta;
                const double c = jc == 0 ? nc[0] : (jc == 1 ? nc[1] : (jc == 2 ? nc[2] : (jc == 3 ? nc[3] : 0.0)));
                const double d = nf[j] - c;
                if (r > 0) { atomicAdd(&ws[r], d); if (NEED_SQ) atomicAdd(&wsp[r], d * d); }
            }
#pragma unroll
            for (int j = 0; j < 4; ++j) {
                const int r = gc.k + j, jf = j + delta;
                if ((jf < 0 || jf > 3) && r > 0) { atomicAdd(&ws[r], -nc[j]); if (NEED_SQ) atomicAdd(&wsp[r], nc[j] * nc[j]); }
            }
        }
    }
    n_keep = wave_sum_i(n_keep);
    n_rm = wave_sum_i(n_rm);
    if (lane == 0) { ldc[wave][0] = n_keep; ldc[wave][1] = n_rm; }
    __syncthreads();
    const int keep_block = ldc[0][0] + ldc[1][0] + ldc[2][0] + ldc[3][0];
    for (int j = threadIdx.x; j < 2 * R; j += ACC_THREADS) {
        const int which = j / R, r = j % R;
        const int o = which * RP + r;
        double v = ((sacc[o] + sacc[2 * RP + o]) + sacc[4 * RP + o]) + sacc[6 * RP + o];
        if (r == 0) v = pair ? 0.0 : (double)keep_block;
        partials[(int64_t)blockIdx.x * (2 * R) + j] = v;
    }
    if (threadIdx.x < 2) {
        int v = ldc[0][threadIdx.x] + ldc[1][threadIdx.x] + ldc[2][threadIdx.x] + ldc[3][threadIdx.x];
        pcounts[(int64_t)blockIdx.x * 2 + threadIdx.x] = v;
    }
}

template <int KIND, int RT, int T0C, bool PLAIN>
static int launch_accum_rt(const BasisParams &bp, const SegTable &tab, int total_blocks, int t0,
                           double *partials, int64_t *pcounts) {
    hipLaunchKernelGGL((k_moments_accum<KIND, RT, T0C, PLAIN>), dim3(total_blocks), dim3(ACC_THREADS), 0, rt().stream, bp, tab, t0, partials,
                       pcounts);
    MLMC_HIP_CHECK(hipGetLastError());
    return 0;
}

template <int KIND, int RT, int T0C, bool PLAIN>
static int occupancy_rt(int *per_cu) {
    MLMC_HIP_CHECK(hipOccupancyMaxActiveBlocksPerMultiprocessor(per_cu, (const void *)k_moments_accum<KIND, RT, T0C, PLAIN>, ACC_THREADS, 0));
    return 0;
}

static int pick_rt(int kind, int n_terms, int t0) {
    if (kind == MLMC_IDENTITY) return 4;
    if (t0 == 32) return n_terms <= 16 ? 16 : 32;
    if (t0 == 64) return n_terms <= 16 ? 16 : (n_terms <= 32 ? 32 : (n_terms <= 48 ? 48 : 64));
    if (t0 > 0) return 64;
    if (kind == MLMC_LEGENDRE) {
        const int opts[] = {4, 6, 8, 10, 12, 16, 20, 24, 28, 32, 40, 48, 56, 64};
        for (int o : opts)
            if (n_terms <= o) return o;
        return 64;
    }
    const int opts[] = {8, 16, 24, 32, 48, 64};
    for (int o : opts)
        if (n_terms <= o) return o;
    return 64;
}

static int accum_dispatch(int op, bool plain, const BasisParams &bp, int rt_sel, const SegTable *tab, int total_blocks,
                          int t0, double *partials, int64_t *pcounts, int *out) {
#define MLMC_RT_GO1(KIND, N, T0C, P) \
    (op == 0 ? occupancy_rt<KIND, N, T0C, P>(out) : launch_accum_rt<KIND, N, T0C, P>(bp, *tab, total_blocks, t0, partials, pcounts))
#define MLMC_RT_GO(KIND, N, T0C) (plain ? MLMC_RT_GO1(KIND, N, T0C, true) : MLMC_RT_GO1(KIND, N, T0C, false))
#define MLMC_RT_CASE(KIND, N) case N: return MLMC_RT_GO(KIND, N, 0)
#define MLMC_RT_LATER(KIND)                                                                                  \
    if (t0 == 32) return rt_sel == 16 ? MLMC_RT_GO(KIND, 16, 32) : MLMC_RT_GO(KIND, 32, 32);                 \
    if (t0 == 64) {                                                                                          \
        switch (rt_sel) {                                                                                    \
            case 16: return MLMC_RT_GO(KIND, 16, 64);                                                        \
            case 32: return MLMC_RT_GO(KIND, 32, 64);                                                        \
            case 48: return MLMC_RT_GO(KIND, 48, 64);                                                        \
            default: return MLMC_RT_GO(KIND, 64, 64);                                                        \
        }                                                                                                    \
    }                                                                                                        \
    return MLMC_RT_GO(KIND, 64, -1)
    if (t0 > 0) {
        switch (bp.kind) {
            case MLMC_LEGENDRE: MLMC_RT_LATER(MLMC_LEGENDRE);
            case MLMC_MONOMIAL: MLMC_RT_LATER(MLMC_MONOMIAL);
            case MLMC_FOURIER: MLMC_RT_LATER(MLMC_FOURIER);
            default: return fail("moments: a later pass needs a polynomial / Fourier basis");
        }
    }
    switch (bp.kind) {
        case MLMC_LEGENDRE:
            switch (rt_sel) {
                MLMC_RT_CASE(MLMC_LEGENDRE, 4); MLMC_RT_CASE(MLMC_LEGENDRE, 6); MLMC_RT_CASE(MLMC_LEGENDRE, 8);
                MLMC_RT_CASE(MLMC_LEGENDRE, 10); MLMC_RT_CASE(MLMC_LEGENDRE, 12);
                MLMC_RT_CASE(MLMC_LEGENDRE, 16); MLMC_RT_CASE(MLMC_LEGENDRE, 20); MLMC_RT_CASE(MLMC_LEGENDRE, 24);
                MLMC_RT_CASE(MLMC_LEGENDRE, 28); MLMC_RT_CASE(MLMC_LEGENDRE, 32); MLMC_RT_CASE(MLMC_LEGENDRE, 40);
                MLMC_RT_CASE(MLMC_LEGENDRE, 48); MLMC_RT_CASE(MLMC_LEGENDRE, 56);
                default: return MLMC_RT_GO(MLMC_LEGENDRE, 64, 0);
            }
        case MLMC_MONOMIAL:
            switch (rt_sel) {
                MLMC_RT_CASE(MLMC_MONOMIAL, 8); MLMC_RT_CASE(MLMC_MONOMIAL, 16); MLMC_RT_CASE(MLMC_MONOMIAL, 24);
                MLMC_RT_CASE(MLMC_MONOMIAL, 32); MLMC_RT_CASE(MLMC_MONOMIAL, 48);
                default: return MLMC_RT_GO(MLMC_MONOMIAL, 64, 0);
            }
        case MLMC_FOURIER:
            switch (rt_sel) {
                MLMC_RT_CASE(MLMC_FOURIER, 8); MLMC_RT_CASE(MLMC_FOURIER, 16); MLMC_RT_CASE(MLMC_FOURIER, 24);
                MLMC_RT_CASE(MLMC_FOURIER, 32); MLMC_RT_CASE(MLMC_FOURIER, 48);
                default: return MLMC_RT_GO(MLMC_FOURIER, 64, 0);
            }
        case MLMC_IDENTITY: return MLMC_RT_GO1(MLMC_IDENTITY, 4, 0, false);
        default: return fail("unknown basis kind");
    }
#undef MLMC_RT_LATER
#undef MLMC_RT_CASE
#undef MLMC_RT_GO
#undef MLMC_RT_GO1
}

template <int KIND, bool PLAIN, int HT, int TT, int WPS, bool SQ, int T0 = 0>
static int split_go(int op, const BasisParams &bp, const SegTable *tab, int total_blocks, double *partials, int64_t *pcounts, int *out) {
    if (op == 0) {
        MLMC_HIP_CHECK(hipOccupancyMaxActiveBlocksPerMultiprocessor(out, (const void *)k_moments_accum_split<KIND, PLAIN, HT, TT, WPS, SQ, MLMC_SPLIT_NS, T0>, ACC_THREADS, 0));
        return 0;
    }
    hipLaunchKernelGGL((k_moments_accum_split<KIND, PLAIN, HT, TT, WPS, SQ, MLMC_SPLIT_NS, T0>), dim3(total_blocks), dim3(ACC_THREADS), 0, rt().stream, bp, *tab, partials, pcounts);
    MLMC_HIP_CHECK(hipGetLastError());
    return 0;
}
constexpr int SPLIT_MEAN_HEAD_96 = 46, SPLIT_MEAN_HEAD_128 = 62;
constexpr int SPLIT_MEAN_HEAD_W2 = 40;
static int split_dispatch(int op, bool plain, const BasisParams &bp, int n_split, int t0, const SegTable *tab, int total_blocks, double *partials,
                          int64_t *pcounts, int *out) {
#define MLMC_SPLIT_GO(KIND, P)                                                                                                          \
    (t0 == 128 ? split_go<KIND, P, SPLIT_MEAN_HEAD_W2, 128 - SPLIT_MEAN_HEAD_W2, 2, false, 128>(op, bp, tab, total_blocks, partials, pcounts, out) \
     : n_split == 64 ? split_go<KIND, P, SPLIT_HEAD, 64 - SPLIT_HEAD, MLMC_SPLIT_WPS, true>(op, bp, tab, total_blocks, partials, pcounts, out)   \
     : n_split == 96 ? split_go<KIND, P, SPLIT_MEAN_HEAD_96, 96 - SPLIT_MEAN_HEAD_96, 2, false>(op, bp, tab, total_blocks, partials, pcounts, out) \
                     : split_go<KIND, P, SPLIT_MEAN_HEAD_128, 128 - SPLIT_MEAN_HEAD_128, 2, false>(op, bp, tab, total_blocks, partials, pcounts, out))
    if (bp.kind == MLMC_LEGENDRE) return plain ? MLMC_SPLIT_GO(MLMC_LEGENDRE, true) : MLMC_SPLIT_GO(MLMC_LEGENDRE, false);
    return plain ? MLMC_SPLIT_GO(MLMC_MONOMIAL, true) : MLMC_SPLIT_GO(MLMC_MONOMIAL, false);
#undef MLMC_SPLIT_GO
}

int flush_moments(mlmc_accum *a) {
    const int nseg = (int)a->pending.size();
    if (nseg == 0) return 0;
    hipStream_t st = rt().stream;
    const int R = a->R;
    const BasisParams &bp = a->basis->p;
    const bool sparse_spline = bp.kind == MLMC_SPLINE;
    if (sparse_spline && R > SPLINE_MAX_R) return fail("spline moments: at most 512 basis functions");
    static const bool no_split = std::getenv("MLMC_HIP_NO_SPLIT") != nullptr;
    const bool poly = bp.kind == MLMC_LEGENDRE || bp.kind == MLMC_MONOMIAL;
    const bool poly64 = poly && R > 48 && R <= 64;
    const bool split_mean = poly && a->mean_only_plain && R > 64 && R <= 256 && !no_split;
    const bool split = (poly64 && !no_split) || split_mean;
    const int pass_terms = split_mean ? 128 : ((poly64 && !split) ? 32 : MAX_TERMS_PER_PASS);
    for (int t0 = 0; t0 < (sparse_spline ? 1 : R); t0 += pass_terms) {
        const int n_terms = (R - t0 < pass_terms) ? R - t0 : pass_terms;
        const int n_split = split_mean ? ((t0 == 0 && R <= 96) ? 96 : 128) : 64;
        const int rt_sel = sparse_spline ? R : (split ? n_split : pick_rt(bp.kind, n_terms, t0));
        const int width = 2 * rt_sel;
        int per_cu = 4;
        bool plain = bp.kind != MLMC_IDENTITY && !bp.is_log && bp.is_clip;
        for (const PendingSeg &p : a->pending) plain = plain && p.mask == nullptr;
        if (split) {
            static int occ_split[2][2][4];
            int &cached = occ_split[bp.kind == MLMC_LEGENDRE ? 0 : 1][plain ? 1 : 0][t0 ? 3 : (n_split == 64 ? 0 : (n_split == 96 ? 1 : 2))];
            if (cached == 0)
                if (int rc = split_dispatch(0, plain, bp, n_split, t0, nullptr, 0, nullptr, nullptr, &cached)) return rc;
            per_cu = cached;
        } else if (!sparse_spline) {
            static int occ_cache[8][4][2][65];
            int &cached = occ_cache[bp.kind & 7][t0 == 0 ? 0 : (t0 == 64 ? 1 : (t0 == 32 ? 2 : 3))][plain ? 1 : 0][rt_sel];
            if (cached == 0)
                if (int rc = accum_dispatch(0, plain, bp, rt_sel, nullptr, 0, t0, nullptr, nullptr, &cached)) return rc;
            per_cu = cached;
        }
        if (per_cu < 1) per_cu = 1;
        if (per_cu > 8) per_cu = 8;
        const int resident = rt().n_cu * per_cu;
        constexpr double W_PAIR = 7.0, W_SINGLE = 4.3;
        double wsum = 0.0;
        for (const PendingSeg &p : a->pending) wsum += (double)p.n * (p.coarse ? W_PAIR : W_SINGLE);
        SegTable tab;
        ReduceTable rtab;
        std::memset(&tab, 0, sizeof(tab));
        std::memset(&rtab, 0, sizeof(rtab));
        tab.nseg = nseg;
        tab.prio_mod = per_cu < 1 ? 1 : (per_cu > 8 ? 8 : per_cu);
        int total = 0;
        int64_t bytes = 0;
        for (int k = 0; k < nseg; ++k) {
            const PendingSeg &p = a->pending[k];
            int nb = (int)((double)resident * ((double)p.n * (p.coarse ? W_PAIR : W_SINGLE)) / wsum);
            const int64_t per_trip = split ? (int64_t)MLMC_SPLIT_NS * SPLIT_LANES : 2 * ACC_THREADS;
            const int64_t want = (p.n + per_trip - 1) / per_trip;
            if (nb > want) nb = (int)want;
            if (nb < 1) nb = 1;
            tab.seg[k].fine = p.fine;
            tab.seg[k].coarse = p.coarse;
            tab.seg[k].mask = p.mask;
            tab.seg[k].n = p.n;
            tab.seg[k].block0 = total;
            tab.seg[k].nblocks = nb;
            total += nb;
            rtab.t[k].totals = a->d_totals + ((int64_t)p.level * a->n_comp + p.comp) * a->int_width;
            rtab.t[k].counts = (p.count && t0 == 0) ? a->d_counts + (int64_t)p.level * 2 : nullptr;
            if (a->host_outputs) {
                rtab.t[k].h_s = a->h_out_s + (int64_t)p.level * R;
                rtab.t[k].h_sp = a->h_out_sp + (int64_t)p.level * R;
                rtab.t[k].h_n = a->h_out_n + p.level;
                rtab.t[k].h_n_stride = a->n_levels;
                if (a->packed_target) {
                    double *pk = a->packed_target;
                    rtab.t[k].p_nd = pk + p.level;
                    rtab.t[k].p_s = pk + 2 * (int64_t)a->n_levels + (int64_t)p.level * R;
                    rtab.t[k].p_sp = rtab.t[k].p_s + (int64_t)a->n_levels * R;
                }
                rtab.t[k].scale = a->basis->d_scale;
                a->level_flushed[p.level] = 1;
            }
            bytes += p.n * (p.coarse ? 16 : 8);
        }
        if (int rc = ensure((void **)&a->d_partials, &a->partials_cap, sizeof(double) * (size_t)total * width)) return rc;
        if (int rc = ensure((void **)&a->d_pcounts, &a->pcounts_cap, sizeof(int64_t) * (size_t)total * 2)) return rc;
        if (int rc = timing_begin(a)) return rc;
        if (sparse_spline) {
            const size_t lds = sizeof(double) * 4 * 2 * (size_t)(R + 8);
            if (a->mean_only)
                hipLaunchKernelGGL(k_spline_accum<false>, dim3(total), dim3(ACC_THREADS), lds, st, bp, tab, R, a->d_partials, a->d_pcounts);
            else
                hipLaunchKernelGGL(k_spline_accum<true>, dim3(total), dim3(ACC_THREADS), lds, st, bp, tab, R, a->d_partials, a->d_pcounts);
            MLMC_HIP_CHECK(hipGetLastError());
        } else if (split) {
            if (int rc = split_dispatch(1, plain, bp, n_split, t0, &tab, total, a->d_partials, a->d_pcounts, nullptr)) return rc;
        } else if (int rc = accum_dispatch(1, plain, bp, rt_sel, &tab, total, t0, a->d_partials, a->d_pcounts, nullptr)) {
            return rc;
        }
        if (int rc = timing_end(a)) return rc;
        a->launches += 1;
        a->alg_bytes += bytes;
        hipLaunchKernelGGL(k_reduce_partials, dim3(nseg), dim3(1024), 0, st, a->d_partials, a->d_pcounts, tab, rtab, width, rt_sel, t0, R);
        MLMC_HIP_CHECK(hipGetLastError());
    }
    a->pending.clear();
    return 0;
}

int launch_moments_accum(mlmc_accum *a, int level, int comp, const double *d_f, const double *d_c, const uint8_t *d_mask,
                         int64_t n, bool count, bool defer) {
    if (n == 0) return 0;
    for (const PendingSeg &p : a->pending)
        if (p.level == level && p.comp == comp) {
            if (int rc = flush_moments(a)) return rc;
            break;
        }
    if ((int)a->pending.size() >= MAX_SEG)
        if (int rc = flush_moments(a)) return rc;
    a->pending.push_back(PendingSeg{d_f, d_c, d_mask, n, level, comp, count});
    if (!defer) return flush_moments(a);
    return 0;
}

__global__ void k_moments_finalize(const double *__restrict__ totals, const double *__restrict__ scale_c,
                                   const double *__restrict__ T, int R, int RP, int Rout, int has_T, int64_t int_width,
                                   int n_lc, double *__restrict__ out_s, double *__restrict__ out_sp,
                                   const int64_t *__restrict__ counts, int n_levels, int64_t *__restrict__ out_n,
                               double *__restrict__ out_nd, int mean_only) {
    const int lc = blockIdx.x;
    if (lc >= n_lc) return;
    if (lc == 0)
        for (int l = threadIdx.x; l < n_levels; l += blockDim.x) {
            out_n[l] = counts[2 * l];
            out_n[n_levels + l] = counts[2 * l + 1];
            out_nd[l] = (double)counts[2 * l];
            out_nd[n_levels + l] = (double)counts[2 * l + 1];
        }
    const double *tot = totals + (int64_t)lc * int_width;
    for (int j = threadIdx.x; j < Rout; j += blockDim.x) {
        double s, sp;
        if (!has_T) {
            const double c = scale_c[j];
            s = c * tot[j];
            sp = (c * c) * tot[R + j];
        } else {
            const double *G = tot + 2 * R;
            s = 0.0;
            sp = 0.0;
            for (int i = 0; i < R; ++i) {
                const double ti = T[(int64_t)j * R + i] * scale_c[i];
                s = __builtin_fma(ti, tot[i], s);
                if (mean_only) continue;
                double row = 0.0;
                for (int k = 0; k < R; ++k) row = __builtin_fma(T[(int64_t)j * R + k] * scale_c[k], G[(int64_t)i * RP + k], row);
                sp = __builtin_fma(ti, row, sp);
            }
            if (mean_only) sp = __builtin_nan("");
        }
        out_s[(int64_t)lc * Rout + j] = s;
        out_sp[(int64_t)lc * Rout + j] = sp;
    }
}

int launch_moments_finalize(mlmc_accum *a) {
    const int n_lc = a->n_levels * a->n_comp;
    hipLaunchKernelGGL(k_moments_finalize, dim3(n_lc), dim3(128), 0, rt().stream, a->d_totals, a->basis->d_scale,
                       a->basis->d_matrix, a->R, a->RP, a->Rout, a->basis->out_size > 0 ? 1 : 0, a->int_width, n_lc,
                       a->d_out_s, a->d_out_sp, a->d_counts, a->n_levels, a->d_out_n, a->d_out_nd, a->mean_only ? 1 : 0);
    MLMC_HIP_CHECK(hipGetLastError());
    return 0;
}

}
```

Baseline: 294.4 billion.

## Accumulate linearized Legendre moments as Chebyshev sums with composed product tables

When Legendre moments are linearized into a larger inner basis (K > 64), the inner accumulator now sums Chebyshev polynomials. Their recurrence is a single FMA with no per-term coefficient load, and it can jump straight to T128 by doubling, which avoids stepping through the first 128 terms on the second pass. The Legendre product tables are recomputed in long double and composed with a Legendre-to-Chebyshev conversion matrix so the final moments stay the same. The lin-mean reduction kernel is also batched into multi-row jobs per level class, and occupancy for the Chebyshev split kernel is capped at 2 per CU. The change risks precision loss from the basis change and relies on new split-head constants.

```diff
diff --git a/mlmc_amd/csrc/api.hip b/mlmc_amd/csrc/api.hip
--- a/mlmc_amd/csrc/api.hip
+++ b/mlmc_amd/csrc/api.hip
@@ -6,6 +6,7 @@
 #include "common.hpp"
 #include <algorithm>
 #include <map>
+#include <tuple>
 
 namespace mlmc {
 
@@ -112,16 +113,14 @@
     *x_hi = as_double(last);
 }
 
-bool product_table(int kind, int R, std::vector<double> &out) {
-    if (kind != MLMC_LEGENDRE && kind != MLMC_MONOMIAL) return false;
+typedef long double ld;
+static void legendre_products_ld(int R, std::vector<ld> &out) {
     const int K = 2 * R - 1;
     const size_t RR = (size_t)R * R;
-    out.assign((size_t)K * RR, 0.0);
+    out.assign((size_t)K * RR, 0.0L);
     for (int i = 0; i < R; ++i)
         for (int j = 0; j < R; ++j) {
             const size_t ij = (size_t)i * R + j;
-            if (kind == MLMC_MONOMIAL) { out[(size_t)(i + j) * RR + ij] = 1.0; continue; }
-            typedef long double ld;
             const int hi = i > j ? i : j, lo = i > j ? j : i;
             const ld diff = (ld)(hi - lo);
             ld c = (2 * diff + 1) / (2 * (ld)hi + 1);
@@ -131,7 +130,7 @@
             }
             for (int t = 0; t <= lo; ++t) {
                 const int k = (hi - lo) + 2 * t;
-                out[(size_t)k * RR + ij] = (double)c;
+                out[(size_t)k * RR + ij] = c;
                 if (t == lo) break;
                 const ld s = (ld)hi + t, kk = (ld)k;
                 const ld si = s - hi, sj = s - lo, sk = s - kk;
@@ -142,20 +141,28 @@
                 c = c * ratio;
             }
         }
-    return true;
-}
-
-bool square_product_table(int kind, int R, std::vector<double> &out) {
+}
+
+bool product_table(int kind, int R, std::vector<double> &out) {
     if (kind != MLMC_LEGENDRE && kind != MLMC_MONOMIAL) return false;
-    const int K = 4 * R - 3;
+    const int K = 2 * R - 1;
     const size_t RR = (size_t)R * R;
     out.assign((size_t)K * RR, 0.0);
     if (kind == MLMC_MONOMIAL) {
         for (int i = 0; i < R; ++i)
-            for (int j = 0; j < R; ++j) out[(size_t)(2 * (i + j)) * RR + (size_t)i * R + j] = 1.0;
+            for (int j = 0; j < R; ++j) out[(size_t)(i + j) * RR + (size_t)i * R + j] = 1.0;
         return true;
     }
-    typedef long double ld;
+    std::vector<ld> c;
+    legendre_products_ld(R, c);
+    for (size_t q = 0; q < c.size(); ++q) out[q] = (double)c[q];
+    return true;
+}
+
+static void legendre_square_products_ld(int R, std::vector<ld> &out) {
+    const int K = 4 * R - 3;
+    const size_t RR = (size_t)R * R;
+    out.assign((size_t)K * RR, 0.0L);
     const int Q = 4 * R;
     const ld pi = 3.14159265358979323846264338327950288L;
     std::vector<ld> x(Q), w(Q), P((size_t)K * Q);
@@ -205,24 +212,88 @@
                 ld acc = 0.0L;
                 const ld *Pk = &P[(size_t)k * Q];
                 for (int q = 0; q < Q; ++q) acc += sq[q] * Pk[q];
-                const double c = (double)(acc * (2 * k + 1) / 2);
+                const ld c = acc * (2 * k + 1) / 2;
                 out[(size_t)k * RR + (size_t)i * R + j] = c;
                 out[(size_t)k * RR + (size_t)j * R + i] = c;
             }
         }
-    std::vector<double> t1;
-    product_table(kind, R, t1);
+    std::vector<ld> t1;
+    legendre_products_ld(R, t1);
     for (int j = 0; j < R; ++j)
         for (int k = 0; k < K; ++k) {
-            const double c = k < 2 * R - 1 ? t1[(size_t)k * RR + (size_t)j * R + j] : 0.0;
+            const ld c = k < 2 * R - 1 ? t1[(size_t)k * RR + (size_t)j * R + j] : 0.0L;
             out[(size_t)k * RR + (size_t)j] = c;
             out[(size_t)k * RR + (size_t)j * R] = c;
         }
+}
+
+bool square_product_table(int kind, int R, std::vector<double> &out) {
+    if (kind != MLMC_LEGENDRE && kind != MLMC_MONOMIAL) return false;
+    const int K = 4 * R - 3;
+    const size_t RR = (size_t)R * R;
+    out.assign((size_t)K * RR, 0.0);
+    if (kind == MLMC_MONOMIAL) {
+        for (int i = 0; i < R; ++i)
+            for (int j = 0; j < R; ++j) out[(size_t)(2 * (i + j)) * RR + (size_t)i * R + j] = 1.0;
+        return true;
+    }
+    std::vector<ld> c;
+    legendre_square_products_ld(R, c);
+    for (size_t q = 0; q < c.size(); ++q) out[q] = (double)c[q];
+    return true;
+}
+
+static void chebyshev_compose(const std::vector<ld> &c, int K, int R, std::vector<double> &out) {
+    const size_t RR = (size_t)R * R;
+    std::vector<ld> g(K), at((size_t)K * K, 0.0L), col(K);
+    g[0] = 1.0L;
+    for (int j = 1; j < K; ++j) g[j] = g[j - 1] * (ld)(2 * j - 1) / (ld)(2 * j);
+    for (int k = 0; k < K; ++k)
+        for (int j = 0; j <= k; ++j) at[(size_t)(k - 2 * j < 0 ? 2 * j - k : k - 2 * j) * K + k] += g[j] * g[k - j];
+    out.assign((size_t)K * RR, 0.0);
+    for (int i = 0; i < R; ++i)
+        for (int j = i; j < R; ++j) {
+            const size_t ij = (size_t)i * R + j, ji = (size_t)j * R + i;
+            for (int k = 0; k < K; ++k) col[k] = c[(size_t)k * RR + ij];
+            for (int m = 0; m < K; ++m) {
+                ld acc = 0.0L;
+                for (int k = m; k < K; k += 2) acc += col[k] * at[(size_t)m * K + k];
+                out[(size_t)m * RR + ij] = out[(size_t)m * RR + ji] = (double)acc;
+            }
+        }
+}
+
+bool product_table_chebyshev(int R, std::vector<double> &out) {
+    std::vector<ld> c;
+    legendre_products_ld(R, c);
+    chebyshev_compose(c, 2 * R - 1, R, out);
+    return true;
+}
+
+bool square_product_table_chebyshev(int R, std::vector<double> &out) {
+    std::vector<ld> c;
+    legendre_square_products_ld(R, c);
+    const int K = 4 * R - 3;
+    chebyshev_compose(c, K, R, out);
+    std::vector<double> t1;
+    product_table_chebyshev(R, t1);
+    const size_t RR = (size_t)R * R;
+    for (int j = 0; j < R; ++j)
+        for (int m = 0; m < K; ++m) {
+            const double v = m < 2 * R - 1 ? t1[(size_t)m * RR + (size_t)j * R + j] : 0.0;
+            out[(size_t)m * RR + (size_t)j] = v;
+            out[(size_t)m * RR + (size_t)j * R] = v;
+        }
     return true;
 }
 
 static bool linearize_enabled() {
     const char *e = std::getenv("MLMC_HIP_LINEARIZE");
+    return !(e && e[0] == '0');
+}
+
+static bool linearize_chebyshev_enabled() {
+    const char *e = std::getenv("MLMC_HIP_LINEARIZE_CHEB");
     return !(e && e[0] == '0');
 }
 
@@ -426,56 +497,66 @@
 struct LinTables {
     double *d_prod = nullptr, *d_prod2 = nullptr;
 };
-static int lin_tables(int kind, int R, bool squares, LinTables **out) {
-    static std::map<std::pair<int, int>, LinTables> cache;
-    LinTables &t = cache[std::make_pair(kind, R)];
+static int lin_tables(int kind, int R, bool cheb, bool squares, LinTables **out) {
+    static std::map<std::tuple<int, int, int>, LinTables> cache;
+    LinTables &t = cache[std::make_tuple(cheb ? 1 : 0, kind, R)];
     if (!t.d_prod) {
         std::vector<double> h;
-        product_table(kind, R, h);
+        if (cheb) product_table_chebyshev(R, h);
+        else product_table(kind, R, h);
         MLMC_HIP_CHECK(hipMalloc(&t.d_prod, sizeof(double) * h.size()));
         MLMC_HIP_CHECK(hipMemcpy(t.d_prod, h.data(), sizeof(double) * h.size(), hipMemcpyHostToDevice));
     }
     if (squares && !t.d_prod2) {
         std::vector<double> h;
-        square_product_table(kind, R, h);
+        if (cheb) square_product_table_chebyshev(R, h);
+        else square_product_table(kind, R, h);
         MLMC_HIP_CHECK(hipMalloc(&t.d_prod2, sizeof(double) * h.size()));
         MLMC_HIP_CHECK(hipMemcpy(t.d_prod2, h.data(), sizeof(double) * h.size(), hipMemcpyHostToDevice));
     }
     *out = &t;
+    return 0;
+}
+
+static int inner_basis_create(const mlmc_basis *b, int size, bool cheb, mlmc_basis **out) {
+    mlmc_basis_desc d;
+    std::memset(&d, 0, sizeof(d));
+    d.kind = cheb ? (int)MLMC_MONOMIAL : b->p.kind;
+    d.size = size;
+    d.shift = b->p.shift; d.scale = b->p.scale; d.ref0 = b->p.ref0; d.ref1 = b->p.ref1;
+    d.is_log = b->p.is_log; d.is_clip = b->p.is_clip;
+    d.x_lo = b->p.x_lo; d.x_hi = b->p.x_hi;
+    if (int rc = mlmc_basis_create(&d, out)) return rc;
+    (*out)->p.x_lo = b->p.x_lo;
+    (*out)->p.x_hi = b->p.x_hi;
+    if (cheb) (*out)->p.kind = KIND_CHEBYSHEV;
     return 0;
 }
 
 static int ensure_lin(mlmc_accum *a) {
     if (a->lin) return 0;
     const mlmc_basis *b = a->basis;
-    LinTables *t = nullptr;
-    if (int rc = lin_tables(b->p.kind, a->R, a->lin0_eligible, &t)) return rc;
-    mlmc_basis_desc d;
-    std::memset(&d, 0, sizeof(d));
-    d.kind = b->p.kind;
-    d.size = 2 * a->R - 1;
-    d.shift = b->p.shift; d.scale = b->p.scale; d.ref0 = b->p.ref0; d.ref1 = b->p.ref1;
-    d.is_log = b->p.is_log; d.is_clip = b->p.is_clip;
-    d.x_lo = b->p.x_lo; d.x_hi = b->p.x_hi;
-    int rc = mlmc_basis_create(&d, &a->lin_basis);
+    const int K1 = 2 * a->R - 1, K2 = 4 * a->R - 3;
+    const bool cheb1 = a->lin_cheb && K1 > 64, cheb2 = a->lin_cheb && K2 > 64;
+    LinTables *t1 = nullptr, *t2 = nullptr;
+    if (int rc = lin_tables(b->p.kind, a->R, cheb1, false, &t1)) return rc;
+    if (a->lin0_eligible)
+        if (int rc = lin_tables(b->p.kind, a->R, cheb2, true, &t2)) return rc;
+    int rc = inner_basis_create(b, K1, cheb1, &a->lin_basis);
     if (!rc) rc = mlmc_accum_create(a->lin_basis, a->n_levels, MLMC_MODE_MOMENTS | MLMC_MODE_MEAN_ONLY, a->n_comp, &a->lin);
     if (!rc) {
-        a->lin_basis->p.x_lo = b->p.x_lo;
-        a->lin_basis->p.x_hi = b->p.x_hi;
         a->lin->host_outputs = false;
-        a->lin_K = d.size;
-        a->d_lin_prod = t->d_prod;
+        a->lin_K = K1;
+        a->d_lin_prod = t1->d_prod;
     }
     if (!rc && a->lin0_eligible) {
-        d.size = 4 * a->R - 3;
-        rc = mlmc_basis_create(&d, &a->lin0_basis);
+        rc = inner_basis_create(b, K2, cheb2, &a->lin0_basis);
         if (!rc) rc = mlmc_accum_create(a->lin0_basis, a->n_levels, MLMC_MODE_MOMENTS | MLMC_MODE_MEAN_ONLY, a->n_comp, &a->lin0);
         if (!rc) {
-            a->lin0_basis->p.x_lo = b->p.x_lo;
-            a->lin0_basis->p.x_hi = b->p.x_hi;
             a->lin0->host_outputs = false;
-            a->lin0_K = d.size;
-            a->d_lin0_prod = t->d_prod2;
+            a->lin0_K = K2;
+            a->d_lin0_prod1 = t2->d_prod;
+            a->d_lin0_prod = t2->d_prod2;
         }
     }
     if (rc) {
@@ -507,7 +588,8 @@
     a->cov_from_values = mode == MLMC_MODE_COV && (b->out_size > 0 || (b->p.size > 128 && !spline_band));
     a->mean_only = mean_only && ((mode == MLMC_MODE_COV && !a->cov_from_values) || (mode == MLMC_MODE_MOMENTS && b->out_size > 0));
     a->mean_only_plain = mean_only && mode == MLMC_MODE_MOMENTS && b->out_size == 0 &&
-                         (b->p.kind == MLMC_LEGENDRE || b->p.kind == MLMC_MONOMIAL) && b->p.size > 64 && b->p.size <= 256;
+                         (b->p.kind == MLMC_LEGENDRE || b->p.kind == MLMC_MONOMIAL || b->p.kind == KIND_CHEBYSHEV) && b->p.size > 64 &&
+                         b->p.size <= 256;
     a->n_comp = n_comp;
     a->R = b->p.size;
     a->Rout = b->out_size > 0 ? b->out_size : b->p.size;
@@ -552,6 +634,7 @@
         a->lin_min_n = min_n ? std::atoll(min_n) : (a->R > 32 ? 100000 : 1500000);
         const char *lin0_env = std::getenv("MLMC_HIP_LINEARIZE_LEVEL0");
         a->lin0_eligible = a->R <= 64 && !(lin0_env && lin0_env[0] == '0');
+        a->lin_cheb = b->p.kind == MLMC_LEGENDRE && linearize_chebyshev_enabled() && std::getenv("MLMC_HIP_NO_SPLIT") == nullptr;
     }
     *out = a;
     return mlmc_accum_reset(a);
@@ -570,6 +653,8 @@
         a->xcov_pushes = 0;
     }
     a->lin_used = a->lin0_used = false;
+    a->lin_levels.assign(a->n_levels, 0);
+    a->lin0_levels.assign(a->n_levels, 0);
     if (a->lin0)
         if (int rc = mlmc_accum_reset(a->lin0)) return rc;
     if (a->lin) return mlmc_accum_reset(a->lin);
@@ -714,6 +799,7 @@
             const bool use_lin0 = a->lin0 && !d_c && n >= a->lin_min_n;
             if (use_lin0) {
                 a->lin0_used = true;
+                a->lin0_levels[level] = 1;
                 rc = launch_moments_accum(a->lin0, level, m, f_m, nullptr, d_mask, n, count_in_kernel && m == 0,
                                           mem_kind == MLMC_DEVICE || a->n_comp > 1);
                 if (rc) return rc;
@@ -721,7 +807,7 @@
             }
             const bool use_lin = a->lin && n >= a->lin_min_n;
             rc = m == 0 ? launch_cov_accum(a, level, 0, d_f, d_c, d_mask, n, count_in_kernel, a->mean_only ? 2 : (use_lin ? 3 : 0), a->n_comp) : 0;
-            if (!rc && use_lin) a->lin_used = true;
+            if (!rc && use_lin) { a->lin_used = true; a->lin_levels[level] = 1; }
             if (!rc && use_lin)
                 rc = launch_moments_accum(a->lin, level, m, f_m, c_m, d_mask, n, false, mem_kind == MLMC_DEVICE || a->n_comp > 1);
         }
@@ -865,12 +951,21 @@
 int mlmc_linearization_table(int32_t kind, int32_t R, int32_t squares, double *out, int64_t out_len) {
     if (!out) return fail("mlmc_linearization_table: null argument");
     if (kind != MLMC_LEGENDRE && kind != MLMC_MONOMIAL) return fail("mlmc_linearization_table: Legendre or monomial moments");
-    if (R < 1 || R > (squares ? 64 : 128)) return fail("mlmc_linearization_table: size out of range");
-    const int64_t K = squares ? 4 * (int64_t)R - 3 : 2 * (int64_t)R - 1;
+    if (squares < 0 || squares > 3) return fail("mlmc_linearization_table: squares is 0 .. 3");
+    const bool cheb = squares >= 2, sq = squares == 1 || squares == 3;
+    if (cheb && kind != MLMC_LEGENDRE) return fail("mlmc_linearization_table: the tables for Chebyshev sums belong to Legendre moments");
+    if (R < 1 || R > (sq ? 64 : 128)) return fail("mlmc_linearization_table: size out of range");
+    const int64_t K = sq ? 4 * (int64_t)R - 3 : 2 * (int64_t)R - 1;
     if (out_len < K * R * R) return fail("mlmc_linearization_table: output too small");
     std::vector<double> t;
-    if (squares) square_product_table(kind, R, t);
-    else product_table(kind, R, t);
+    if (cheb) {
+        if (sq) square_product_table_chebyshev(R, t);
+        else product_table_chebyshev(R, t);
+    } else if (sq) {
+        square_product_table(kind, R, t);
+    } else {
+        product_table(kind, R, t);
+    }
     std::memcpy(out, t.data(), sizeof(double) * t.size());
     return 0;
 }
diff --git a/mlmc_amd/csrc/common.hpp b/mlmc_amd/csrc/common.hpp
--- a/mlmc_amd/csrc/common.hpp
+++ b/mlmc_amd/csrc/common.hpp
@@ -15,6 +15,10 @@
 #define MLMC_TERMS_PER_PASS 64
 #endif
 constexpr int MAX_TERMS_PER_PASS = MLMC_TERMS_PER_PASS;
+constexpr int KIND_CHEBYSHEV = 16;
+static_assert(KIND_CHEBYSHEV > MLMC_SPLINE && KIND_CHEBYSHEV > MLMC_IDENTITY && KIND_CHEBYSHEV > MLMC_FOURIER && KIND_CHEBYSHEV > MLMC_MONOMIAL &&
+                  KIND_CHEBYSHEV > MLMC_LEGENDRE && KIND_CHEBYSHEV > 7,
+              "KIND_CHEBYSHEV must not collide with a public basis kind of mlmc_hip.h");
 constexpr int SPLINE_BAND_MAX_R = 256;
 
 void set_error(const std::string &msg);
@@ -127,6 +131,9 @@
     mlmc_accum *lin0 = nullptr;
     mlmc_basis *lin0_basis = nullptr;
     double *d_lin0_prod = nullptr;
+    double *d_lin0_prod1 = nullptr;
+    bool lin_cheb = false;
+    std::vector<char> lin_levels, lin0_levels;
     int lin0_K = 0;
     bool lin0_used = false;
     int64_t lin_min_n = 0;
@@ -155,6 +162,8 @@
 int launch_xcov_finalize(mlmc_accum *a);
 bool product_table(int kind, int R, std::vector<double> &out);
 bool square_product_table(int kind, int R, std::vector<double> &out);
+bool product_table_chebyshev(int R, std::vector<double> &out);
+bool square_product_table_chebyshev(int R, std::vector<double> &out);
 int launch_cov_from_values(mlmc_accum *a, int level, int comp, const double *d_vf, const double *d_vc, const uint8_t *d_mask,
                            int64_t n, bool count, int gram_mode = 0);
 int ensure(void **p, size_t *cap, size_t bytes);
diff --git a/mlmc_amd/csrc/cov.hip b/mlmc_amd/csrc/cov.hip
--- a/mlmc_amd/csrc/cov.hip
+++ b/mlmc_amd/csrc/cov.hip
@@ -1,3 +1,5 @@
+#include <cstring>
+
 #include "device_basis.hpp"
 
 namespace mlmc {
@@ -1069,30 +1071,53 @@
 }
 
 constexpr int LIN_LC = 8;
-__global__ void k_cov_lin_mean(const double *__restrict__ prod, const double *__restrict__ lin_totals, const double *__restrict__ lin_scale,
-                               int R, int K, int64_t lin_width, double *__restrict__ out_s, int n_lc, int parity_step, int squares) {
+constexpr int LIN_MAX_JOBS = 12;
+struct LinSrc {
+    const double *prod;
+    const double *totals;
+    const double *scale;
+    int64_t width;
+    int K, squares;
+};
+struct LinJob {
+    double *out;
+    int n_rows;
+    int row[LIN_LC];
+    LinSrc src[2];
+};
+struct LinJobs {
+    LinJob job[LIN_MAX_JOBS];
+};
+__global__ void k_cov_lin_mean(LinJobs jobs, int R, int parity_step) {
     extern __shared__ double m_s[];
-    const int lc0 = blockIdx.y * LIN_LC;
-    for (int q = threadIdx.x; q < LIN_LC * K; q += blockDim.x) {
-        const int l = q / K, k = q % K;
-        m_s[q] = lc0 + l < n_lc ? lin_scale[k] * lin_totals[(int64_t)(lc0 + l) * lin_width + k] : 0.0;
-    }
-    __syncthreads();
+    const LinJob &jb = jobs.job[blockIdx.y];
     const int idx = blockIdx.x * blockDim.x + threadIdx.x;
     const int RR = R * R;
-    if (idx >= RR) return;
-    double acc[LIN_LC];
-#pragma unroll
-    for (int l = 0; l < LIN_LC; ++l) acc[l] = 0.0;
-    const int k0 = (parity_step == 2 && !squares) ? ((idx / R + idx % R) & 1) : 0;
-    for (int k = k0; k < K; k += parity_step) {
-        const double c = prod[(int64_t)k * RR + idx];
-#pragma unroll
-        for (int l = 0; l < LIN_LC; ++l) acc[l] = __builtin_fma(c, m_s[l * K + k], acc[l]);
-    }
-#pragma unroll
-    for (int l = 0; l < LIN_LC; ++l)
-        if (lc0 + l < n_lc) out_s[(int64_t)(lc0 + l) * RR + idx] += acc[l];
+    for (int e = 0; e < 2; ++e) {
+        const LinSrc &sr = jb.src[e];
+        if (!sr.prod) continue;
+        const int K = sr.K;
+        __syncthreads();
+        for (int q = threadIdx.x; q < LIN_LC * K; q += blockDim.x) {
+            const int l = q / K, k = q % K;
+            m_s[q] = l < jb.n_rows ? sr.scale[k] * sr.totals[(int64_t)jb.row[l] * sr.width + k] : 0.0;
+        }
+        __syncthreads();
+        if (idx < RR) {
+            double acc[LIN_LC];
+#pragma unroll
+            for (int l = 0; l < LIN_LC; ++l) acc[l] = 0.0;
+            const int k0 = (parity_step == 2 && !sr.squares) ? ((idx / R + idx % R) & 1) : 0;
+            for (int k = k0; k < K; k += parity_step) {
+                const double c = sr.prod[(int64_t)k * RR + idx];
+#pragma unroll
+                for (int l = 0; l < LIN_LC; ++l) acc[l] = __builtin_fma(c, m_s[l * K + k], acc[l]);
+            }
+#pragma unroll
+            for (int l = 0; l < LIN_LC; ++l)
+                if (l < jb.n_rows) jb.out[(int64_t)jb.row[l] * RR + idx] += acc[l];
+        }
+    }
 }
 
 int launch_cov_finalize(mlmc_accum *a) {
@@ -1103,7 +1128,6 @@
     if (lin0) {
         if (int rc = flush_moments(a->lin0)) return rc;
     }
-    const dim3 lin_grid((a->R * a->R + 255) / 256, (a->n_levels * a->n_comp + LIN_LC - 1) / LIN_LC);
     const int pstep = a->basis->p.kind == MLMC_LEGENDRE ? 2 : 1;
     const int n_lc = a->n_levels * a->n_comp;
     const bool vals = a->cov_from_values;
@@ -1113,19 +1137,55 @@
                        a->RP, a->int_width, a->d_out_s, a->d_out_sp, a->d_counts, a->n_levels, a->d_out_n, a->d_out_nd,
                        a->mean_only ? 1 : 0, lin0 ? a->lin0->d_counts : (const int64_t *)nullptr);
     MLMC_HIP_CHECK(hipGetLastError());
+    const bool lin = a->lin && a->lin_used;
+    if (!lin && !lin0) return 0;
+    LinSrc src0, src02, src1;
+    std::memset(&src0, 0, sizeof(src0));
+    std::memset(&src02, 0, sizeof(src02));
+    std::memset(&src1, 0, sizeof(src1));
+    int max_K = 0;
     if (lin0) {
-        hipLaunchKernelGGL(k_cov_lin_mean, lin_grid, dim3(256), sizeof(double) * LIN_LC * a->lin_K, rt().stream,
-                           a->d_lin_prod, a->lin0->d_totals, a->lin0_basis->d_scale, R, a->lin_K, a->lin0->int_width, a->d_out_s, n_lc, pstep, 0);
-        hipLaunchKernelGGL(k_cov_lin_mean, lin_grid, dim3(256), sizeof(double) * LIN_LC * a->lin0_K, rt().stream,
-                           a->d_lin0_prod, a->lin0->d_totals, a->lin0_basis->d_scale, R, a->lin0_K, a->lin0->int_width, a->d_out_sp, n_lc, pstep, 1);
+        src0.prod = a->d_lin0_prod1; src0.totals = a->lin0->d_totals; src0.scale = a->lin0_basis->d_scale;
+        src0.width = a->lin0->int_width; src0.K = a->lin_K; src0.squares = 0;
+        src02 = src0;
+        src02.prod = a->d_lin0_prod; src02.K = a->lin0_K; src02.squares = 1;
+        max_K = a->lin0_K;
+    }
+    if (lin) {
+        src1.prod = a->d_lin_prod; src1.totals = a->lin->d_totals; src1.scale = a->lin_basis->d_scale;
+        src1.width = a->lin->int_width; src1.K = a->lin_K; src1.squares = 0;
+        if (a->lin_K > max_K) max_K = a->lin_K;
+    }
+    LinJobs jobs;
+    std::memset(&jobs, 0, sizeof(jobs));
+    int n_jobs = 0;
+    const dim3 block(256);
+    auto launch = [&]() -> int {
+        if (n_jobs == 0) return 0;
+        hipLaunchKernelGGL(k_cov_lin_mean, dim3((R * R + 255) / 256, n_jobs), block, sizeof(double) * LIN_LC * max_K, rt().stream, jobs, R, pstep);
         MLMC_HIP_CHECK(hipGetLastError());
-    }
-    if (a->lin && a->lin_used) {
-        hipLaunchKernelGGL(k_cov_lin_mean, lin_grid, dim3(256), sizeof(double) * LIN_LC * a->lin_K, rt().stream,
-                           a->d_lin_prod, a->lin->d_totals, a->lin_basis->d_scale, R, a->lin_K, a->lin->int_width, a->d_out_s, n_lc, pstep, 0);
-        MLMC_HIP_CHECK(hipGetLastError());
-    }
-    return 0;
-}
-
-}
+        std::memset(&jobs, 0, sizeof(jobs));
+        n_jobs = 0;
+        return 0;
+    };
+    for (int cls = 1; cls <= 4; ++cls) {
+        LinJob *jb = nullptr;
+        for (int lc = 0; lc < n_lc; ++lc) {
+            const int level = lc / a->n_comp;
+            const int fed = ((lin0 && a->lin0_levels[level]) ? 1 : 0) | ((lin && a->lin_levels[level]) ? 2 : 0);
+            if (cls <= 3 ? fed != cls : !(fed & 1)) continue;
+            if (!jb || jb->n_rows == LIN_LC) {
+                if (n_jobs == LIN_MAX_JOBS)
+                    if (int rc = launch()) return rc;
+                jb = &jobs.job[n_jobs++];
+                jb->out = cls == 4 ? a->d_out_sp : a->d_out_s;
+                jb->src[0] = cls == 4 ? src02 : (cls == 2 ? src1 : src0);
+                if (cls == 3) jb->src[1] = src1;
+            }
+            jb->row[jb->n_rows++] = lc;
+        }
+    }
+    return launch();
+}
+
+}
diff --git a/mlmc_amd/csrc/device_basis.hpp b/mlmc_amd/csrc/device_basis.hpp
--- a/mlmc_amd/csrc/device_basis.hpp
+++ b/mlmc_amd/csrc/device_basis.hpp
@@ -44,7 +44,7 @@
 struct TermGen {
     double x, p1, p2, c1, s1;
     __device__ __forceinline__ void init(double x_, double w, const BasisParams &) {
-        x = KIND == MLMC_LEGENDRE ? 2.0 * x_ : x_;
+        x = (KIND == MLMC_LEGENDRE || KIND == KIND_CHEBYSHEV) ? 2.0 * x_ : x_;
         p1 = w;
         p2 = 0.0;
         if (KIND == MLMC_FOURIER) {
@@ -59,9 +59,27 @@
             p2 = p1;
             p1 = q;
             return q;
+        } else if (KIND == KIND_CHEBYSHEV) {
+            const double q = __builtin_fma(x, p1, -p2);
+            p2 = p1;
+            p1 = q;
+            return q;
         } else {
             return next(2 + (j & 1));
         }
+    }
+    __device__ __forceinline__ void jump128() {
+        const double w = p1, t = 0.5 * x;
+        double a = t, b = __builtin_fma(x, t, -1.0);
+#pragma unroll
+        for (int k = 0; k < 7; ++k) {
+            const double a2 = 2.0 * a;
+            b = __builtin_fma(a2, b, -t);
+            a = __builtin_fma(a2, a, -1.0);
+        }
+        const double c = __builtin_fma(x, a, -b);
+        p2 = __builtin_fma(x, c, -a) * w;
+        p1 = c * w;
     }
     __device__ __forceinline__ double next(int i) {
         if (i == 0) return p1;
@@ -69,6 +87,13 @@
             double q;
             if (i == 1) q = x * p1;
             else q = __builtin_fma(x, p1, -(kLegendreG.v[i] * p2));
+            p2 = p1;
+            p1 = q;
+            return q;
+        } else if (KIND == KIND_CHEBYSHEV) {
+            double q;
+            if (i == 1) q = (0.5 * x) * p1;
+            else q = __builtin_fma(x, p1, -p2);
             p2 = p1;
             p1 = q;
             return q;
diff --git a/mlmc_amd/csrc/moments.hip b/mlmc_amd/csrc/moments.hip
--- a/mlmc_amd/csrc/moments.hip
+++ b/mlmc_amd/csrc/moments.hip
@@ -454,13 +454,13 @@
 __device__ __forceinline__ void split_export(const TermGen<KIND> &g, double *__restrict__ slot) {
     slot[0 * SPLIT_LANES] = g.x;
     slot[1 * SPLIT_LANES] = g.p1;
-    if (KIND == MLMC_LEGENDRE) slot[2 * SPLIT_LANES] = g.p2;
+    if (KIND == MLMC_LEGENDRE || KIND == KIND_CHEBYSHEV) slot[2 * SPLIT_LANES] = g.p2;
 }
 template <int KIND>
 __device__ __forceinline__ void split_import(TermGen<KIND> &g, const double *__restrict__ slot) {
     g.x = slot[0 * SPLIT_LANES];
     g.p1 = slot[1 * SPLIT_LANES];
-    g.p2 = KIND == MLMC_LEGENDRE ? slot[2 * SPLIT_LANES] : 0.0;
+    g.p2 = (KIND == MLMC_LEGENDRE || KIND == KIND_CHEBYSHEV) ? slot[2 * SPLIT_LANES] : 0.0;
     g.c1 = g.s1 = 0.0;
 }
 
@@ -515,7 +515,13 @@
             gf[q].init(keep ? tf : 0.0, w, bp);
             if (PAIR) gc[q].init(keep ? tc : 0.0, w, bp);
         }
-        if (T0 > 0) {
+        if constexpr (KIND == KIND_CHEBYSHEV && T0 == 128) {
+#pragma unroll
+            for (int q = 0; q < NS; ++q) {
+                gf[q].jump128();
+                if (PAIR) gc[q].jump128();
+            }
+        } else if (T0 > 0) {
 #pragma unroll
             for (int i = 0; i < T0; ++i) {
 #pragma unroll
@@ -863,6 +869,7 @@
 }
 constexpr int SPLIT_MEAN_HEAD_96 = 46, SPLIT_MEAN_HEAD_128 = 62;
 constexpr int SPLIT_MEAN_HEAD_W2 = 40;
+constexpr int SPLIT_CHEB_HEAD_96 = 45, SPLIT_CHEB_HEAD_128 = 61, SPLIT_CHEB_HEAD_W2 = 51;
 static int split_dispatch(int op, bool plain, const BasisParams &bp, int n_split, int t0, const SegTable *tab, int total_blocks, double *partials,
                           int64_t *pcounts, int *out) {
 #define MLMC_SPLIT_GO(KIND, P)                                                                                                          \
@@ -870,8 +877,17 @@
      : n_split == 64 ? split_go<KIND, P, SPLIT_HEAD, 64 - SPLIT_HEAD, MLMC_SPLIT_WPS, true>(op, bp, tab, total_blocks, partials, pcounts, out)   \
      : n_split == 96 ? split_go<KIND, P, SPLIT_MEAN_HEAD_96, 96 - SPLIT_MEAN_HEAD_96, 2, false>(op, bp, tab, total_blocks, partials, pcounts, out) \
                      : split_go<KIND, P, SPLIT_MEAN_HEAD_128, 128 - SPLIT_MEAN_HEAD_128, 2, false>(op, bp, tab, total_blocks, partials, pcounts, out))
+#define MLMC_SPLIT_GO_CHEB(P)                                                                                                           \
+    (t0 == 128 ? split_go<KIND_CHEBYSHEV, P, SPLIT_CHEB_HEAD_W2, 128 - SPLIT_CHEB_HEAD_W2, 2, false, 128>(op, bp, tab, total_blocks, partials, pcounts, out) \
+     : n_split == 96 ? split_go<KIND_CHEBYSHEV, P, SPLIT_CHEB_HEAD_96, 96 - SPLIT_CHEB_HEAD_96, 2, false>(op, bp, tab, total_blocks, partials, pcounts, out) \
+                     : split_go<KIND_CHEBYSHEV, P, SPLIT_CHEB_HEAD_128, 128 - SPLIT_CHEB_HEAD_128, 2, false>(op, bp, tab, total_blocks, partials, pcounts, out))
+    if (bp.kind == KIND_CHEBYSHEV) {
+        if (n_split == 64 && t0 == 0) return fail("moments: Chebyshev sums exist for the mean-only term-split kernels (65..256 terms)");
+        return plain ? MLMC_SPLIT_GO_CHEB(true) : MLMC_SPLIT_GO_CHEB(false);
+    }
     if (bp.kind == MLMC_LEGENDRE) return plain ? MLMC_SPLIT_GO(MLMC_LEGENDRE, true) : MLMC_SPLIT_GO(MLMC_LEGENDRE, false);
     return plain ? MLMC_SPLIT_GO(MLMC_MONOMIAL, true) : MLMC_SPLIT_GO(MLMC_MONOMIAL, false);
+#undef MLMC_SPLIT_GO_CHEB
 #undef MLMC_SPLIT_GO
 }
 
@@ -884,10 +900,12 @@
     const bool sparse_spline = bp.kind == MLMC_SPLINE;
     if (sparse_spline && R > SPLINE_MAX_R) return fail("spline moments: at most 512 basis functions");
     static const bool no_split = std::getenv("MLMC_HIP_NO_SPLIT") != nullptr;
-    const bool poly = bp.kind == MLMC_LEGENDRE || bp.kind == MLMC_MONOMIAL;
+    const bool cheb = bp.kind == KIND_CHEBYSHEV;
+    const bool poly = bp.kind == MLMC_LEGENDRE || bp.kind == MLMC_MONOMIAL || cheb;
     const bool poly64 = poly && R > 48 && R <= 64;
-    const bool split_mean = poly && a->mean_only_plain && R > 64 && R <= 256 && !no_split;
+    const bool split_mean = poly && a->mean_only_plain && R > 64 && R <= 256 && (!no_split || cheb);
     const bool split = (poly64 && !no_split) || split_mean;
+    if (cheb && !split_mean) return fail("moments: Chebyshev sums exist for the mean-only term-split kernels (65..256 terms)");
     const int pass_terms = split_mean ? 128 : ((poly64 && !split) ? 32 : MAX_TERMS_PER_PASS);
     for (int t0 = 0; t0 < (sparse_spline ? 1 : R); t0 += pass_terms) {
         const int n_terms = (R - t0 < pass_terms) ? R - t0 : pass_terms;
@@ -898,8 +916,8 @@
         bool plain = bp.kind != MLMC_IDENTITY && !bp.is_log && bp.is_clip;
         for (const PendingSeg &p : a->pending) plain = plain && p.mask == nullptr;
         if (split) {
-            static int occ_split[2][2][4];
-            int &cached = occ_split[bp.kind == MLMC_LEGENDRE ? 0 : 1][plain ? 1 : 0][t0 ? 3 : (n_split == 64 ? 0 : (n_split == 96 ? 1 : 2))];
+            static int occ_split[3][2][4];
+            int &cached = occ_split[bp.kind == MLMC_LEGENDRE ? 0 : (cheb ? 2 : 1)][plain ? 1 : 0][t0 ? 3 : (n_split == 64 ? 0 : (n_split == 96 ? 1 : 2))];
             if (cached == 0)
                 if (int rc = split_dispatch(0, plain, bp, n_split, t0, nullptr, 0, nullptr, nullptr, &cached)) return rc;
             per_cu = cached;
@@ -910,6 +928,7 @@
                 if (int rc = accum_dispatch(0, plain, bp, rt_sel, nullptr, 0, t0, nullptr, nullptr, &cached)) return rc;
             per_cu = cached;
         }
+        if (cheb && per_cu > 2) per_cu = 2;
         if (per_cu < 1) per_cu = 1;
         if (per_cu > 8) per_cu = 8;
         const int resident = rt().n_cu * per_cu;
```

Measured after the change: 308.9 billion, median of 6. 1.05x the previous value.
